# Swedish-Rock-Art-Research-Archives/rock-art-radnet

Hardware: AMD Instinct MI355X
Metric: train images/sec, ResNet50 Faster R-CNN 1000x600 (higher is better)
Workload: dtype f32; 1 GPU; full train step (RPN + RoiPoolingConv + classifier head + losses + 2x Adam), ResNet50, 1000x600, batch=1 per GPU, base frozen (train.py); identical panel and boxes on every rank and step (per-rank RNG seed); bench_workload=train, per_gpu_batch=1, global_batch=1, anchors=12, n_rois=20, mini_batch_form=image by image, parallelism=dp1, base_forward=launch list (hipGraph)

## Files before the change

### include/radnet_hip.h

```cpp
#ifndef RADNET_HIP_H
#define RADNET_HIP_H

#include <stdint.h>

#ifdef __cplusplus
extern "C" {
#endif

typedef struct radnet_ctx radnet_ctx;

#define RADNET_OK 0
#define RADNET_ERR_ARG (-1)
#define RADNET_ERR_HIP (-2)
#define RADNET_ERR_UNSUPPORTED (-3)

int radnet_create(int device, void* hip_stream, radnet_ctx** out);
void radnet_destroy(radnet_ctx* ctx);
const char* radnet_last_error(radnet_ctx* ctx);
int radnet_sync(radnet_ctx* ctx);
int radnet_set_stream(radnet_ctx* ctx, void* hip_stream);
int radnet_version(void);
int radnet_set_workspace(radnet_ctx* ctx, void* ws, uint64_t bytes);
int radnet_set_autotune(radnet_ctx* ctx, int enable);
int radnet_tuned_shapes(radnet_ctx* ctx);
int radnet_tune_save(radnet_ctx* ctx, const char* path);
int radnet_share_tuning(radnet_ctx* ctx, radnet_ctx* owner);
int radnet_tune_load(radnet_ctx* ctx, const char* path);
int radnet_force_config(radnet_ctx* ctx, int tile_a, int tile_b, int slices);
int radnet_force_waves(radnet_ctx* ctx, int waves);
int radnet_set_deterministic(radnet_ctx* ctx, int enable);
int radnet_get_deterministic(radnet_ctx* ctx);
int radnet_timing_enable(radnet_ctx* ctx, int enable);
int radnet_timing_read(radnet_ctx* ctx, int cls, double* ms, int64_t* launches, double* flops);
int radnet_timing_reset(radnet_ctx* ctx);

typedef struct radnet_conv_desc {
  const float* x;
  const float* w;
  float* y;
  const float* scale;
  const float* shift;
  const float* addend;
  int32_t nb, h, w_, c;
  int32_t oh, ow;
  int32_t kh, kw, stride, pad_t, pad_l;
  int32_t n;
  int32_t ldw, ldy, ld_add;
  int32_t act;
  int32_t act_cols;
  const float* dy;
  const float* gscale;
  float* dx;
  const float* dx_add;
  const float* dx_mask;
  float* dw;
  int32_t ld_dy, ld_dx, ld_dx_add, ld_dx_mask;
  int32_t dw_accumulate;
  float* db;
} radnet_conv_desc;

int radnet_conv_fwd(radnet_ctx* ctx, const radnet_conv_desc* d);
int radnet_gemm_batched(radnet_ctx* ctx, const float* a, const float* b, float* y, int32_t batch, int32_t m, int32_t n, int32_t k);
int radnet_winograd_filter(radnet_ctx* ctx, const float* w, int32_t c, int32_t n, int32_t ldw, float* u);
int radnet_winograd_input(radnet_ctx* ctx, const float* x, int32_t nb, int32_t h, int32_t w, int32_t c, float* v);
int radnet_winograd_output(radnet_ctx* ctx, const float* m, int32_t nb, int32_t oh, int32_t ow, int32_t n, const float* scale,
                           const float* shift, int32_t act, float* y, int32_t ldy);
int radnet_winograd_dy(radnet_ctx* ctx, const float* dy, int32_t nb, int32_t oh, int32_t ow, int32_t n, int32_t ld_dy,
                       const float* gscale, float* dz);
int radnet_wgrad_batched(radnet_ctx* ctx, const float* a, const float* dy, float* dw, int32_t batch, int32_t m, int32_t k, int32_t n,
                         int32_t accumulate);
int radnet_winograd_filter_grad(radnet_ctx* ctx, const float* du, int32_t c, int32_t n, int32_t ldw, float* dw, int32_t accumulate);
int radnet_winograd4_filter(radnet_ctx* ctx, const float* w, int32_t c, int32_t n, int32_t ldw, float* u);
int radnet_winograd4_input(radnet_ctx* ctx, const float* x, int32_t nb, int32_t h, int32_t w, int32_t c, float* v);
int radnet_winograd4_output(radnet_ctx* ctx, const float* m, int32_t nb, int32_t oh, int32_t ow, int32_t n, const float* scale,
                            const float* shift, int32_t act, float* y, int32_t ldy);
int radnet_winograd4_dy(radnet_ctx* ctx, const float* dy, int32_t nb, int32_t oh, int32_t ow, int32_t n, int32_t ld_dy,
                        const float* gscale, float* dz);
int radnet_winograd4_filter_grad(radnet_ctx* ctx, const float* du, int32_t c, int32_t n, int32_t ldw, float* dw, int32_t accumulate);
int radnet_conv_dgrad(radnet_ctx* ctx, const radnet_conv_desc* d);
int radnet_conv_wgrad(radnet_ctx* ctx, const radnet_conv_desc* d);
int radnet_conv_bwd(radnet_ctx* ctx, const radnet_conv_desc* d);
typedef struct radnet_wgrad_adam {
  float* p; float* g; float* m; float* v;
  int64_t n;
  int32_t t;
  float lr, beta1, beta2, eps, grad_scale;
} radnet_wgrad_adam;
int radnet_conv_wgrad_multi(radnet_ctx* ctx, const radnet_conv_desc* descs, int32_t n, const radnet_wgrad_adam* opt);
int radnet_conv_fwd_pair(radnet_ctx* ctx, const radnet_conv_desc* d1, const radnet_conv_desc* d2);
int radnet_conv_bottleneck(radnet_ctx* ctx, const radnet_conv_desc* db, const radnet_conv_desc* dc, const radnet_conv_desc* da);

int radnet_weights_to_bf16(radnet_ctx* ctx, const float* w, int32_t k, int32_t n, int32_t ldw, uint16_t* wt, int32_t ldk);
int radnet_conv_fwd_bf16(radnet_ctx* ctx, const radnet_conv_desc* d, const uint16_t* wt, int32_t ldk);
int radnet_conv_fwd_bf16_split(radnet_ctx* ctx, const radnet_conv_desc* d, const uint16_t* wt, int32_t ldk, int32_t ksplit);
int32_t radnet_conv_bf16_pick_split(int64_t m, int32_t n, int32_t k);
int64_t radnet_conv_bf16_tile_shape(int64_t rows, int32_t cols, int32_t* bm, int32_t* bn);

typedef struct radnet_bf16_dgrad_image {
  int64_t off;
  int32_t taps, c, n, ldw;
  uint16_t* wd;
  int32_t ldkd;
} radnet_bf16_dgrad_image;
int radnet_weights_to_bf16_dgrad(radnet_ctx* ctx, const float* w, int32_t taps, int32_t c, int32_t n, int32_t ldw, uint16_t* wd, int32_t ldkd);
int radnet_weights_to_bf16_dgrad_arena(radnet_ctx* ctx, const float* p, int64_t n_arena, const radnet_bf16_dgrad_image* layers, int32_t n_layers);
int radnet_conv_dgrad_bf16(radnet_ctx* ctx, const radnet_conv_desc* d, const uint16_t* wd, int32_t ldkd);
int radnet_conv_dgrad_bf16_split(radnet_ctx* ctx, const radnet_conv_desc* d, const uint16_t* wd, int32_t ldkd, int32_t ksplit);
int radnet_conv_wgrad_bf16(radnet_ctx* ctx, const radnet_conv_desc* d, int32_t msplit);
int32_t radnet_dgrad_bf16_pick_split(int64_t p, int32_t c, int32_t kd);
int32_t radnet_wgrad_bf16_pick_split(int64_t m, int32_t n, int32_t k);

int radnet_colsum(radnet_ctx* ctx, const float* g, int32_t m, int32_t n, int32_t ld, const float* gscale,
                  float* out, int32_t accumulate);

int radnet_maxpool_fwd(radnet_ctx* ctx, const float* x, float* y, int32_t nb, int32_t h, int32_t w, int32_t c,
                       int32_t k, int32_t s);
int radnet_roi_resize_fwd(radnet_ctx* ctx, const float* fmap, int32_t h, int32_t w, int32_t c, const float* rois,
                          int32_t r, int32_t ps, float* y);
int radnet_roi_resize_bwd(radnet_ctx* ctx, const float* dy, int32_t h, int32_t w, int32_t c, const float* rois,
                          int32_t r, int32_t ps, float* dfmap);
int radnet_avgpool_fwd(radnet_ctx* ctx, const float* x, int32_t r, int32_t hw, int32_t c, float* y);
int radnet_avgpool_bwd_relu(radnet_ctx* ctx, const float* dfeat, const float* y_act, int32_t r, int32_t hw, int32_t c,
                            float* dx);

int radnet_dense_heads_fwd(radnet_ctx* ctx, const float* feat, int32_t r, int32_t k, const float* w, int32_t ldw,
                           const float* b, int32_t nc, int32_t nreg, float* out_cls, float* out_regr);
int radnet_dense_heads_bwd(radnet_ctx* ctx, const float* feat, const float* dz, int32_t r, int32_t k, const float* w,
                           int32_t ldw, int32_t nout, float* dw, float* db, float* dfeat, int32_t accumulate);

uint64_t radnet_head_tail_scratch_bytes(int32_t r);
int radnet_head_tail_fwd(radnet_ctx* ctx, const float* y5, int32_t r, int32_t hw, int32_t c, const float* w, int32_t ldw, const float* b,
                         int32_t nc, int32_t nreg, float* feat, float* p_cls, float* p_regr, const float* y1, const float* y2,
                         float* dz, float* losses, int32_t groups, const int32_t* group_live, void* scratch);

int radnet_rpn_loss(radnet_ctx* ctx, const float* pred, int32_t ld_pred, const float* y_cls, const float* y_regr,
                    int32_t m, int32_t a, int32_t bce_mode, float* dz, int32_t ld_dz, float* losses,
                    double* scratch8);
int radnet_det_loss(radnet_ctx* ctx, const float* p_cls, const float* p_regr, const float* y1, const float* y2,
                    int32_t r, int32_t nc, int32_t nreg, float* dz, float* losses);

int radnet_adam_step(radnet_ctx* ctx, float* p, float* g, float* m, float* v, int64_t n, int32_t t, float lr,
                     float beta1, float beta2, float eps, float grad_scale, int32_t zero_grad);
int radnet_adam_step_affine(radnet_ctx* ctx, float* p, float* g, float* m, float* v, int64_t n, int32_t t, float lr, float beta1, float beta2,
                            float eps, float grad_scale, int32_t zero_grad, int64_t bias_off, int64_t bias_len, const float* scale,
                            const float* t0, float* shift);
typedef struct radnet_adam_wino {
  int64_t off;
  int32_t c, n;
  float* u;
} radnet_adam_wino;
int radnet_adam_step_fused(radnet_ctx* ctx, float* p, float* g, float* m, float* v, int64_t n, int32_t t, float lr, float beta1, float beta2,
                           float eps, float grad_scale, int32_t zero_grad, int64_t bias_off, int64_t bias_len, const float* scale,
                           const float* t0, float* shift, const radnet_adam_wino* layers, int32_t n_layers);
int radnet_adam_step_tail(radnet_ctx* ctx, float* p, float* g, float* m, float* v, int64_t n, int32_t t, float lr, float beta1, float beta2,
                          float eps, float grad_scale, int32_t zero_grad, int64_t bias_off, int64_t bias_len, const float* scale,
                          const float* t0, float* shift, const radnet_adam_wino* layers, int32_t n_layers, int64_t sweep_from);
typedef struct radnet_adam_bf16 {
  int64_t off;
  int32_t k, n, ldw;
  uint16_t* wt;
  int32_t ldk;
} radnet_adam_bf16;
int radnet_adam_step_bf16(radnet_ctx* ctx, float* p, float* g, float* m, float* v, int64_t n, int32_t t, float lr, float beta1, float beta2,
                          float eps, float grad_scale, int32_t zero_grad, int64_t bias_off, int64_t bias_len, const float* scale,
                          const float* t0, float* shift, const radnet_adam_bf16* layers, int32_t n_layers);

uint64_t radnet_proposals_ws_bytes(int64_t n_anchors_total);
int radnet_rpn_to_roi(radnet_ctx* ctx, const float* pred, int32_t ld_pred, int32_t rows, int32_t cols, int32_t a,
                      const double* anchor_wh_host, double std_scaling, int32_t use_regr, double overlap_thresh,
                      int32_t max_boxes, int64_t* out_boxes, float* out_probs, int32_t* out_count, void* ws);
int radnet_nms(radnet_ctx* ctx, const double* boxes, const float* probs, int32_t n, double overlap_thresh,
               int32_t max_boxes, int32_t* out_idx, int32_t* out_count, void* ws);

int radnet_anchor_targets(radnet_ctx* ctx, const double* gt, const int32_t* gt_is_bg, int32_t g, int32_t width,
                          int32_t height, int32_t rw, int32_t rh, int32_t fw, int32_t fh, const double* anchor_sizes_host,
                          int32_t ns, const double* anchor_ratios_host, int32_t nr, double rpn_stride,
                          double max_overlap, uint8_t* valid, uint8_t* overlap, double* regr, int32_t* best_anchor,
                          int32_t* n_for_gt, void* scratch);
int radnet_anchor_targets_pack(radnet_ctx* ctx, const uint8_t* valid, const uint8_t* overlap, const double* regr,
                               int32_t fw, int32_t fh, int32_t a, double std_scaling, float* y_cls, float* y_regr);

int radnet_roi_targets(radnet_ctx* ctx, const int64_t* rois, int32_t n, const double* gt, const int32_t* gt_cls, int32_t g,
                       int32_t width, int32_t height, int32_t rw, int32_t rh, double rpn_stride, double min_overlap,
                       double max_overlap, const double* regr_std_host4, int32_t bg_class, uint8_t* keep, int32_t* cls,
                       int32_t* box, double* t, double* iou, const int32_t* n_dev);
int radnet_roi_batch_pack(radnet_ctx* ctx, const int32_t* sel, int32_t r, const int32_t* cls, const int32_t* box,
                          const double* t, int32_t nc, int32_t bg_class, float* rois_out, float* y1, float* y2);

int64_t radnet_host_choice_round(double* live_p, int64_t* live_idx, int64_t* n_live_io, int64_t* found, int64_t n_found,
                                 const double* x, int64_t k, double* cdf, uint8_t* sel);

int radnet_preprocess_bgr(radnet_ctx* ctx, const uint8_t* img, int32_t h, int32_t w, int32_t cpad, float* out);
int radnet_copy_bytes(radnet_ctx* ctx, void* dst, const void* src, uint64_t bytes);
int radnet_resize_bicubic_u8(radnet_ctx* ctx, const uint8_t* src, int32_t sh, int32_t sw, uint8_t* dst, int32_t dh,
                             int32_t dw, int32_t channels);
int radnet_resize_bicubic_window_u8(radnet_ctx* ctx, const uint8_t* src, int32_t sh, int32_t sw, int32_t y0, int32_t x0, int32_t wh,
                                    int32_t ww, uint8_t* dst, int32_t dh, int32_t dw, int32_t channels);
int radnet_warp_affine_u8(radnet_ctx* ctx, const uint8_t* src, int32_t sh, int32_t sw, int32_t channels, uint8_t* dst, int32_t dh,
                          int32_t dw, const int32_t* col_tab, const int32_t* row_tab);
int radnet_aug_gather_u8(radnet_ctx* ctx, const uint8_t* src, int32_t sh, int32_t sw, int32_t y0, int32_t x0, int32_t wh, int32_t ww,
                         int32_t transform, uint8_t* dst);
int radnet_aug_extent_u8(radnet_ctx* ctx, const uint8_t* img, int32_t h, int32_t w, int32_t* out4);
int radnet_aug_histogram_u8(radnet_ctx* ctx, const uint8_t* img, int32_t h, int32_t w, int32_t all_channels, uint32_t* bins256);
#define RADNET_AUG_BRIGHTNESS 0
#define RADNET_AUG_CONTRAST 1
#define RADNET_AUG_SALT_PEPPER 2
#define RADNET_AUG_GAUSSIAN 3
#define RADNET_AUG_POISSON 4
int radnet_aug_pointwise_u8(radnet_ctx* ctx, const uint8_t* src, uint8_t* dst, int32_t h, int32_t w, int32_t mode, int32_t grey, double p0,
                            double p1, uint64_t noise_seed, uint32_t field_id);
#define RADNET_PNG_UNFILTER_BAND_ROWS 512
#define RADNET_PNG_UNFILTER_CHUNK_BYTES 96
int radnet_png_unfilter_u8(radnet_ctx* ctx, uint8_t* stream, int32_t rows, int32_t rowbytes, int32_t bpp);
typedef struct radnet_png_segment {
  int64_t offset;
  int32_t rows;
  int32_t rowbytes;
} radnet_png_segment;
#define RADNET_PNG_SEGMENT_TARGET_ROWS 64
int radnet_png_plan_segments(const uint8_t* stream, int64_t stream_offset, int32_t rows, int32_t rowbytes, int32_t target_rows,
                             radnet_png_segment* out, int32_t cap);
int radnet_png_unfilter_segments_u8(radnet_ctx* ctx, uint8_t* base, int64_t base_len, const radnet_png_segment* segs_host,
                                    const radnet_png_segment* segs_dev, int32_t count, int32_t bpp);
int radnet_png_expand_bgr_u8(radnet_ctx* ctx, const uint8_t* stream, int32_t pass_h, int32_t pass_w, int32_t rowbytes, int32_t color_type,
                             int32_t bit_depth, const uint8_t* palette_bgr, uint8_t* dst, int32_t dst_h, int32_t dst_w, int32_t y0,
                             int32_t x0, int32_t dy, int32_t dx);
int radnet_png_filter_rows_u8(radnet_ctx* ctx, const uint8_t* img, int32_t h, int32_t w, int32_t channels, int64_t pitch_bytes, int32_t mode,
                              uint8_t* stream);
#define RADNET_DEFLATE_CHUNK 65536
#define RADNET_DEFLATE_TILE 4096
#define RADNET_DEFLATE_SYMBOLS 286
#define RADNET_DEFLATE_HEADER_MAX_BITS 2048
typedef struct radnet_deflate_code {
  uint16_t bits, length;
} radnet_deflate_code;
int radnet_deflate_rle_scan_u8(radnet_ctx* ctx, const uint8_t* stream, int64_t n, uint32_t* hist, uint64_t* adler_parts);
int radnet_deflate_rle_emit_u8(radnet_ctx* ctx, const uint8_t* stream, int64_t n, const radnet_deflate_code* code, const uint8_t* header_bits,
                               int32_t header_nbits, int32_t dist_nbits, uint8_t* pieces, int64_t piece_cap, uint32_t* sizes);
int64_t radnet_deflate_piece_cap(const radnet_deflate_code* code, int32_t header_nbits, int32_t dist_nbits);
int radnet_deflate_pack(radnet_ctx* ctx, const uint8_t* pieces, int64_t piece_cap, const uint32_t* sizes, int32_t count, uint8_t* out,
                        int64_t out_cap, uint64_t* total);
// ... 292 lines not shown
```

### rock-art-radnet_amd/csrc/adam.hip

```cpp
#include "radnet_internal.h"
#include "adam_update.h"
#include "radnet_wino4.h"

namespace {

constexpr int kAdamWinoMax = 12;
constexpr int kAdamBf16Max = 16;
constexpr int kAdamBf16Tile = 64;
constexpr int kAdamGapMax = kAdamBf16Max + 1;

struct AdamArgs {
  float4 *p, *g, *m, *v;
  float lr_t, b1, b2, eps, gs;
  int zero_grad;
  long long aff_off4, aff_n4;
  const float4 *aff_scale, *aff_t0;
  float4* aff_shift;
  long long gap0[kAdamGapMax], pref[kAdamGapMax + 1];
  int ngap;
  unsigned sweep_blocks;
};

__device__ __forceinline__ void adam_one(float4& pp, const float4& gg, float4& mm, float4& vv, float lr_t, float b1, float b2, float eps, float gs) {
  adam_update1(pp.x, gg.x, mm.x, vv.x, lr_t, b1, b2, eps, gs);
  adam_update1(pp.y, gg.y, mm.y, vv.y, lr_t, b1, b2, eps, gs);
  adam_update1(pp.z, gg.z, mm.z, vv.z, lr_t, b1, b2, eps, gs);
  adam_update1(pp.w, gg.w, mm.w, vv.w, lr_t, b1, b2, eps, gs);
}

__device__ __forceinline__ float4 adam_at(const AdamArgs& a, long long i) {
  float4 pp = a.p[i], mm = a.m[i], vv = a.v[i];
  adam_one(pp, a.g[i], mm, vv, a.lr_t, a.b1, a.b2, a.eps, a.gs);
  a.p[i] = pp;
  a.m[i] = mm;
  a.v[i] = vv;
  if (a.zero_grad) a.g[i] = make_float4(0.f, 0.f, 0.f, 0.f);
  return pp;
}

__device__ __forceinline__ void adam_sweep(const AdamArgs& a) {
  const long long rest = a.pref[a.ngap];
  for (long long j = (long long)blockIdx.x * blockDim.x + threadIdx.x; j < rest; j += (long long)a.sweep_blocks * blockDim.x) {
    long long at = a.gap0[0];
    for (int q = 1; q < a.ngap; ++q) {
      const long long first = a.pref[q], to = a.gap0[q] - first;
      at = j >= first ? to : at;
    }
    const long long i = at + j;
    const float4 pp = adam_at(a, i);
    if (a.aff_shift != nullptr && i >= a.aff_off4 && i < a.aff_off4 + a.aff_n4) {
      const long long s = i - a.aff_off4;
      const float4 sc = a.aff_scale[s], c = a.aff_t0[s];
      a.aff_shift[s] = make_float4(sc.x * pp.x + c.x, sc.y * pp.y + c.y, sc.z * pp.z + c.z, sc.w * pp.w + c.w);
    }
  }
}

struct AdamWino {
  long long off4[kAdamWinoMax];
  int cn4[kAdamWinoMax];
  int unit0[kAdamWinoMax + 1];
  float* u[kAdamWinoMax];
  int n;
  int load_only;
};
__global__ void __launch_bounds__(256) adam_kernel(AdamArgs a, AdamWino wz) {
  if (blockIdx.x < a.sweep_blocks) {
    adam_sweep(a);
    return;
  }
  __shared__ float4 taps[9][64];
  const int unit = (int)(blockIdx.x - a.sweep_blocks);
  int layer = 0;
  for (int l = 1; l < wz.n; ++l)
    if (unit >= wz.unit0[l]) layer = l;
  const int cn4 = wz.cn4[layer];
  const long long j0 = (long long)(unit - wz.unit0[layer]) * 64;
  for (int it = threadIdx.x; it < 9 * 64; it += 256) {
    const int tap = it >> 6, jj = it & 63;
    const long long i = wz.off4[layer] + (long long)tap * cn4 + j0 + jj;
    taps[tap][jj] = wz.load_only ? a.p[i] : adam_at(a, i);
  }
  __syncthreads();
  if (threadIdx.x < 64) {
    float4 t[6][3];
#pragma unroll
    for (int bb = 0; bb < 3; ++bb) {
      float4 col[3], o[6];
#pragma unroll
      for (int aa = 0; aa < 3; ++aa) col[aa] = taps[aa * 3 + bb][threadIdx.x];
      g6(col, o);
#pragma unroll
      for (int aa = 0; aa < 6; ++aa) t[aa][bb] = o[aa];
    }
    float4* dst = reinterpret_cast<float4*>(wz.u[layer]) + j0 + threadIdx.x;
#pragma unroll
    for (int aa = 0; aa < 6; ++aa) {
      float4 o[6];
      g6(t[aa], o);
#pragma unroll
      for (int bb = 0; bb < 6; ++bb) dst[(long long)(6 * aa + bb) * cn4] = o[bb];
    }
  }
}

struct AdamBf16 {
  long long off4[kAdamBf16Max];
  int k[kAdamBf16Max], n[kAdamBf16Max], ldw4[kAdamBf16Max], ldk[kAdamBf16Max];
  int ntn[kAdamBf16Max];
  int unit0[kAdamBf16Max + 1];
  uint16_t* wt[kAdamBf16Max];
  int nl;
};
__global__ void __launch_bounds__(256) adam_bf16_kernel(AdamArgs a, AdamBf16 lz) {
  if (blockIdx.x < a.sweep_blocks) {
    adam_sweep(a);
    return;
  }
  __shared__ float tile[kAdamBf16Tile][kAdamBf16Tile + 1];
  const int unit = (int)(blockIdx.x - a.sweep_blocks);
  int layer = 0;
  for (int l = 1; l < lz.nl; ++l)
    if (unit >= lz.unit0[l]) layer = l;
  const int u = unit - lz.unit0[layer];
  const int k0 = (u / lz.ntn[layer]) * kAdamBf16Tile, n0 = (u % lz.ntn[layer]) * kAdamBf16Tile;
  const int K = lz.k[layer], ldw4 = lz.ldw4[layer];
  const int c4 = threadIdx.x & 15;
#pragma unroll
  for (int it = 0; it < 4; ++it) {
    const int r = (threadIdx.x >> 4) + 16 * it;
    const int kk = k0 + r, j4 = n0 / 4 + c4;
    float4 pp = make_float4(0.f, 0.f, 0.f, 0.f);
    if (kk < K && j4 < ldw4) pp = adam_at(a, lz.off4[layer] + (long long)kk * ldw4 + j4);
    tile[r][4 * c4] = pp.x; tile[r][4 * c4 + 1] = pp.y; tile[r][4 * c4 + 2] = pp.z; tile[r][4 * c4 + 3] = pp.w;
  }
  __syncthreads();
  const int N = lz.n[layer], ldk = lz.ldk[layer];
#pragma unroll
  for (int it = 0; it < 2; ++it) {
    const int q = threadIdx.x + 256 * it;
    const int c = q >> 3, kc = (q & 7) * 8;
    const int col = n0 + c, kk = k0 + kc;
    if (col >= N || kk >= ldk) continue;
    uint16_t h[8];
#pragma unroll
    for (int e = 0; e < 8; ++e) h[e] = kk + e < K ? __builtin_bit_cast(uint16_t, (__bf16)tile[kc + e][c]) : (uint16_t)0;
    uint4 o;
    o.x = h[0] | ((unsigned)h[1] << 16); o.y = h[2] | ((unsigned)h[3] << 16);
    o.z = h[4] | ((unsigned)h[5] << 16); o.w = h[6] | ((unsigned)h[7] << 16);
    *reinterpret_cast<uint4*>(lz.wt[layer] + (long long)col * ldk + kk) = o;
  }
}

struct AdamRange {
  int64_t off, len;
};

float adam_lr_t(float lr, float beta1, float beta2, int t) { return radnet_adam_lr_t(lr, beta1, beta2, t); }

int adam_check(radnet_ctx* ctx, const char* who, const float* p, const float* g, const float* m, const float* v, int64_t n, int32_t t,
               int64_t bias_off, int64_t bias_len, const float* scale, const float* t0, const float* shift) {
  if (!p || !g || !m || !v) RADNET_FAIL(ctx, RADNET_ERR_ARG, "%s: null arena", who);
  if (shift != nullptr && (!scale || !t0)) RADNET_FAIL(ctx, RADNET_ERR_ARG, "%s: shift without scale / t0", who);
  if ((n % 4) || (bias_off % 4) || (bias_len % 4) || n < 0 || bias_off < 0 || bias_len < 0 || bias_off + bias_len > n)
    RADNET_FAIL(ctx, RADNET_ERR_ARG, "%s: arena length %lld, bias range [%lld, +%lld) must be multiples of 4 inside the arena", who, (long long)n,
                (long long)bias_off, (long long)bias_len);
  if (((uintptr_t)p | (uintptr_t)g | (uintptr_t)m | (uintptr_t)v) & 15) RADNET_FAIL(ctx, RADNET_ERR_ARG, "%s: arenas must be 16-byte aligned", who);
  if (shift && (((uintptr_t)scale | (uintptr_t)t0 | (uintptr_t)shift) & 15)) RADNET_FAIL(ctx, RADNET_ERR_ARG, "%s: scale / t0 / shift must be 16-byte aligned", who);
  if (t < 1) RADNET_FAIL(ctx, RADNET_ERR_ARG, "%s: step counter starts at 1", who);
  return RADNET_OK;
}

int adam_gaps(radnet_ctx* ctx, const char* who, AdamRange* r, int nr, int64_t n, int64_t bias_off, int64_t bias_len, AdamArgs& a) {
  std::sort(r, r + nr, [](const AdamRange& x, const AdamRange& y) { return x.off < y.off; });
  long long at4 = 0;
  a.ngap = 0;
  a.pref[0] = 0;
  for (int q = 0; q <= nr; ++q) {
    if (q < nr) {
      if ((r[q].off & 3) || (r[q].len & 3) || r[q].off < 0 || r[q].len <= 0 || r[q].off + r[q].len > n)
        RADNET_FAIL(ctx, RADNET_ERR_ARG, "%s: layer [%lld, +%lld) must be multiples of 4 inside the arena", who, (long long)r[q].off, (long long)r[q].len);
      if (r[q].off / 4 < at4) RADNET_FAIL(ctx, RADNET_ERR_ARG, "%s: the layers at %lld and %lld overlap", who, (long long)r[q - 1].off, (long long)r[q].off);
      if (bias_len > 0 && r[q].off < bias_off + bias_len && bias_off < r[q].off + r[q].len)
        RADNET_FAIL(ctx, RADNET_ERR_ARG, "%s: layer [%lld, +%lld) overlaps the bias range", who, (long long)r[q].off, (long long)r[q].len);
    }
    const long long end4 = q < nr ? r[q].off / 4 : n / 4;
    a.gap0[a.ngap] = at4;
    a.pref[a.ngap + 1] = a.pref[a.ngap] + (end4 - at4);
    ++a.ngap;
    if (q < nr) at4 = end4 + r[q].len / 4;
  }
  a.sweep_blocks = (unsigned)grid_for(std::max<long long>(a.pref[a.ngap], 1), 256, 8192);
  return RADNET_OK;
}

int adam_prepare(radnet_ctx* ctx, const char* who, float* p, float* g, float* m, float* v, int64_t n, int32_t t, float lr, float beta1,
                 float beta2, float eps, float grad_scale, int32_t zero_grad, int64_t bias_off, int64_t bias_len, const float* scale,
                 const float* t0, float* shift, AdamRange* r, int nr, AdamArgs& a) {
  if (int rc = adam_check(ctx, who, p, g, m, v, n, t, bias_off, bias_len, scale, t0, shift)) return rc;
  a.p = reinterpret_cast<float4*>(p); a.g = reinterpret_cast<float4*>(g); a.m = reinterpret_cast<float4*>(m); a.v = reinterpret_cast<float4*>(v);
  a.lr_t = adam_lr_t(lr, beta1, beta2, t);
  a.b1 = beta1; a.b2 = beta2; a.eps = eps; a.gs = grad_scale;
  a.zero_grad = (int)zero_grad;
  a.aff_off4 = bias_off / 4;
  a.aff_n4 = shift ? bias_len / 4 : 0;
  a.aff_scale = reinterpret_cast<const float4*>(scale); a.aff_t0 = reinterpret_cast<const float4*>(t0); a.aff_shift = reinterpret_cast<float4*>(shift);
  return adam_gaps(ctx, who, r, nr, n, bias_off, shift ? bias_len : 0, a);
}

int adam_fused(radnet_ctx* ctx, const char* who, float* p, float* g, float* m, float* v, int64_t n, int32_t t, float lr, float beta1,
               float beta2, float eps, float grad_scale, int32_t zero_grad, int64_t bias_off, int64_t bias_len, const float* scale,
               const float* t0, float* shift, const radnet_adam_wino* layers, int32_t n_layers, int64_t sweep_from = 0) {
  if (!ctx) return RADNET_ERR_ARG;
  if (n_layers < 0 || n_layers > kAdamWinoMax || (n_layers > 0 && !layers)) RADNET_FAIL(ctx, RADNET_ERR_ARG, "%s: %d layers (at most %d, in a table)", who, n_layers, kAdamWinoMax);
  AdamWino wz{};
  AdamRange r[kAdamGapMax];
  wz.n = n_layers;
  wz.load_only = sweep_from > 0 ? 1 : 0;
  for (int l = 0; l < n_layers; ++l) {
    const radnet_adam_wino& d = layers[l];
    if (!d.u || d.c <= 0 || d.n <= 0 || (d.n & 3) || ((uintptr_t)d.u & 15) || (int64_t)d.c * d.n / 4 >= (1ll << 28) || ((int64_t)d.c * d.n / 4) % 64)
      RADNET_FAIL(ctx, RADNET_ERR_ARG, "%s: layer %d (offset %lld, c %d, n %d) does not describe a dense [3][3][c][n] kernel with c*n a multiple of 256 and a 16-byte aligned u",
                  who, l, (long long)d.off, d.c, d.n);
    wz.off4[l] = d.off / 4;
    wz.cn4[l] = (int)((int64_t)d.c * d.n / 4);
    wz.u[l] = d.u;
    wz.unit0[l + 1] = wz.unit0[l] + wz.cn4[l] / 64;
    r[l] = {d.off, 9ll * d.c * d.n};
  }
  int nr = n_layers;
  if (sweep_from > 0) {
    if ((sweep_from & 3) || sweep_from > n) RADNET_FAIL(ctx, RADNET_ERR_ARG, "%s: sweep_from %lld must be a multiple of 4 inside the arena", who, (long long)sweep_from);
    std::sort(r, r + n_layers, [](const AdamRange& x, const AdamRange& y) { return x.off < y.off; });
    int64_t at = 0;
    for (int l = 0; l <= n_layers; ++l) {
      const int64_t end = l < n_layers ? r[l].off : sweep_from;
      if (l < n_layers && (r[l].off < at || r[l].off + r[l].len > sweep_from))
        RADNET_FAIL(ctx, RADNET_ERR_ARG, "%s: layer [%lld, +%lld) overlaps another or reaches past sweep_from", who, (long long)r[l].off, (long long)r[l].len);
      if (end > at) {
        if (nr + 1 >= kAdamGapMax) RADNET_FAIL(ctx, RADNET_ERR_ARG, "%s: too many layers for the gap table", who);
        r[nr++] = {at, end - at};
      }
      if (l < n_layers) at = r[l].off + r[l].len;
    }
  }
  AdamArgs a{};
  if (int rc = adam_prepare(ctx, who, p, g, m, v, n, t, lr, beta1, beta2, eps, grad_scale, zero_grad, bias_off, bias_len, scale, t0, shift, r, nr, a)) return rc;
  hipLaunchKernelGGL(adam_kernel, dim3(a.sweep_blocks + (unsigned)wz.unit0[n_layers]), dim3(256), 0, ctx->stream, a, wz);
  RADNET_CHECK_LAUNCH(ctx, who);
  return RADNET_OK;
}

}

extern "C" int radnet_adam_step(radnet_ctx* ctx, float* p, float* g, float* m, float* v, int64_t n, int32_t t, float lr, float beta1,
// ... 56 lines not shown
```

### rock-art-radnet_amd/csrc/conv_args.h

```cpp
#pragma once

constexpr int BK = 32;
constexpr int NTHREADS = 256;
constexpr int kNumCU = 256;

struct GemmArgs {
  const float* x;
  const float* w;
  float* y;
  const float* scale;
  const float* shift;
  const float* addend;
  const float* mask;
  const float* in_scale;
  float* partial;
  int H, W, C;
  int OH, OW;
  int KW, npos;
  int stride, pad_t, pad_l;
  int M, N, K;
  int ldw, ldy, ld_add, ld_mask;
  int act, act_cols;
  int flip;
  int cin_fwd;
  const int* units;
  unsigned long long magic_ohow, magic_ow;
  int OHOW;
  unsigned x_bytes, w_bytes;
  unsigned y_bytes, add_bytes, mask_bytes;
  int batch;
  long long x_bstride, w_bstride, y_bstride;
  unsigned* counters;
  unsigned long long* stamps;
  int xcd_batch;
  int zper;
};

struct TailArgs {
  const float* w2; const float* sc2; const float* sh2; const float* add; float* y;
  const float* w3; const float* sc3; const float* sh3; float* t;
  int N2, ldw2, ldy2, ld_add2, ldw3, ldt;
  unsigned w2_bytes, w3_bytes, y_bytes, add_bytes, t_bytes;
};

struct WgradArgs {
  const float* x;
  const float* dy;
  const float* gscale;
  float* dw;
  float* db;
  int H, W, C, OH, OW, KW, stride, pad_t, pad_l;
  int M, N, K;
  int ld_dy, ldw;
  int mt_per_split;
  int atomic;
  const int* rowtab;
  int mpad;
  int xcd_batch;
  unsigned x_bias;
  unsigned x_bytes, dy_bytes;
  int batch, splits;
  long long x_bstride, dy_bstride, dw_bstride;
  float* slabs;
  unsigned* counters;
  int accumulate;
  int tiles_x, tiles_y;
  float* ow;
  float* om;
  float* ov;
  float lr_t, beta1, beta2, eps, grad_scale;
  int pad_opt;
};

constexpr int kWgradMultiMax = 16;
struct WgradMultiMap {
  unsigned first[kWgradMultiMax + 1];
  unsigned wx[kWgradMultiMax], wy[kWgradMultiMax];
  int n;
};
struct WgradOptScalars {
  float lr_t, beta1, beta2, eps, grad_scale;
};

struct PairMap {
  unsigned n_a, n_w;
  unsigned ax, ay;
  unsigned wx, wy;
};

struct ChainStage {
  GemmArgs g;
  const float* t_src;
  float* t_dst;
  const float* t_scale;
  const float* t_shift;
  int t_nb, t_h, t_w, t_c, t_th, t_tw, t_act, t_ldy;
  unsigned t_dst_bytes;
  int type;
};
struct ChainItem {
  int stage, bx, by, bz;
  int d0_first, d0_count, d1_first, d1_count;
  int sig0, sig1, pad0, pad1;
};
struct ChainHeader {
  unsigned next, exited, error, last_error;
  unsigned runs, host_lo, host_hi, pad;
};

constexpr int kCtrStride = 16;

static_assert(sizeof(GemmArgs) == 264 && sizeof(TailArgs) == 120 && sizeof(WgradArgs) == 248 && sizeof(PairMap) == 24, "kernel argument layout");
static_assert(sizeof(WgradMultiMap) == 200 && sizeof(WgradOptScalars) == 20, "multi-problem weight-gradient launch layout");
static_assert(sizeof(ChainStage) == 336 && sizeof(ChainItem) == 48 && sizeof(ChainHeader) == 32, "chain list layout");
```

### rock-art-radnet_amd/csrc/conv_device.h

```cpp
#pragma once
#include <hip/hip_runtime.h>
#include "conv_args.h"

typedef float f32x16 __attribute__((ext_vector_type(16)));
typedef float f32x4 __attribute__((ext_vector_type(4)));

namespace {
#ifndef RADNET_CHAINS
#define RADNET_CHAINS 2
#endif
constexpr int kChainsSmallTile = RADNET_CHAINS;

#ifdef RADNET_DIAG_STAMPS
#define RADNET_STAMP(var) const unsigned long long var = __builtin_amdgcn_s_memtime()
#else
#define RADNET_STAMP(var)
#endif

__device__ __forceinline__ int div_magic(int m, unsigned long long magic) {
  return (int)(((unsigned long long)(unsigned)m * magic) >> 40);
}

constexpr unsigned kOOB = 0x80000000u;
__device__ __forceinline__ __amdgpu_buffer_rsrc_t make_rsrc(const void* p, unsigned bytes) {
  return __builtin_amdgcn_make_buffer_rsrc(const_cast<void*>(p), 0, (int)bytes, 0x00020000);
}
__device__ __forceinline__ float4 buf_load4(__amdgpu_buffer_rsrc_t r, unsigned off) {
  f32x4 v = __builtin_bit_cast(f32x4, __builtin_amdgcn_raw_buffer_load_b128(r, (int)off, 0, 0));
  return make_float4(v.x, v.y, v.z, v.w);
}
__device__ __forceinline__ float4 buf_load4s(__amdgpu_buffer_rsrc_t r, unsigned voff, unsigned soff) {
  f32x4 v = __builtin_bit_cast(f32x4, __builtin_amdgcn_raw_buffer_load_b128(r, (int)voff, (int)__builtin_amdgcn_readfirstlane(soff), 0));
  return make_float4(v.x, v.y, v.z, v.w);
}
__device__ __forceinline__ float buf_load1s(__amdgpu_buffer_rsrc_t r, unsigned voff, unsigned soff) {
  return __builtin_bit_cast(float, __builtin_amdgcn_raw_buffer_load_b32(r, (int)voff, (int)__builtin_amdgcn_readfirstlane(soff), 0));
}
typedef unsigned u32x2 __attribute__((ext_vector_type(2)));
__device__ __forceinline__ int2 buf_load2i(__amdgpu_buffer_rsrc_t r, unsigned off) {
  const u32x2 v = __builtin_amdgcn_raw_buffer_load_b64(r, (int)off, 0, 0);
  return make_int2((int)v.x, (int)v.y);
}
__device__ __forceinline__ float buf_load1(__amdgpu_buffer_rsrc_t r, unsigned off) {
  return __builtin_bit_cast(float, __builtin_amdgcn_raw_buffer_load_b32(r, (int)off, 0, 0));
}
__device__ __forceinline__ float buf_load1_sc1(__amdgpu_buffer_rsrc_t r, unsigned off) {
  return __builtin_bit_cast(float, __builtin_amdgcn_raw_buffer_load_b32(r, (int)off, 0, 16));
}
__device__ __forceinline__ float4 buf_load4_sc1(__amdgpu_buffer_rsrc_t r, unsigned off) {
  f32x4 v = __builtin_bit_cast(f32x4, __builtin_amdgcn_raw_buffer_load_b128(r, (int)off, 0, 16));
  return make_float4(v.x, v.y, v.z, v.w);
}
__device__ __forceinline__ void buf_store4_sc1(__amdgpu_buffer_rsrc_t r, unsigned off, float4 v) {
  typedef unsigned u32x4 __attribute__((ext_vector_type(4)));
  f32x4 f = {v.x, v.y, v.z, v.w};
  __builtin_amdgcn_raw_buffer_store_b128(__builtin_bit_cast(u32x4, f), r, (int)off, 0, 16);
}
__device__ __forceinline__ void buf_store1_sc1(__amdgpu_buffer_rsrc_t r, unsigned off, float v) {
  __builtin_amdgcn_raw_buffer_store_b32(__builtin_bit_cast(unsigned, v), r, (int)off, 0, 16);
}
__device__ __forceinline__ void buf_store1(__amdgpu_buffer_rsrc_t r, unsigned off, float v) {
  __builtin_amdgcn_raw_buffer_store_b32(__builtin_bit_cast(unsigned, v), r, (int)off, 0, 0);
}
typedef float f32x2v __attribute__((ext_vector_type(2)));
__device__ __forceinline__ void buf_store2_sc1(__amdgpu_buffer_rsrc_t r, unsigned off, float2 v) {
  f32x2v f = {v.x, v.y};
  __builtin_amdgcn_raw_buffer_store_b64(__builtin_bit_cast(u32x2, f), r, (int)off, 0, 16);
}

__device__ __forceinline__ float f4_comp(const float4& v, int c) { return c == 0 ? v.x : c == 1 ? v.y : c == 2 ? v.z : v.w; }

struct NoStaging {
  __device__ __forceinline__ void operator()(int) const {}
};
template <int TM, int TN, int CH, typename Staging>
__device__ __forceinline__ void mfma_tile(const float* sA, const float* sB, int pitchA, int pitchB, int a_off, int b_off,
                                          f32x16 (&acc)[CH][TM][TN], Staging staging) {
  constexpr int kSteps = BK / 2;
  float a[3][TM], b[3][TN];
#pragma unroll
  for (int p = 0; p < 2; ++p) {
#pragma unroll
    for (int i = 0; i < TM; ++i) a[p][i] = sA[2 * p * pitchA + a_off + i * 32];
#pragma unroll
    for (int j = 0; j < TN; ++j) b[p][j] = sB[2 * p * pitchB + b_off + j * 32];
  }
#pragma unroll
  for (int s = 0; s < kSteps; ++s) {
    const int cur = s % 3, nxt = (s + 2) % 3;
    if (s + 2 < kSteps) {
#pragma unroll
      for (int i = 0; i < TM; ++i) a[nxt][i] = sA[(2 * s + 4) * pitchA + a_off + i * 32];
#pragma unroll
      for (int j = 0; j < TN; ++j) b[nxt][j] = sB[(2 * s + 4) * pitchB + b_off + j * 32];
    }
#pragma unroll
    for (int i = 0; i < TM; ++i)
#pragma unroll
      for (int j = 0; j < TN; ++j)
        acc[s % CH][i][j] = __builtin_amdgcn_mfma_f32_32x32x2f32(a[cur][i], b[cur][j], acc[s % CH][i][j], 0, 0, 0);
    staging(s);
    __builtin_amdgcn_sched_group_barrier(0x100, TM + TN, 0);
    __builtin_amdgcn_sched_group_barrier(0x008, TM * TN, 0);
    __builtin_amdgcn_sched_barrier(0);
  }
}

constexpr int kRowPitch = BK + 4;
template <int TM, int TN, int CH, bool B_ROWMAJOR, int KSTEPS, typename Staging>
__device__ __forceinline__ void mfma_tile_rows(const float* sA, const float* sB, int pitchB, int a_off, int b_off,
                                               f32x16 (&acc)[CH][TM][TN], Staging staging) {
  constexpr int kSteps = KSTEPS;
  float4 af[2][TM], bq[2][TN];
  float bf[3][TN];
#pragma unroll
  for (int i = 0; i < TM; ++i) af[0][i] = *reinterpret_cast<const float4*>(sA + a_off + i * 32 * kRowPitch);
  if (B_ROWMAJOR) {
#pragma unroll
    for (int j = 0; j < TN; ++j) bq[0][j] = *reinterpret_cast<const float4*>(sB + b_off + j * 32 * kRowPitch);
  } else {
#pragma unroll
    for (int p = 0; p < 2; ++p)
#pragma unroll
      for (int j = 0; j < TN; ++j) bf[p][j] = sB[p * pitchB + b_off + j * 32];
  }
#pragma unroll
  for (int s = 0; s < kSteps; ++s) {
    const int q = s >> 2, c = s & 3;
    const bool group_reads = c == 1 && q + 1 < kSteps / 4;
    const bool step_reads = !B_ROWMAJOR && s + 2 < kSteps;
    if (group_reads) {
#pragma unroll
      for (int i = 0; i < TM; ++i) af[(q + 1) & 1][i] = *reinterpret_cast<const float4*>(sA + a_off + i * 32 * kRowPitch + 8 * (q + 1));
      if (B_ROWMAJOR) {
#pragma unroll
        for (int j = 0; j < TN; ++j) bq[(q + 1) & 1][j] = *reinterpret_cast<const float4*>(sB + b_off + j * 32 * kRowPitch + 8 * (q + 1));
      }
    }
    if (step_reads) {
      const int s2 = s + 2;
#pragma unroll
      for (int j = 0; j < TN; ++j) bf[s2 % 3][j] = sB[(8 * (s2 >> 2) + (s2 & 3)) * pitchB + b_off + j * 32];
    }
#pragma unroll
    for (int i = 0; i < TM; ++i)
#pragma unroll
      for (int j = 0; j < TN; ++j)
        acc[s % CH][i][j] = __builtin_amdgcn_mfma_f32_32x32x2f32(f4_comp(af[q & 1][i], c), B_ROWMAJOR ? f4_comp(bq[q & 1][j], c) : bf[s % 3][j],
                                                                 acc[s % CH][i][j], 0, 0, 0);
    staging(s);
    if (group_reads && (B_ROWMAJOR || step_reads)) __builtin_amdgcn_sched_group_barrier(0x100, TM + TN, 0);
    else if (group_reads) __builtin_amdgcn_sched_group_barrier(0x100, TM, 0);
    else if (step_reads) __builtin_amdgcn_sched_group_barrier(0x100, TN, 0);
    __builtin_amdgcn_sched_group_barrier(0x008, TM * TN, 0);
    __builtin_amdgcn_sched_barrier(0);
  }
}
}
```

### rock-art-radnet_amd/csrc/conv_wgrad.hip

```cpp
#include "conv_host.h"
#include "conv_igemm_body.h"
#include "conv_wgrad_body.h"
#include "wgrad_multi_plan.h"

namespace {
template <int BMK, int BN>
__global__ void __launch_bounds__(NTHREADS) conv_wgrad_kernel(WgradArgs g) {
  __shared__ __attribute__((aligned(16))) float lds[wgrad_lds_floats<BMK, BN>()];
  if (g.batch > 1 && g.xcd_batch) {
    const unsigned gx = gridDim.x, gy = gridDim.y, total = gx * gy * gridDim.z;
    const unsigned lin = blockIdx.x + gx * (blockIdx.y + gy * blockIdx.z), per = total >> 3;
    const unsigned l2 = lin < (per << 3) ? (lin & 7u) * per + (lin >> 3) : lin;
    const unsigned z = l2 / (gx * gy), r = l2 - z * gx * gy, y = r / gx;
    conv_wgrad_body<BMK, BN>(g, lds, r - y * gx, y, z);
    return;
  }
  conv_wgrad_body<BMK, BN>(g, lds, blockIdx.x, blockIdx.y, blockIdx.z);
}


template <int ABM>
__global__ void __launch_bounds__(NTHREADS) conv_bwd_pair_kernel(GemmArgs ga, WgradArgs gw, PairMap pm) {
  constexpr int kLds = igemm_lds_floats<ABM, 64, 1>() > wgrad_lds_floats<64, 64>() ? igemm_lds_floats<ABM, 64, 1>() : wgrad_lds_floats<64, 64>();
  __shared__ __attribute__((aligned(16))) float lds[kLds];
// ... 128 lines not shown
    else if (bmk == 128 && bn == 64) RADNET_LAUNCH((conv_wgrad_kernel<128, 64>), grid, block, 0, ctx->stream, ctx->arm0, ctx->arm1, g);
    else if (bmk == 64 && bn == 128) RADNET_LAUNCH((conv_wgrad_kernel<64, 128>), grid, block, 0, ctx->stream, ctx->arm0, ctx->arm1, g);
    else RADNET_LAUNCH((conv_wgrad_kernel<64, 64>), grid, block, 0, ctx->stream, ctx->arm0, ctx->arm1, g);
    RADNET_CHECK_LAUNCH(ctx, "conv_wgrad");
    return RADNET_OK;
  };
  int bmk = (d->c % 128 == 0) ? 128 : 64, bn = g.N > 64 ? 128 : 64, splits = 1;
  const radnet_shape_key key{2 + (d->dw_accumulate == 1 ? 1 : 0) + (batch > 1 ? 16 : 0), g.M, g.N, g.K, g.C, d->kh * d->kw, batch > 1 ? batch : g.stride};
  auto it = ctx->tuned->find(key);
  if (ctx->force_a > 0) {
    bmk = ctx->force_a; bn = ctx->force_b; splits = ctx->force_splits < 1 ? 1 : ctx->force_splits;
    if (bmk < 64) bmk = 64;
    if (bn < 64) bn = 64;
    if (d->c % bmk) RADNET_FAIL(ctx, RADNET_ERR_ARG, "conv_wgrad: forced k tile %d does not divide c=%d", bmk, d->c);
  } else if (it != ctx->tuned->end()) {
    bmk = it->second.a; bn = it->second.b; splits = it->second.splits;
  } else if (const radnet_tuned* nb = (ctx->autotune == 2 && d->dw_accumulate != 1) ? radnet_tuned_neighbour(*ctx->tuned, key) : nullptr;
             nb && (nb->splits <= 1 || (nmt / nb->splits >= 2 && radnet_cdiv(nmt, radnet_cdiv(nmt, nb->splits)) == nb->splits))) {
    bmk = nb->a; bn = nb->b; splits = nb->splits;
    (*ctx->tuned)[key] = *nb;
  } else if (ctx->autotune && d->dw_accumulate != 1) {
    PairPause pause(ctx);
    struct WCand { float ms; int bmk, bn, s; };
    std::vector<WCand> seen;
    const bool for_pair = pause.saved != nullptr && batch <= 1 && d->dx != nullptr;
    for (int cb = 128; cb >= 64; cb -= 64) {
      if (d->c % cb) continue;
      if (for_pair && cb != 64) continue;
      for (int cn = 128; cn >= 64; cn -= 64) {
        if (cn > 64 && g.N <= 64) continue;
        if (for_pair && cn != 64) continue;
        for (int s0 : {1, 2, 3, 4, 6, 8, 12, 16}) {
          if (s0 > 1 && (nmt / s0 < 2 || radnet_cdiv(nmt, radnet_cdiv(nmt, s0)) != s0)) continue;
          for (int s = s0; s >= (batch > 1 ? -s0 : s0); s -= 2 * s0) {
            float ms = 0.f;
            int rc = radnet_time_launches(ctx, [&]() { return launch(cb, cn, s); }, 3, &ms);
            if (rc == RADNET_ERR_UNSUPPORTED) continue;
            if (rc != RADNET_OK) return rc;
            seen.push_back(WCand{ms, cb, cn, s});
          }
        }
      }
    }
    std::sort(seen.begin(), seen.end(), [](const WCand& a, const WCand& b) { return a.ms < b.ms; });
    float best = 1e30f;
    for (size_t i = 0; i < seen.size() && i < 4; ++i) {
      float ms = 0.f;
      const int rc = radnet_time_launches_twice(ctx, [&]() { return launch(seen[i].bmk, seen[i].bn, seen[i].s); }, 12, &ms);
      if (rc != RADNET_OK) return rc;
      if (ms < best) { best = ms; bmk = seen[i].bmk; bn = seen[i].bn; splits = seen[i].s; }
    }
    (*ctx->tuned)[key] = radnet_tuned{bmk, bn, splits, best, 4};
    if (getenv("RADNET_TUNE_LOG"))
      fprintf(stderr, "radnet tune: wgrad M=%d N=%d K=%d C=%d -> tile %dx%d slices %d : %.1f us (%.1f TFLOP/s)\n", g.M, g.N, g.K, g.C,
              bmk, bn, splits, best * 1e3, 2.0 * g.M * g.N * g.K / (best * 1e9));
    if (d->dw_accumulate == 2)
      RADNET_CHECK_HIP(ctx, hipMemset2DAsync(d->dw, (size_t)g.ldw * sizeof(float), 0, (size_t)g.N * sizeof(float), (size_t)g.K, ctx->stream));
  } else {
    const radnet_shape_key k0{2, g.M, g.N, g.K, g.C, d->kh * d->kw, g.stride};
    auto it0 = ctx->tuned->find(k0);
    if (it0 != ctx->tuned->end()) {
      bmk = it0->second.a; bn = it0->second.b; splits = it0->second.splits;
    } else {
      long long tiles = (long long)radnet_cdiv(g.K, bmk) * radnet_cdiv(g.N, bn);
      if (tiles < kNumCU && bmk == 128 && bn == 128) {
        bn = 64;
        tiles = (long long)radnet_cdiv(g.K, bmk) * radnet_cdiv(g.N, bn);
      }
      while (tiles * splits < 2 * kNumCU && nmt / (splits * 2) >= 4 && splits < 16) splits *= 2;
    }
  }
  radnet_timing_arm(ctx);
  {
    g.db = d->db;
    if (d->db && d->dw_accumulate == 0) RADNET_CHECK_HIP(ctx, hipMemsetAsync(d->db, 0, (size_t)g.N * sizeof(float), ctx->stream));
    int rc = launch(bmk, bn, splits);
    if (rc == RADNET_ERR_UNSUPPORTED && splits < 0) {
      splits = -splits;
      rc = launch(bmk, bn, splits);
    }
    if (rc == RADNET_ERR_UNSUPPORTED && splits > 1) {
      while (rc == RADNET_ERR_UNSUPPORTED && splits > 1) {
        splits = splits > 2 ? splits / 2 : 1;
        while (splits > 1 && radnet_cdiv(nmt, radnet_cdiv(nmt, splits)) != splits) --splits;
        rc = launch(bmk, bn, splits);
      }
    }
    if (rc == RADNET_ERR_UNSUPPORTED) RADNET_FAIL(ctx, rc, "conv_wgrad: no launch shape fits (tile %dx%d, workspace %llu bytes)", bmk, bn, (unsigned long long)ctx->ws_bytes);
    if (rc != RADNET_OK) return rc;
  }
  RADNET_CHECK_LAUNCH(ctx, "conv_wgrad");
  radnet_timing_end_armed(ctx, 2, 2.0 * g.M * g.N * g.K * (batch > 1 ? batch : 1));
  return RADNET_OK;
}

extern "C" int radnet_conv_wgrad(radnet_ctx* ctx, const radnet_conv_desc* d) { return run_wgrad(ctx, d, 1, 0, 0, 0); }

extern "C" int radnet_conv_bwd(radnet_ctx* ctx, const radnet_conv_desc* d) {
  if (!ctx || !d) return RADNET_ERR_ARG;
  static const bool disabled = radnet_env_flag("RADNET_NO_BWD_PAIR");
  if (disabled || ctx->pair_capture != nullptr || !d->dx) {
    int rc = radnet_conv_wgrad(ctx, d);
    return rc != RADNET_OK || !d->dx ? rc : radnet_conv_dgrad(ctx, d);
  }
  PairCapture pc;
  const int timed = ctx->timing;
  ctx->timing = 0;
  ctx->pair_capture = &pc;
  int rc = radnet_conv_wgrad(ctx, d);
  if (rc == RADNET_OK) rc = radnet_conv_dgrad(ctx, d);
  ctx->pair_capture = nullptr;
  ctx->timing = timed;
  if (rc != RADNET_OK) return rc;
  if (pc.a_slab_bytes + pc.w_slab_bytes > ctx->ws_bytes) pc.a_ok = false;
  if (!(pc.have_a && pc.have_w && pc.a_ok && pc.w_ok)) {
    rc = radnet_conv_wgrad(ctx, d);
    return rc != RADNET_OK ? rc : radnet_conv_dgrad(ctx, d);
  }
  PairMap pm{pc.ax * pc.ay, pc.wx * pc.wy * pc.wz, pc.ax, pc.ay, pc.wx, pc.wy};
  radnet_timing_arm(ctx);
  if (pc.a_bm == 32) RADNET_LAUNCH(conv_bwd_pair_kernel<32>, dim3(pm.n_a + pm.n_w), dim3(NTHREADS), 0, ctx->stream, ctx->arm0, ctx->arm1, pc.ga, pc.gw, pm);
  else RADNET_LAUNCH(conv_bwd_pair_kernel<64>, dim3(pm.n_a + pm.n_w), dim3(NTHREADS), 0, ctx->stream, ctx->arm0, ctx->arm1, pc.ga, pc.gw, pm);
  RADNET_CHECK_LAUNCH(ctx, "conv_bwd_pair");
  radnet_timing_end_armed(ctx, 4, pc.flops);
  return RADNET_OK;
}

radnet_ctx::MultiTables::~MultiTables() {
  for (auto& e : v)
    if (e.second) (void)hipFree(e.second);
}

namespace {
const WgradArgs* get_multi_table(radnet_ctx* ctx, const WgradArgs* host, int n) {
  const size_t bytes = sizeof(WgradArgs) * (size_t)n;
  auto& v = ctx->multi_tables.v;
  for (auto& e : v)
    if (e.first.size() == bytes && memcmp(e.first.data(), host, bytes) == 0) return (const WgradArgs*)e.second;
  if (v.size() >= 256) {
    (void)hipFree(v.front().second);
    v.erase(v.begin());
  }
  void* dev = nullptr;
  if (hipMalloc(&dev, bytes) != hipSuccess) return nullptr;
  if (hipMemcpy(dev, host, bytes, hipMemcpyHostToDevice) != hipSuccess) {
    (void)hipFree(dev);
    return nullptr;
  }
  v.emplace_back(std::vector<char>((const char*)host, (const char*)host + bytes), dev);
  return (const WgradArgs*)dev;
}
}

extern "C" int radnet_conv_wgrad_multi(radnet_ctx* ctx, const radnet_conv_desc* descs, int32_t n, const radnet_wgrad_adam* opt) {
  if (!ctx || n < 0 || (n > 0 && !descs)) return RADNET_ERR_ARG;
  if (n == 0) return RADNET_OK;
  if (ctx->pair_capture != nullptr) RADNET_FAIL(ctx, RADNET_ERR_ARG, "conv_wgrad_multi: called inside radnet_conv_bwd");
  const bool adam = opt != nullptr && opt->p != nullptr;
  if (adam) {
    if (!opt->g || !opt->m || !opt->v || opt->n <= 0) RADNET_FAIL(ctx, RADNET_ERR_ARG, "conv_wgrad_multi: optimizer block with a null arena");
    if (opt->t < 1) RADNET_FAIL(ctx, RADNET_ERR_ARG, "conv_wgrad_multi: step counter starts at 1");
  }
  std::vector<PairCapture> pcs((size_t)n);
  std::vector<WgradMultiItem> items((size_t)n);
  const int timed = ctx->timing;
  for (int i = 0; i < n; ++i) {
    radnet_conv_desc d = descs[i];
    d.dx = nullptr;
    if (adam) {
      if (d.dw_accumulate == 1) RADNET_FAIL(ctx, RADNET_ERR_ARG, "conv_wgrad_multi: problem %d adds to its gradient; the optimizer epilogue needs the whole gradient", i);
      const int64_t off = d.dw - opt->g, last = (int64_t)(d.kh * d.kw * d.c - 1) * d.ldw + d.n;
      if (!d.dw || d.dw < opt->g || off + last > opt->n) RADNET_FAIL(ctx, RADNET_ERR_ARG, "conv_wgrad_multi: problem %d's dw lies outside the gradient arena", i);
    }
    ctx->timing = 0;
    ctx->pair_capture = &pcs[i];
    const int rc = radnet_conv_wgrad(ctx, &d);
    ctx->pair_capture = nullptr;
    ctx->timing = timed;
    if (rc != RADNET_OK) return rc;
    PairCapture& pc = pcs[i];
    if (!pc.have_w) RADNET_FAIL(ctx, RADNET_ERR_UNSUPPORTED, "conv_wgrad_multi: problem %d produced no launch", i);
    const bool ordered = pc.gw.slabs != nullptr;
    if (adam && !ordered && pc.gw.atomic)
      RADNET_FAIL(ctx, RADNET_ERR_UNSUPPORTED, "conv_wgrad_multi: problem %d adds its slices with atomics (no final writer); the optimizer epilogue needs ordered reductions", i);
    items[i] = WgradMultiItem{pc.w_bmk, pc.w_bn, pc.wx, pc.wy, pc.wz, ordered ? pc.w_slab_need : 0, ordered ? pc.wx * pc.wy : 0u};
  }
  std::vector<WgradMultiLaunch> plan((size_t)n);
  const int nl = wgrad_multi_plan(items.data(), n, ctx->ws_bytes, (unsigned)kAuxWgradCounterCount, plan.data(), n);
  if (nl < 0) RADNET_FAIL(ctx, RADNET_ERR_UNSUPPORTED, "conv_wgrad_multi: the problems do not fit a launch plan (%d)", nl);
  WgradOptScalars os{};
  if (adam) os = WgradOptScalars{radnet_adam_lr_t(opt->lr, opt->beta1, opt->beta2, opt->t), opt->beta1, opt->beta2, opt->eps, opt->grad_scale};
  for (int l = 0; l < nl; ++l) {
    const WgradMultiLaunch& L = plan[l];
    WgradArgs host[kWgradMultiMax];
    memset(host, 0, sizeof(host));
    double flops = 0.0;
    for (int k = 0; k < L.n; ++k) {
      const PairCapture& pc = pcs[L.problem[k]];
      WgradArgs& g = host[k];
      memcpy(&g, &pc.gw, sizeof(g));
      if (g.slabs != nullptr) {
        g.slabs = reinterpret_cast<float*>(reinterpret_cast<char*>(ctx->ws) + L.slab_off[k]);
        g.counters = reinterpret_cast<unsigned*>(ctx->aux + kAuxWgradCounters) + L.counter_off[k];
      }
      g.ow = g.om = g.ov = nullptr;
      g.lr_t = g.beta1 = g.beta2 = g.eps = g.grad_scale = 0.f;
      g.pad_opt = 0;
      if (adam) {
        const int64_t off = g.dw - opt->g;
        g.ow = opt->p + off; g.om = opt->m + off; g.ov = opt->v + off;
      }
      flops += 2.0 * g.M * g.N * g.K;
    }
    const WgradArgs* tab = get_multi_table(ctx, host, L.n);
    if (!tab) RADNET_FAIL(ctx, RADNET_ERR_HIP, "conv_wgrad_multi: cannot place the problem table on the device");
    const dim3 grid(L.map.first[L.n]), block(NTHREADS);
    radnet_timing_arm(ctx);
    if (L.bmk == 128 && L.bn == 128) RADNET_LAUNCH((conv_wgrad_multi_kernel<128, 128>), grid, block, 0, ctx->stream, ctx->arm0, ctx->arm1, tab, L.map, os);
    else if (L.bmk == 128 && L.bn == 64) RADNET_LAUNCH((conv_wgrad_multi_kernel<128, 64>), grid, block, 0, ctx->stream, ctx->arm0, ctx->arm1, tab, L.map, os);
    else if (L.bmk == 64 && L.bn == 128) RADNET_LAUNCH((conv_wgrad_multi_kernel<64, 128>), grid, block, 0, ctx->stream, ctx->arm0, ctx->arm1, tab, L.map, os);
    else RADNET_LAUNCH((conv_wgrad_multi_kernel<64, 64>), grid, block, 0, ctx->stream, ctx->arm0, ctx->arm1, tab, L.map, os);
    RADNET_CHECK_LAUNCH(ctx, "conv_wgrad_multi");
    radnet_timing_end_armed(ctx, 2, flops);
  }
  return RADNET_OK;
}

extern "C" int radnet_wgrad_batched(radnet_ctx* ctx, const float* a, const float* dy, float* dw, int32_t batch, int32_t m, int32_t k, int32_t n,
                                    int32_t accumulate) {
  if (!ctx || !a || !dy || !dw) return RADNET_ERR_ARG;
  if (batch < 1 || batch > 4096) RADNET_FAIL(ctx, RADNET_ERR_ARG, "wgrad_batched: batch %d", batch);
  radnet_conv_desc d{};
  d.x = a; d.dy = dy; d.dw = dw;
  d.nb = 1; d.h = 1; d.w_ = m; d.c = k; d.oh = 1; d.ow = m;
  d.kh = 1; d.kw = 1; d.stride = 1; d.pad_t = 0; d.pad_l = 0; d.n = n;
  d.ldw = n; d.ld_dy = n;
  d.dw_accumulate = accumulate;
  return run_wgrad(ctx, &d, batch, (long long)m * k, (long long)m * n, (long long)k * n);
}
```

### rock-art-radnet_amd/csrc/conv_wgrad_body.h

```cpp
#pragma once
#include "adam_update.h"
#include "conv_device.h"

namespace {
template <int BMK, int BN>
constexpr int wgrad_lds_floats() { return 2 * BK * ((BMK + 4) + (BN + 4)); }

template <int BMK, int BN, bool OPT = false>
__device__ __forceinline__ void conv_wgrad_body(const WgradArgs& g, float* __restrict__ lds, const unsigned bid_x, const unsigned bid_y, const unsigned bid_z) {
  constexpr int TM = BMK / 64, TN = BN / 64;
  constexpr int PA = BMK + 4, PB = BN + 4;
  constexpr int A_ITERS = BMK / 32, B_ITERS = BN / 32;
  constexpr int CPRA = BMK / 4, CPRB = BN / 4;
  float* sA0 = lds;
  float* sB0 = lds + 2 * BK * PA;

  const int tid = threadIdx.x;
  const int lane = tid & 63, wave = tid >> 6;
  const int hi = lane >> 5, l31 = lane & 31;
  const int wm = wave >> 1, wn = wave & 1;
  const int k0 = bid_x * BMK, n0 = bid_y * BN;

  const int pos = k0 / g.C;
  const int cbase = k0 - pos * g.C;

  const int a_k4 = tid % CPRA, a_mr = tid / CPRA;
  const int b_n4 = tid % CPRB, b_mr = tid / CPRB;
  const bool a_kv = (k0 + a_k4 * 4) < g.K;
  const bool b_nv = (n0 + b_n4 * 4) < g.N;
  float4 gs = make_float4(1, 1, 1, 1);
  if (g.gscale != nullptr && b_nv) gs = *reinterpret_cast<const float4*>(g.gscale + n0 + b_n4 * 4);

  const int nmt = (g.M + BK - 1) / BK;
  const int zsplit = g.batch > 1 ? (int)(bid_z % (unsigned)g.splits) : (int)bid_z;
  const long long bp = g.batch > 1 ? (long long)(bid_z / (unsigned)g.splits) : 0;
  const int mt_begin = zsplit * g.mt_per_split;
  int mt_end = mt_begin + g.mt_per_split;
  if (mt_end > nmt) mt_end = nmt;

  const __amdgpu_buffer_rsrc_t rx = make_rsrc(reinterpret_cast<const char*>(g.x + bp * g.x_bstride) - g.x_bias, g.x_bytes + g.x_bias);
  const __amdgpu_buffer_rsrc_t rdy = make_rsrc(g.dy + bp * g.dy_bstride, g.dy_bytes);
  float4 ra[A_ITERS], rb[B_ITERS];
  const bool do_bias = g.db != nullptr && bid_x == 0;
  float4 csum = make_float4(0.f, 0.f, 0.f, 0.f);

  const __amdgpu_buffer_rsrc_t rtab = make_rsrc(g.rowtab + (size_t)pos * g.mpad, (unsigned)g.mpad * 4u);
  const unsigned s_tap = (unsigned)(cbase * 4);
  unsigned b_voff[B_ITERS], e_voff[A_ITERS];
#pragma unroll
  for (int i = 0; i < B_ITERS; ++i) b_voff[i] = b_nv ? (unsigned)(((b_mr + (NTHREADS / CPRB) * i) * g.ld_dy + n0 + b_n4 * 4) * 4) : kOOB;
#pragma unroll
  for (int i = 0; i < A_ITERS; ++i) e_voff[i] = (unsigned)((a_mr + (NTHREADS / CPRA) * i) * 4);
  const unsigned a_lane = a_kv ? (unsigned)a_k4 * 16u : kOOB;
  const unsigned dy_tile_bytes = (unsigned)(BK * g.ld_dy * 4);
  struct Entries {
    unsigned e[A_ITERS];
  };
  Entries ent0, ent1;

  constexpr int kLoadOps = A_ITERS + B_ITERS, kStoreOps = A_ITERS + B_ITERS;
  auto entry_op = [&](int i, int mt, Entries& en) {
    en.e[i] = __builtin_amdgcn_raw_buffer_load_b32(rtab, (int)e_voff[i], (int)__builtin_amdgcn_readfirstlane(mt < mt_end ? (unsigned)mt * (BK * 4u) : kOOB), 0);
  };
  auto load_op = [&](int idx, int mt, const Entries& en) {
    const bool live = mt < mt_end;
    if (idx < A_ITERS) {
      ra[idx] = buf_load4s(rx, en.e[idx] + a_lane, live ? s_tap : kOOB);
    } else {
      rb[idx - A_ITERS] = buf_load4s(rdy, b_voff[idx - A_ITERS], live ? (unsigned)mt * dy_tile_bytes : kOOB);
    }
  };
  auto store_op = [&](int idx, int buf) {
    float* sA = sA0 + buf * BK * PA;
    float* sB = sB0 + buf * BK * PB;
    if (idx < A_ITERS) {
      const int i = idx;
      *reinterpret_cast<float4*>(sA + (a_mr + (NTHREADS / CPRA) * i) * PA + a_k4 * 4) = ra[i];
    } else {
      const int i = idx - A_ITERS;
      float4 v = rb[i];
      v.x *= gs.x; v.y *= gs.y; v.z *= gs.z; v.w *= gs.w;
      *reinterpret_cast<float4*>(sB + (b_mr + (NTHREADS / CPRB) * i) * PB + b_n4 * 4) = v;
      csum.x += do_bias ? v.x : 0.f; csum.y += do_bias ? v.y : 0.f; csum.z += do_bias ? v.z : 0.f; csum.w += do_bias ? v.w : 0.f;
    }
  };

  constexpr int CH = (TM * TN >= 4) ? 1 : kChainsSmallTile;
  f32x16 accs[CH][TM][TN];
#pragma unroll
  for (int c = 0; c < CH; ++c)
#pragma unroll
    for (int i = 0; i < TM; ++i)
#pragma unroll
      for (int j = 0; j < TN; ++j)
#pragma unroll
        for (int r = 0; r < 16; ++r) accs[c][i][j][r] = 0.f;

  if (mt_begin < mt_end) {
#pragma unroll
    for (int i = 0; i < A_ITERS; ++i) entry_op(i, mt_begin, ent0);
#pragma unroll
    for (int op = 0; op < kLoadOps; ++op) load_op(op, mt_begin, ent0);
#pragma unroll
    for (int i = 0; i < A_ITERS; ++i) entry_op(i, mt_begin + 1, ent1);
#pragma unroll
    for (int op = 0; op < kStoreOps; ++op) store_op(op, 0);
    __syncthreads();
    const int a_off = hi * PA + wm * (BMK / 2) + l31;
    const int b_off = hi * PB + wn * (BN / 2) + l31;
    constexpr int kSteps = BK / 2;
    constexpr int kStoreSteps = (kStoreOps < kSteps - 1 - kLoadOps) ? kStoreOps : kSteps - 1 - kLoadOps;
    constexpr int kStoresPerStep = (kStoreOps + kStoreSteps - 1) / kStoreSteps;
    constexpr int kFirstStoreStep = kSteps - 1 - kStoreSteps;
    static_assert(kStoreSteps >= 1, "tile too large for the 16-step staging schedule");
    auto step = [&](int mt, int buf, Entries& cur, Entries& nxt) {
      mfma_tile<TM, TN, CH>(sA0 + buf * BK * PA, sB0 + buf * BK * PB, PA, PB, a_off, b_off, accs, [&](int s) {
        if (s < kLoadOps) {
          load_op(s, mt + 1, cur);
          if (s < A_ITERS) entry_op(s, mt + 2, nxt);
        } else if (s >= kFirstStoreStep && s < kSteps - 1) {
#pragma unroll
          for (int q = 0; q < kStoresPerStep; ++q) {
            const int op = (s - kFirstStoreStep) * kStoresPerStep + q;
            if (op < kStoreOps) store_op(op, buf ^ 1);
          }
        }
      });
      __syncthreads();
    };
    for (int mt = mt_begin; mt < mt_end; mt += 2) {
      step(mt, 0, ent1, ent0);
      if (mt + 1 < mt_end) step(mt + 1, 1, ent0, ent1);
    }
  }
  f32x16(&acc)[TM][TN] = accs[0];
#pragma unroll
  for (int c = 1; c < CH; ++c)
#pragma unroll
    for (int i = 0; i < TM; ++i)
#pragma unroll
      for (int j = 0; j < TN; ++j) acc[i][j] += accs[c][i][j];

  const bool ordered = g.slabs != nullptr;
  float4 bias_t = make_float4(0.f, 0.f, 0.f, 0.f);
  if (do_bias) {
    float4* red = reinterpret_cast<float4*>(lds);
    red[tid] = csum;
    __syncthreads();
    if (tid < CPRB) {
      float4 t = red[tid];
      for (int q = 1; q < NTHREADS / CPRB; ++q) {
        const float4 u = red[tid + q * CPRB];
        t.x += u.x; t.y += u.y; t.z += u.z; t.w += u.w;
      }
      bias_t = t;
      const int n = n0 + tid * 4;
      if (!ordered && n < g.N) {
        atomicAdd(g.db + n, t.x);
        atomicAdd(g.db + n + 1, t.y);
        atomicAdd(g.db + n + 2, t.z);
        atomicAdd(g.db + n + 3, t.w);
      }
    }
    __syncthreads();
  }

  if (ordered) {
    const unsigned tile = ((unsigned)bp * (unsigned)g.tiles_y + bid_y) * (unsigned)g.tiles_x + bid_x;
    const unsigned lane_off = (unsigned)((wave * TM * TN * 64 + lane) * 16) * 4u;
    const size_t total_tiles = (size_t)(g.batch > 1 ? g.batch : 1) * g.tiles_y * g.tiles_x;
    const __amdgpu_buffer_rsrc_t rslab = make_rsrc(g.slabs + ((size_t)tile * g.splits + zsplit) * (BMK * BN), BMK * BN * 4u);
#pragma unroll
    for (int i = 0; i < TM; ++i)
#pragma unroll
      for (int j = 0; j < TN; ++j)
#pragma unroll
        for (int q = 0; q < 4; ++q)
          buf_store4_sc1(rslab, lane_off + (unsigned)(((i * TN + j) * 64 * 16 + q * 4) * 4),
                         make_float4(acc[i][j][4 * q], acc[i][j][4 * q + 1], acc[i][j][4 * q + 2], acc[i][j][4 * q + 3]));
    float* bias_slabs = g.slabs + total_tiles * g.splits * (size_t)(BMK * BN) + ((size_t)((unsigned)bp * g.tiles_y + bid_y) * g.splits) * BN;
    if (do_bias && tid < CPRB) {
      const __amdgpu_buffer_rsrc_t rb = make_rsrc(bias_slabs + (size_t)zsplit * BN, BN * 4u);
      buf_store4_sc1(rb, (unsigned)tid * 16u, bias_t);
    }
    asm volatile("s_waitcnt vmcnt(0)" ::: "memory");
    __syncthreads();
    volatile int* flag = reinterpret_cast<volatile int*>(lds);
    if (tid == 0) {
      const unsigned ticket = __hip_atomic_fetch_add(g.counters + tile, 1u, __ATOMIC_RELAXED, __HIP_MEMORY_SCOPE_AGENT);
      const int last = ticket == (unsigned)(g.splits - 1);
      if (last) __hip_atomic_store(g.counters + tile, 0u, __ATOMIC_RELAXED, __HIP_MEMORY_SCOPE_AGENT);
      flag[0] = last;
    }
    __syncthreads();
    if (flag[0] == 0) return;
    __builtin_amdgcn_fence(__ATOMIC_ACQUIRE, "wavefront");
#pragma unroll
    for (int i = 0; i < TM; ++i)
#pragma unroll
      for (int j = 0; j < TN; ++j)
#pragma unroll
        for (int r = 0; r < 16; ++r) acc[i][j][r] = 0.f;
    constexpr int kGroup = (TM * TN == 1) ? 4 : 1;
    for (int s0 = 0; s0 < g.splits; s0 += kGroup) {
      float4 v[kGroup][TM * TN * 4];
#pragma unroll
      for (int u = 0; u < kGroup; ++u) {
        const __amdgpu_buffer_rsrc_t rsrc = make_rsrc(g.slabs + ((size_t)tile * g.splits + (s0 + u < g.splits ? s0 + u : 0)) * (BMK * BN), BMK * BN * 4u);
        const unsigned off = (s0 + u < g.splits) ? lane_off : kOOB;
#pragma unroll
        for (int t = 0; t < TM * TN * 4; ++t) v[u][t] = buf_load4_sc1(rsrc, off + (unsigned)(((t >> 2) * 64 * 16 + (t & 3) * 4) * 4));
      }
#pragma unroll
      for (int u = 0; u < kGroup; ++u)
#pragma unroll
        for (int i = 0; i < TM; ++i)
#pragma unroll
          for (int j = 0; j < TN; ++j)
#pragma unroll
            for (int q = 0; q < 4; ++q) {
              const float4 w = v[u][(i * TN + j) * 4 + q];
              acc[i][j][4 * q] += w.x; acc[i][j][4 * q + 1] += w.y; acc[i][j][4 * q + 2] += w.z; acc[i][j][4 * q + 3] += w.w;
            }
    }
    if (do_bias && tid < CPRB) {
      float4 t = make_float4(0.f, 0.f, 0.f, 0.f);
      for (int z = 0; z < g.splits; ++z) {
        const __amdgpu_buffer_rsrc_t rb = make_rsrc(bias_slabs + (size_t)z * BN, BN * 4u);
        const float4 u = buf_load4_sc1(rb, (unsigned)tid * 16u);
        t.x += u.x; t.y += u.y; t.z += u.z; t.w += u.w;
      }
      const int n = n0 + tid * 4;
      if (n < g.N) {
        g.db[n] += t.x; g.db[n + 1] += t.y; g.db[n + 2] += t.z; g.db[n + 3] += t.w;
      }
    }
  }

  if (!ordered && g.atomic) {
#pragma unroll
    for (int j = 0; j < TN; ++j) {
      const int n = n0 + wn * (BN / 2) + j * 32 + l31;
#pragma unroll
      for (int i = 0; i < TM; ++i) {
#pragma unroll
        for (int r = 0; r < 16; ++r) {
          const int k = k0 + wm * (BMK / 2) + i * 32 + (r & 3) + 8 * (r >> 2) + 4 * hi;
          if (n < g.N && k < g.K) atomicAdd(g.dw + bp * g.dw_bstride + (size_t)k * g.ldw + n, acc[i][j][r]);
        }
      }
    }
    return;
  }
  if constexpr (OPT) {
    if (g.ow != nullptr) {
      const unsigned bytes = (unsigned)((size_t)g.K * (size_t)g.ldw * 4u);
      const __amdgpu_buffer_rsrc_t rw = make_rsrc(g.ow + bp * g.dw_bstride, bytes), rm = make_rsrc(g.om + bp * g.dw_bstride, bytes),
                                   rv = make_rsrc(g.ov + bp * g.dw_bstride, bytes);
      const unsigned ldw4 = (unsigned)g.ldw * 4u;
#pragma unroll
      for (int j = 0; j < TN; ++j) {
        const int n = n0 + wn * (BN / 2) + j * 32 + l31;
#pragma unroll
        for (int i = 0; i < TM; ++i) {
          const int kb = k0 + wm * (BMK / 2) + i * 32 + 4 * hi;
          const unsigned voff = (n < g.N && kb < g.K) ? ((unsigned)kb * (unsigned)g.ldw + (unsigned)n) * 4u : kOOB;
          float pw[16], pm[16], pv[16];
#pragma unroll
          for (int r = 0; r < 16; ++r) {
            const unsigned off = voff + (unsigned)((r & 3) + 8 * (r >> 2)) * ldw4;
            pw[r] = buf_load1(rw, off);
            pm[r] = buf_load1(rm, off);
            pv[r] = buf_load1(rv, off);
          }
#pragma unroll
          for (int r = 0; r < 16; ++r) {
            const unsigned off = voff + (unsigned)((r & 3) + 8 * (r >> 2)) * ldw4;
            adam_update1(pw[r], acc[i][j][r], pm[r], pv[r], g.lr_t, g.beta1, g.beta2, g.eps, g.grad_scale);
            buf_store1(rw, off, pw[r]);
            buf_store1(rm, off, pm[r]);
            buf_store1(rv, off, pv[r]);
          }
        }
      }
      return;
    }
  }
  const __amdgpu_buffer_rsrc_t rdw = make_rsrc(g.dw + bp * g.dw_bstride, (unsigned)((size_t)g.K * (size_t)g.ldw * 4u));
  const bool rmw = ordered && g.accumulate;
  const unsigned ldw4 = (unsigned)g.ldw * 4u;
#pragma unroll
  for (int j = 0; j < TN; ++j) {
    const int n = n0 + wn * (BN / 2) + j * 32 + l31;
#pragma unroll
    for (int i = 0; i < TM; ++i) {
      const int kb = k0 + wm * (BMK / 2) + i * 32 + 4 * hi;
      const unsigned voff = (n < g.N && kb < g.K) ? ((unsigned)kb * (unsigned)g.ldw + (unsigned)n) * 4u : kOOB;
      float old[16];
      if (rmw) {
#pragma unroll
        for (int r = 0; r < 16; ++r) old[r] = buf_load1(rdw, voff + (unsigned)((r & 3) + 8 * (r >> 2)) * ldw4);
      } else {
#pragma unroll
        for (int r = 0; r < 16; ++r) old[r] = 0.f;
      }
#pragma unroll
      for (int r = 0; r < 16; ++r) buf_store1(rdw, voff + (unsigned)((r & 3) + 8 * (r >> 2)) * ldw4, rmw ? old[r] + acc[i][j][r] : acc[i][j][r]);
    }
  }
}
}
```

### rock-art-radnet_amd/csrc/radnet_wino4.h

```cpp
#pragma once
#include <hip/hip_runtime.h>

namespace {

template <typename VT> __device__ __forceinline__ VT vzero();
template <> __device__ __forceinline__ float vzero<float>() { return 0.f; }
template <> __device__ __forceinline__ float2 vzero<float2>() { return make_float2(0.f, 0.f); }
template <> __device__ __forceinline__ float4 vzero<float4>() { return make_float4(0.f, 0.f, 0.f, 0.f); }
__device__ __forceinline__ float vmax0(float a) { return fmaxf(a, 0.f); }
__device__ __forceinline__ float2 vmax0(float2 a) { return make_float2(fmaxf(a.x, 0.f), fmaxf(a.y, 0.f)); }
__device__ __forceinline__ float4 vmax0(float4 a) { return make_float4(fmaxf(a.x, 0.f), fmaxf(a.y, 0.f), fmaxf(a.z, 0.f), fmaxf(a.w, 0.f)); }

template <typename VT> __device__ __forceinline__ void bt6(const VT (&d)[6], VT (&o)[6]) {
  o[0] = d[0] * 4.f + (d[4] - d[2] * 5.f);
  const VT p = d[4] - d[2] * 4.f, q = d[3] - d[1] * 4.f;
  o[1] = p + q;
  o[2] = p - q;
  const VT r = d[4] - d[2], t = (d[3] - d[1]) * 2.f;
  o[3] = r + t;
  o[4] = r - t;
  o[5] = d[1] * 4.f + (d[5] - d[3] * 5.f);
}
template <typename VT> __device__ __forceinline__ void at6(const VT (&m)[6], VT (&o)[4]) {
  const VT s12 = m[1] + m[2], d12 = m[1] - m[2], s34 = m[3] + m[4], d34 = m[3] - m[4];
  o[0] = (m[0] + s12) + s34;
  o[1] = d34 * 2.f + d12;
  o[2] = s34 * 4.f + s12;
  o[3] = (d34 * 8.f + d12) + m[5];
}
template <typename VT> __device__ __forceinline__ void a6(const VT (&y)[4], VT (&z)[6]) {
  const VT e = y[0] + y[2], o = y[1] + y[3];
  const VT e4 = y[2] * 4.f + y[0], o2 = y[3] * 8.f + y[1] * 2.f;
  z[0] = y[0];
  z[1] = e + o;
  z[2] = e - o;
  z[3] = e4 + o2;
  z[4] = e4 - o2;
  z[5] = y[3];
}
template <typename VT> __device__ __forceinline__ void g6(const VT (&g)[3], VT (&u)[6]) {
  const VT s = g[0] + g[2];
  u[0] = g[0] * 0.25f;
  u[1] = (s + g[1]) * (-1.f / 6.f);
  u[2] = (s - g[1]) * (-1.f / 6.f);
  const VT a = g[0] * (1.f / 24.f) + g[2] * (1.f / 6.f), b = g[1] * (1.f / 12.f);
  u[3] = a + b;
  u[4] = a - b;
  u[5] = g[2];
}
template <typename VT> __device__ __forceinline__ void gt6(const VT (&u)[6], VT (&w)[3]) {
  const VT s12 = u[1] + u[2], s34 = u[3] + u[4];
  w[0] = u[0] * 0.25f + (s12 * (-1.f / 6.f) + s34 * (1.f / 24.f));
  w[1] = (u[2] - u[1]) * (1.f / 6.f) + (u[3] - u[4]) * (1.f / 12.f);
  w[2] = (s12 * (-1.f / 6.f) + s34 * (1.f / 6.f)) + u[5];
}


}
```

### rock-art-radnet_amd/csrc/wgrad_multi_plan.cpp

```cpp
#include "wgrad_multi_plan.h"

#include <string.h>

int wgrad_multi_plan(const WgradMultiItem* items, int n, uint64_t ws_bytes, unsigned counter_cap, WgradMultiLaunch* out, int cap) {
  if (n < 0 || cap < 0 || (n > 0 && !items) || (cap > 0 && !out)) return kWgradMultiErrArg;
  const uint64_t kMaxGrid = 0x7fffffffull;
  for (int i = 0; i < n; ++i) {
    const WgradMultiItem& it = items[i];
    if ((it.bmk != 64 && it.bmk != 128) || (it.bn != 64 && it.bn != 128) || it.wx == 0 || it.wy == 0 || it.wz == 0) return kWgradMultiErrArg;
    if ((uint64_t)it.wx * it.wy * it.wz > kMaxGrid) return kWgradMultiErrFit;
    if (it.slab_bytes > ws_bytes || it.counters > counter_cap) return kWgradMultiErrFit;
  }
  int n_out = 0;
  for (int first = 0; first < n; ++first) {
    const int bmk = items[first].bmk, bn = items[first].bn;
    bool seen = false;
    for (int j = 0; j < first && !seen; ++j) seen = items[j].bmk == bmk && items[j].bn == bn;
    if (seen) continue;
    WgradMultiLaunch* cur = nullptr;
    uint64_t slab_at = 0, grid = 0;
    unsigned ctr_at = 0;
    for (int i = first; i < n; ++i) {
      const WgradMultiItem& it = items[i];
      if (it.bmk != bmk || it.bn != bn) continue;
      const uint64_t wgs = (uint64_t)it.wx * it.wy * it.wz;
      if (cur != nullptr && (cur->n == kWgradMultiMax || slab_at + it.slab_bytes > ws_bytes || (uint64_t)ctr_at + it.counters > counter_cap ||
                             grid + wgs > kMaxGrid))
        cur = nullptr;
      if (cur == nullptr) {
        if (n_out == cap) return kWgradMultiErrCap;
        cur = &out[n_out++];
        memset(cur, 0, sizeof(*cur));
        cur->bmk = bmk;
        cur->bn = bn;
        slab_at = 0;
        grid = 0;
        ctr_at = 0;
      }
      const int k = cur->n++;
      cur->problem[k] = i;
      cur->slab_off[k] = slab_at;
      cur->counter_off[k] = ctr_at;
      cur->map.first[k] = (unsigned)grid;
      cur->map.wx[k] = it.wx;
      cur->map.wy[k] = it.wy;
      grid += wgs;
      for (int q = k + 1; q <= kWgradMultiMax; ++q) cur->map.first[q] = (unsigned)grid;
      cur->map.n = cur->n;
      slab_at = (slab_at + it.slab_bytes + 255) & ~(uint64_t)255;
      ctr_at += it.counters;
    }
  }
  return n_out;
}
```

### rock-art-radnet_amd/csrc/wgrad_multi_plan.h

```cpp
#pragma once
#include <stdint.h>

#include "conv_args.h"

struct WgradMultiItem {
  int bmk, bn;
  unsigned wx, wy, wz;
  uint64_t slab_bytes;
  unsigned counters;
};

struct WgradMultiLaunch {
  int bmk, bn, n;
  int problem[kWgradMultiMax];
  uint64_t slab_off[kWgradMultiMax];
  unsigned counter_off[kWgradMultiMax];
  WgradMultiMap map;
};

constexpr int kWgradMultiErrArg = -1, kWgradMultiErrFit = -2, kWgradMultiErrCap = -3;

int wgrad_multi_plan(const WgradMultiItem* items, int n, uint64_t ws_bytes, unsigned counter_cap, WgradMultiLaunch* out, int cap);
```

### rock-art-radnet_amd/csrc/winograd.hip

```cpp
#include "radnet_internal.h"
#include "radnet_wino4.h"

namespace {

__device__ __forceinline__ float4 f4add(float4 a, float4 b) { return make_float4(a.x + b.x, a.y + b.y, a.z + b.z, a.w + b.w); }
__device__ __forceinline__ float4 f4sub(float4 a, float4 b) { return make_float4(a.x - b.x, a.y - b.y, a.z - b.z, a.w - b.w); }
__device__ __forceinline__ float4 f4half(float4 a) { return make_float4(0.5f * a.x, 0.5f * a.y, 0.5f * a.z, 0.5f * a.w); }

__global__ void __launch_bounds__(256) wino_filter_kernel(const float* __restrict__ g, int C, int N, int ldw, float* __restrict__ U) {
  const int n4 = N >> 2;
  const long long total = (long long)C * n4;
  for (unsigned i = blockIdx.x * blockDim.x + threadIdx.x; i < (unsigned)total; i += gridDim.x * blockDim.x) {
    const int c = (int)(i / (unsigned)n4), nq = (int)(i - (unsigned)c * (unsigned)n4);
    float4 w[3][3];
#pragma unroll
    for (int a = 0; a < 3; ++a)
#pragma unroll
      for (int b = 0; b < 3; ++b) w[a][b] = *reinterpret_cast<const float4*>(g + ((long long)(a * 3 + b) * C + c) * ldw + nq * 4);
    float4 t[4][3];
#pragma unroll
    for (int b = 0; b < 3; ++b) {
      t[0][b] = w[0][b];
      t[1][b] = f4half(f4add(f4add(w[0][b], w[1][b]), w[2][b]));
      t[2][b] = f4half(f4add(f4sub(w[0][b], w[1][b]), w[2][b]));
// ... 28 lines not shown
      for (int b = 0; b < 4; ++b) {
        const int iw = 2 * tj - 1 + b;
        d[a][b] = ((unsigned)ih < (unsigned)H && (unsigned)iw < (unsigned)W)
                      ? *reinterpret_cast<const float4*>(x + (((long long)img * H + ih) * W + iw) * C + cq * 4)
                      : make_float4(0.f, 0.f, 0.f, 0.f);
      }
    }
    float4 t[4][4];
#pragma unroll
    for (int b = 0; b < 4; ++b) {
      t[0][b] = f4sub(d[0][b], d[2][b]);
      t[1][b] = f4add(d[1][b], d[2][b]);
      t[2][b] = f4sub(d[2][b], d[1][b]);
      t[3][b] = f4sub(d[1][b], d[3][b]);
    }
    const long long ps = T * c4;
    float4* dst = reinterpret_cast<float4*>(V) + tile * c4 + cq;
#pragma unroll
    for (int a = 0; a < 4; ++a) {
      dst[(4 * a + 0) * ps] = f4sub(t[a][0], t[a][2]);
      dst[(4 * a + 1) * ps] = f4add(t[a][1], t[a][2]);
      dst[(4 * a + 2) * ps] = f4sub(t[a][2], t[a][1]);
      dst[(4 * a + 3) * ps] = f4sub(t[a][1], t[a][3]);
    }
  }
}

__global__ void __launch_bounds__(256) wino_output_kernel(const float* __restrict__ Mm, int nb, int OH, int OW, int N, int TH, int TW,
                                                          const float* __restrict__ scale, const float* __restrict__ shift, int act,
                                                          float* __restrict__ y, int ldy) {
  const int n4 = N >> 2;
  const long long T = (long long)nb * TH * TW, total = T * n4;
  for (unsigned i = blockIdx.x * blockDim.x + threadIdx.x; i < (unsigned)total; i += gridDim.x * blockDim.x) {
    const unsigned tile = i / (unsigned)n4;
    const int nq = (int)(i - tile * (unsigned)n4);
    const unsigned trow = tile / (unsigned)TW;
    const int tj = (int)(tile - trow * (unsigned)TW);
    const int img = (int)(trow / (unsigned)TH);
    const int ti = (int)(trow - (unsigned)img * (unsigned)TH);
    const long long ps = T * n4;
    const float4* src = reinterpret_cast<const float4*>(Mm) + tile * n4 + nq;
    float4 m[4][4];
#pragma unroll
    for (int a = 0; a < 4; ++a)
#pragma unroll
      for (int b = 0; b < 4; ++b) m[a][b] = src[(4 * a + b) * ps];
    float4 t[2][4];
#pragma unroll
    for (int b = 0; b < 4; ++b) {
      t[0][b] = f4add(f4add(m[0][b], m[1][b]), m[2][b]);
      t[1][b] = f4sub(f4sub(m[1][b], m[2][b]), m[3][b]);
    }
    const float4 sc = scale ? *reinterpret_cast<const float4*>(scale + nq * 4) : make_float4(1.f, 1.f, 1.f, 1.f);
    const float4 sh = shift ? *reinterpret_cast<const float4*>(shift + nq * 4) : make_float4(0.f, 0.f, 0.f, 0.f);
#pragma unroll
    for (int a = 0; a < 2; ++a) {
      const int oh = 2 * ti + a;
      if (oh >= OH) continue;
      const float4 o[2] = {f4add(f4add(t[a][0], t[a][1]), t[a][2]), f4sub(f4sub(t[a][1], t[a][2]), t[a][3])};
#pragma unroll
      for (int b = 0; b < 2; ++b) {
        const int ow = 2 * tj + b;
        if (ow >= OW) continue;
        float4 v = make_float4(o[b].x * sc.x + sh.x, o[b].y * sc.y + sh.y, o[b].z * sc.z + sh.z, o[b].w * sc.w + sh.w);
        if (act == 1) v = make_float4(fmaxf(v.x, 0.f), fmaxf(v.y, 0.f), fmaxf(v.z, 0.f), fmaxf(v.w, 0.f));
        *reinterpret_cast<float4*>(y + (((long long)img * OH + oh) * OW + ow) * ldy + nq * 4) = v;
      }
    }
  }
}

__global__ void __launch_bounds__(256) wino_dy_kernel(const float* __restrict__ dy, int nb, int OH, int OW, int N, int ld_dy, int TH, int TW,
                                                      const float* __restrict__ gscale, float* __restrict__ dZ) {
  const int n4 = N >> 2;
  const long long T = (long long)nb * TH * TW, total = T * n4;
  for (unsigned i = blockIdx.x * blockDim.x + threadIdx.x; i < (unsigned)total; i += gridDim.x * blockDim.x) {
    const unsigned tile = i / (unsigned)n4;
    const int nq = (int)(i - tile * (unsigned)n4);
    const unsigned trow = tile / (unsigned)TW;
    const int tj = (int)(tile - trow * (unsigned)TW);
    const int img = (int)(trow / (unsigned)TH);
    const int ti = (int)(trow - (unsigned)img * (unsigned)TH);
    const float4 gs = gscale ? *reinterpret_cast<const float4*>(gscale + nq * 4) : make_float4(1.f, 1.f, 1.f, 1.f);
    float4 d[2][2];
#pragma unroll
    for (int a = 0; a < 2; ++a)
#pragma unroll
      for (int b = 0; b < 2; ++b) {
        const int oh = 2 * ti + a, ow = 2 * tj + b;
        float4 v = make_float4(0.f, 0.f, 0.f, 0.f);
        if (oh < OH && ow < OW) v = *reinterpret_cast<const float4*>(dy + (((long long)img * OH + oh) * OW + ow) * ld_dy + nq * 4);
        d[a][b] = make_float4(v.x * gs.x, v.y * gs.y, v.z * gs.z, v.w * gs.w);
      }
    float4 r[4][2];
#pragma unroll
    for (int b = 0; b < 2; ++b) {
      r[0][b] = d[0][b];
      r[1][b] = f4add(d[0][b], d[1][b]);
      r[2][b] = f4sub(d[0][b], d[1][b]);
      r[3][b] = f4sub(make_float4(0.f, 0.f, 0.f, 0.f), d[1][b]);
    }
    const long long ps = T * n4;
    float4* dst = reinterpret_cast<float4*>(dZ) + tile * n4 + nq;
#pragma unroll
    for (int a = 0; a < 4; ++a) {
      dst[(4 * a + 0) * ps] = r[a][0];
      dst[(4 * a + 1) * ps] = f4add(r[a][0], r[a][1]);
      dst[(4 * a + 2) * ps] = f4sub(r[a][0], r[a][1]);
      dst[(4 * a + 3) * ps] = f4sub(make_float4(0.f, 0.f, 0.f, 0.f), r[a][1]);
    }
  }
}

__global__ void __launch_bounds__(256) wino_filter_grad_kernel(const float* __restrict__ dU, int C, int N, int ldw, float* __restrict__ dw, int accumulate) {
  const int n4 = N >> 2;
  const long long total = (long long)C * n4;
  for (unsigned i = blockIdx.x * blockDim.x + threadIdx.x; i < (unsigned)total; i += gridDim.x * blockDim.x) {
    const int c = (int)(i / (unsigned)n4), nq = (int)(i - (unsigned)c * (unsigned)n4);
    const long long ps = (long long)C * n4;
    const float4* src = reinterpret_cast<const float4*>(dU) + (long long)c * n4 + nq;
    float4 u[4][4];
#pragma unroll
    for (int a = 0; a < 4; ++a)
#pragma unroll
      for (int b = 0; b < 4; ++b) u[a][b] = src[(4 * a + b) * ps];
    float4 t[3][4];
#pragma unroll
    for (int b = 0; b < 4; ++b) {
      const float4 hs = f4half(f4add(u[1][b], u[2][b])), hd = f4half(f4sub(u[1][b], u[2][b]));
      t[0][b] = f4add(u[0][b], hs);
      t[1][b] = hd;
      t[2][b] = f4add(hs, u[3][b]);
    }
#pragma unroll
    for (int a = 0; a < 3; ++a) {
      const float4 hs = f4half(f4add(t[a][1], t[a][2])), hd = f4half(f4sub(t[a][1], t[a][2]));
      const float4 g3[3] = {f4add(t[a][0], hs), hd, f4add(hs, t[a][3])};
#pragma unroll
      for (int b = 0; b < 3; ++b) {
        float4* p = reinterpret_cast<float4*>(dw + ((long long)(a * 3 + b) * C + c) * ldw + nq * 4);
        *p = accumulate ? f4add(*p, g3[b]) : g3[b];
      }
    }
  }
}

template <typename VT>
__global__ void __launch_bounds__(256) wino4_filter_kernel(const float* __restrict__ g, int C, int N, int ldw, float* __restrict__ U) {
  constexpr int W = sizeof(VT) / 4;
  const int nv = N / W;
  const long long total = (long long)C * nv, ps = total;
  for (unsigned i = blockIdx.x * blockDim.x + threadIdx.x; i < (unsigned)total; i += gridDim.x * blockDim.x) {
    const int c = (int)(i / (unsigned)nv), nq = (int)(i - (unsigned)c * (unsigned)nv);
    VT t[6][3];
#pragma unroll
    for (int b = 0; b < 3; ++b) {
      VT col[3], o[6];
#pragma unroll
      for (int a = 0; a < 3; ++a) col[a] = *reinterpret_cast<const VT*>(g + ((long long)(a * 3 + b) * C + c) * ldw + nq * W);
      g6(col, o);
#pragma unroll
      for (int a = 0; a < 6; ++a) t[a][b] = o[a];
    }
    VT* dst = reinterpret_cast<VT*>(U) + (long long)c * nv + nq;
#pragma unroll
    for (int a = 0; a < 6; ++a) {
      VT o[6];
      g6(t[a], o);
#pragma unroll
      for (int b = 0; b < 6; ++b) dst[(6 * a + b) * ps] = o[b];
    }
  }
}

template <typename VT>
__global__ void __launch_bounds__(256) wino4_input_kernel(const float* __restrict__ x, int nb, int H, int W_, int C, int TH, int TW,
                                                          float* __restrict__ V) {
  constexpr int W = sizeof(VT) / 4;
  const int cv = C / W;
  const long long T = (long long)nb * TH * TW, total = T * cv, ps = total;
  for (unsigned i = blockIdx.x * blockDim.x + threadIdx.x; i < (unsigned)total; i += gridDim.x * blockDim.x) {
    const unsigned tile = i / (unsigned)cv;
    const int cq = (int)(i - tile * (unsigned)cv);
    const unsigned trow = tile / (unsigned)TW;
    const int tj = (int)(tile - trow * (unsigned)TW);
    const int img = (int)(trow / (unsigned)TH);
    const int ti = (int)(trow - (unsigned)img * (unsigned)TH);
    VT t[6][6];
#pragma unroll
    for (int b = 0; b < 6; ++b) {
      const int iw = 4 * tj - 1 + b;
      VT col[6], o[6];
#pragma unroll
      for (int a = 0; a < 6; ++a) {
        const int ih = 4 * ti - 1 + a;
        col[a] = ((unsigned)ih < (unsigned)H && (unsigned)iw < (unsigned)W_)
                     ? *reinterpret_cast<const VT*>(x + (((long long)img * H + ih) * W_ + iw) * C + cq * W)
                     : vzero<VT>();
      }
      bt6(col, o);
#pragma unroll
      for (int a = 0; a < 6; ++a) t[a][b] = o[a];
    }
    VT* dst = reinterpret_cast<VT*>(V) + tile * cv + cq;
#pragma unroll
    for (int a = 0; a < 6; ++a) {
      VT o[6];
      bt6(t[a], o);
#pragma unroll
      for (int b = 0; b < 6; ++b) dst[(6 * a + b) * ps] = o[b];
    }
  }
}

template <typename VT>
__global__ void __launch_bounds__(256) wino4_output_kernel(const float* __restrict__ Mm, int nb, int OH, int OW, int N, int TH, int TW,
                                                           const float* __restrict__ scale, const float* __restrict__ shift, int act,
                                                           float* __restrict__ y, int ldy) {
  constexpr int W = sizeof(VT) / 4;
  const int nv = N / W;
  const long long T = (long long)nb * TH * TW, total = T * nv, ps = total;
  for (unsigned i = blockIdx.x * blockDim.x + threadIdx.x; i < (unsigned)total; i += gridDim.x * blockDim.x) {
    const unsigned tile = i / (unsigned)nv;
    const int nq = (int)(i - tile * (unsigned)nv);
    const unsigned trow = tile / (unsigned)TW;
    const int tj = (int)(tile - trow * (unsigned)TW);
    const int img = (int)(trow / (unsigned)TH);
    const int ti = (int)(trow - (unsigned)img * (unsigned)TH);
    const VT* src = reinterpret_cast<const VT*>(Mm) + tile * nv + nq;
    VT t[4][6];
#pragma unroll
    for (int b = 0; b < 6; ++b) {
      VT col[6], o[4];
#pragma unroll
      for (int a = 0; a < 6; ++a) col[a] = src[(6 * a + b) * ps];
      at6(col, o);
#pragma unroll
      for (int a = 0; a < 4; ++a) t[a][b] = o[a];
    }
    VT sc, sh = vzero<VT>();
    if (scale) sc = *reinterpret_cast<const VT*>(scale + nq * W);
    if (shift) sh = *reinterpret_cast<const VT*>(shift + nq * W);
#pragma unroll
    for (int a = 0; a < 4; ++a) {
      const int oh = 4 * ti + a;
      VT o[4];
      at6(t[a], o);
      if (oh >= OH) continue;
#pragma unroll
      for (int b = 0; b < 4; ++b) {
        const int ow = 4 * tj + b;
        if (ow >= OW) continue;
        VT v = scale ? o[b] * sc + sh : o[b] + sh;
        if (act == 1) v = vmax0(v);
        *reinterpret_cast<VT*>(y + (((long long)img * OH + oh) * OW + ow) * ldy + nq * W) = v;
      }
    }
  }
}

template <typename VT>
__global__ void __launch_bounds__(256) wino4_dy_kernel(const float* __restrict__ dy, int nb, int OH, int OW, int N, int ld_dy, int TH, int TW,
                                                       const float* __restrict__ gscale, float* __restrict__ dZ) {
  constexpr int W = sizeof(VT) / 4;
  const int nv = N / W;
  const long long T = (long long)nb * TH * TW, total = T * nv, ps = total;
  for (unsigned i = blockIdx.x * blockDim.x + threadIdx.x; i < (unsigned)total; i += gridDim.x * blockDim.x) {
    const unsigned tile = i / (unsigned)nv;
    const int nq = (int)(i - tile * (unsigned)nv);
    const unsigned trow = tile / (unsigned)TW;
    const int tj = (int)(tile - trow * (unsigned)TW);
    const int img = (int)(trow / (unsigned)TH);
    const int ti = (int)(trow - (unsigned)img * (unsigned)TH);
    VT gs;
    if (gscale) gs = *reinterpret_cast<const VT*>(gscale + nq * W);
    VT r[6][4];
#pragma unroll
    for (int b = 0; b < 4; ++b) {
      const int ow = 4 * tj + b;
      VT col[4], o[6];
#pragma unroll
      for (int a = 0; a < 4; ++a) {
        const int oh = 4 * ti + a;
        VT v = vzero<VT>();
        if (oh < OH && ow < OW) v = *reinterpret_cast<const VT*>(dy + (((long long)img * OH + oh) * OW + ow) * ld_dy + nq * W);
        col[a] = gscale ? v * gs : v;
      }
      a6(col, o);
#pragma unroll
      for (int a = 0; a < 6; ++a) r[a][b] = o[a];
    }
    VT* dst = reinterpret_cast<VT*>(dZ) + tile * nv + nq;
#pragma unroll
    for (int a = 0; a < 6; ++a) {
      VT o[6];
      a6(r[a], o);
#pragma unroll
      for (int b = 0; b < 6; ++b) dst[(6 * a + b) * ps] = o[b];
    }
  }
}

template <typename VT>
__global__ void __launch_bounds__(256) wino4_filter_grad_kernel(const float* __restrict__ dU, int C, int N, int ldw, float* __restrict__ dw, int accumulate) {
  constexpr int W = sizeof(VT) / 4;
  const int nv = N / W;
  const long long total = (long long)C * nv, ps = total;
  for (unsigned i = blockIdx.x * blockDim.x + threadIdx.x; i < (unsigned)total; i += gridDim.x * blockDim.x) {
    const int c = (int)(i / (unsigned)nv), nq = (int)(i - (unsigned)c * (unsigned)nv);
    const VT* src = reinterpret_cast<const VT*>(dU) + (long long)c * nv + nq;
    VT t[3][6];
#pragma unroll
    for (int b = 0; b < 6; ++b) {
      VT col[6], o[3];
#pragma unroll
      for (int a = 0; a < 6; ++a) col[a] = src[(6 * a + b) * ps];
      gt6(col, o);
#pragma unroll
      for (int a = 0; a < 3; ++a) t[a][b] = o[a];
    }
#pragma unroll
    for (int a = 0; a < 3; ++a) {
      VT o[3];
      gt6(t[a], o);
// ... 221 lines not shown
```

### rock-art-radnet_amd/radnet_hip/engine.py

```python
import collections
import ctypes as C
import contextlib
import os
import math

import numpy as np
import torch

from . import lib as L
from . import program as prog
from .bf16_images import Bf16Images
from .program import MIXED_PRECISIONS, PRECISIONS

BN_EPS = 1e-3
ADAM_BETA1, ADAM_BETA2, ADAM_EPS = 0.9, 0.999, 1e-7
RES_STAGES = ((2, "abc", (64, 64, 256), 1), (3, "abcd", (128, 128, 512), 2), (4, "abcdef", (256, 256, 1024), 2))
HEAD_STAGE = (5, "abc", (512, 512, 2048), 2)
RPN_LD = 64


def feat_len(n):
    n += 6
    for k in (7, 3, 1, 1):
        n = (n - k + 2) // 2
# ... 51 lines not shown
    d.out_boxes, d.out_probs, d.out_count, d.out_status, d.ws = ob.data_ptr(), op.data_ptr(), oc.data_ptr(), os_.data_ptr(), ws.data_ptr()
    ctx.check(ctx.lib.radnet_final_nms(ctx.h, C.byref(d)), "radnet_final_nms")
    ob, op, oc, os_ = ob.cpu().numpy(), op.cpu().numpy(), oc.cpu().numpy(), os_.cpu().numpy()
    out = []
    for g in range(ng):
        lo, k, st = int(offsets[g]), int(oc[g]), int(os_[g])
        out.append((st, None, None) if st < 0 else (0, ob[lo:lo + k].copy(), op[lo:lo + k].copy()))
    return out


def read_scan_records(words):
    words = words.numpy() if hasattr(words, "numpy") else np.asarray(words)
    m, status = int(words[0]), int(words[1])
    rec = words[L.DETECT_HEADER:L.DETECT_HEADER + L.DETECT_RECORD * m].reshape(m, L.DETECT_RECORD).copy()
    return status, rec[:, 0], rec[:, 1:5], rec[:, 5].view(np.float32)


class Arena:

    def __init__(self, device):
        self.device = device
        self.spec = []
        self.views = {}
        self.offsets = {}
        self.n = 0

    def add(self, name, shape):
        size = int(np.prod(shape))
        self.spec.append((name, tuple(shape)))
        self.offsets[name] = (self.n, size)
        self.n += _pad4(size)

    def finalize(self):
        self.n = (self.n + 255) // 256 * 256
        self.p = torch.zeros(self.n, dtype=torch.float32, device=self.device)
        self.g = torch.zeros_like(self.p)
        self.m = torch.zeros_like(self.p)
        self.v = torch.zeros_like(self.p)
        self.t = 0
        for name, shape in self.spec:
            o, s = self.offsets[name]
            self.views[name] = self.p[o:o + s].view(shape)
            self.views["d:" + name] = self.g[o:o + s].view(shape)

    def param(self, name):
        return self.views[name]

    def grad(self, name):
        return self.views["d:" + name]


class PlanCache(collections.OrderedDict):

    def __init__(self, limit, on_evict):
        super().__init__()
        self.limit, self.on_evict = limit, on_evict

    def __getitem__(self, key):
        v = super().__getitem__(key)
        self.move_to_end(key)
        return v

    def __setitem__(self, key, value):
        super().__setitem__(key, value)
        self.move_to_end(key)
        same = [k for k in self if k[0] == key[0]]
        while len(same) > self.limit:
            old = same.pop(0)
            value = collections.OrderedDict.__getitem__(self, old)
            collections.OrderedDict.__delitem__(self, old)
            self.on_evict(old, value)


class ConvLayer:

    def __init__(self, name, kh, cin, cout, stride=1, pad=0, ldw=None):
        self.name, self.kh, self.cin, self.cout, self.stride, self.pad = name, kh, cin, cout, stride, pad
        self.ldw = ldw or cout
        self.weight = None
        self.bias = None
        self.scale = None
        self.shift = None
        self.t0 = None
        self.dweight = None
        self.dbias = None
        self.wino_u = None
        self.wino_m = 2


class FasterRCNNEngine:

    NETWORK = "resnet50"
    N_FEATURES = 1024
    WORKLOAD = "train"
    supports_batched = True
    feat_len = staticmethod(feat_len)

    def __init__(self, C_cfg, device_index=0, n_classes=None, bce_mode=0, lr=5e-5, autotune=True, workload=None, precision="fp32"):
        if precision not in PRECISIONS:
            raise ValueError("precision must be 'fp32', 'bf16', 'bf16-mixed' or 'bf16-train', not %r" % (precision,))
        if precision != "fp32" and (self.NETWORK != "resnet50" or C_cfg.network != "resnet50"):
            raise NotImplementedError("precision=%r is implemented for the ResNet50 network only (not %r)" % (precision, C_cfg.network))
        if precision in MIXED_PRECISIONS and (workload or self.WORKLOAD) == "cont":
            raise NotImplementedError("precision='bf16-mixed' / 'bf16-train' is not implemented for the cont_train.py mode (its gradients flow through stages 3/4)")
        self.precision = precision
        self.bf16 = Bf16Images(self)
        self._inference_filters_stale = False
        self._head_shift_fresh = False
        self._chain_clamped = self._chain_warned = False
        self._head_slices = False
        self._count_pins = {}
        self.workload = workload or self.WORKLOAD
        self.TUNED_PREFIX = "%s_%s_" % (self.workload, self.NETWORK)
        if C_cfg.network != self.NETWORK:
            raise L.RadnetError("engine: %s asked to run network %r (use radnet_hip.make_engine)" % (type(self).__name__, C_cfg.network))
        self.C = C_cfg
        self.dev = torch.device("cuda", device_index)
        torch.cuda.set_device(self.dev)
        self.main_stream = torch.cuda.current_stream(self.dev)
        self.ctx = L.Context(device_index)
        self.lib = self.ctx.lib
        self.A = len(C_cfg.anchor_box_scales) * len(C_cfg.anchor_box_ratios)
        self.nc = n_classes or len(C_cfg.class_mapping)
        self.nreg = 4 * (self.nc - 1)
        self.bg = C_cfg.class_mapping.get("bg", self.nc - 1)
        self.bce_mode = bce_mode
        self.lr = lr
        if 5 * self.A > RPN_LD:
            raise L.RadnetError("engine: %d anchors exceed the fused RPN head width" % self.A)
        if self.nc + self.nreg > 64:
            raise L.RadnetError("engine: %d classes need %d dense-head columns, the fused dense-head kernel holds 64 (at most 13 classes)"
                                % (self.nc, self.nc + self.nreg))
        self.dense_ld = 32 if self.nc + self.nreg <= 32 else 64
        self._build_layers()
        self._plans = PlanCache(int(os.environ.get("RADNET_PLAN_CACHE", "32")), self._evict_plan)
        self._graphs = {}
        self._compiled = {}
        self.use_graphs = os.environ.get("RADNET_NO_GRAPHS", "0") != "1"
        self.fuse_tail = os.environ.get("RADNET_NO_TAIL_FUSION", "0") != "1"
        self.use_winograd = os.environ.get("RADNET_NO_WINOGRAD", "0") != "1"
        self.use_chain = os.environ.get("RADNET_CHAIN", "0") == "1"
        self.fwd_pair = os.environ.get("RADNET_NO_FWD_PAIR", "0") != "1"
        self.bneck_fuse = os.environ.get("RADNET_NO_BNECK_FUSE", "0") != "1"
        self.head_train_wino = (self.HEAD_TRAIN_WINOGRAD and self.use_winograd and os.environ.get("RADNET_NO_HEAD_TRAIN_WINOGRAD", "0") != "1"
                                and os.environ.get("RADNET_NO_INFERENCE_WINOGRAD", "0") != "1")
        self._adam_wino = None
        self.chain_wgs = int(os.environ.get("RADNET_CHAIN_WGS", "256"))
        if precision != "fp32":
            self.use_chain = self.fwd_pair = self.bneck_fuse = self.head_train_wino = False
        self._chain_plans = []
        self.wino_wgrad = os.environ.get("RADNET_NO_WINOGRAD_WGRAD", "0") != "1"
        self.head_wino_wgrad = self.head_train_wino and self.wino_wgrad and os.environ.get("RADNET_NO_HEAD_WINO_WGRAD", "0") != "1"
        self.head_deferred_wgrad = (self.HEAD_DEFERRED_WGRAD and precision == "fp32" and os.environ.get("RADNET_HEAD_DEFERRED_WGRAD", "1") != "0")
        self.ws = torch.empty(256 << 20, dtype=torch.uint8, device=self.dev)
        self.ctx.check(self.lib.radnet_set_workspace(self.ctx.h, self.ws.data_ptr(), self.ws.numel()), "set_workspace")
        self.autotune_mode = int(os.environ.get("RADNET_AUTOTUNE", int(autotune))) if autotune else 0
        self.ctx.check(self.lib.radnet_set_autotune(self.ctx.h, self.autotune_mode), "set_autotune")
        self.use_copy_stream = os.environ.get("RADNET_COPY_STREAM", "0") == "1"
        self.copy_stream = torch.cuda.Stream(device=self.dev) if self.use_copy_stream else None
        self.side_stream = torch.cuda.Stream(device=self.dev)
        self.ctx2 = L.Context(device_index, stream_handle=self.side_stream.cuda_stream)
        self.ctx2.check(self.lib.radnet_set_autotune(self.ctx2.h, self.autotune_mode), "set_autotune")
        self.ws2 = torch.empty(256 << 20, dtype=torch.uint8, device=self.dev)
        self.ctx2.check(self.lib.radnet_set_workspace(self.ctx2.h, self.ws2.data_ptr(), self.ws2.numel()), "set_workspace")
        self.head_stream = torch.cuda.Stream(device=self.dev)
        self.ctx3 = L.Context(device_index, stream_handle=self.head_stream.cuda_stream)
        self.ctx3.check(self.lib.radnet_set_autotune(self.ctx3.h, self.autotune_mode), "set_autotune")
        self.ws3 = torch.empty(256 << 20, dtype=torch.uint8, device=self.dev)
        self.ctx3.check(self.lib.radnet_set_workspace(self.ctx3.h, self.ws3.data_ptr(), self.ws3.numel()), "set_workspace")
        self._lanes = {"side": (self.ctx2, self.side_stream), "head": (self.ctx3, self.head_stream)}
        self.n_side_lanes = max(1, int(os.environ.get("RADNET_SIDE_LANES", "2")))
        self._extra_lanes = []
        for k in range(1, self.n_side_lanes):
            st = torch.cuda.Stream(device=self.dev)
            cx = L.Context(device_index, stream_handle=st.cuda_stream)
            cx.check(self.lib.radnet_set_autotune(cx.h, self.autotune_mode), "set_autotune")
            ws = torch.empty(256 << 20, dtype=torch.uint8, device=self.dev)
            cx.check(self.lib.radnet_set_workspace(cx.h, ws.data_ptr(), ws.numel()), "set_workspace")
            self._extra_lanes.append((st, cx, ws))
            self._lanes["side%d" % k] = (cx, st)
        if os.environ.get("RADNET_FORCE_CONFIG"):
            fa, fb, fs = (int(v) for v in os.environ["RADNET_FORCE_CONFIG"].split(","))
            for c in [self.ctx, self.ctx2, self.ctx3] + [e[1] for e in self._extra_lanes]:
                c.check(self.lib.radnet_force_config(c.h, fa, fb, fs), "force_config")
        for c in [self.ctx2, self.ctx3] + [e[1] for e in self._extra_lanes]:
            self.ctx.check(self.lib.radnet_share_tuning(c.h, self.ctx.h), "share_tuning")
        self.shipped_tuning = []
        tuned_dir = os.path.join(os.path.dirname(os.path.abspath(__file__)), "tuned")
        if self.autotune_mode and os.environ.get("RADNET_SHIPPED_TUNING", "1") != "0" and os.path.isdir(tuned_dir):
            for name in sorted(os.listdir(tuned_dir)):
                if name.endswith(".txt") and name.startswith(self.TUNED_PREFIX):
                    self.load_tuning(os.path.join(tuned_dir, name))
                    self.shipped_tuning.append(name)
        self.anchor_wh = np.array([[(s * r[0]) / C_cfg.rpn_stride, (s * r[1]) / C_cfg.rpn_stride]
                                   for s in C_cfg.anchor_box_scales for r in C_cfg.anchor_box_ratios], dtype=np.float64)
        self.anchor_sizes = np.array(C_cfg.anchor_box_scales, dtype=np.float64)
        self.anchor_ratios = np.array(C_cfg.anchor_box_ratios, dtype=np.float64).reshape(-1, 2)
        self.regr_std = np.array(C_cfg.classifier_regr_std, dtype=np.float64)
        self.loss_scratch = torch.zeros(8, dtype=torch.float64, device=self.dev)
        self.rpn_losses = torch.zeros(2, dtype=torch.float32, device=self.dev)
        self.det_losses = torch.zeros(3, dtype=torch.float32, device=self.dev)

    def _build_layers(self):
        dev = self.dev
        self.base_layers = []
        self.convs = {}
        frozen_elems = 0

        def conv(name, kh, cin, cout, stride=1, pad=0, ldw=None):
            c = ConvLayer(name, kh, cin, cout, stride, pad, ldw)
            self.convs[name] = c
            return c

        conv("conv1", 7, 4, 64, 2, 3)
        cin = 64
        for st, blocks, (f1, f2, f3), stride in RES_STAGES + (HEAD_STAGE,):
            if st == 5:
                cin = 1024
            for bl in blocks:
                b = "res%d%s_branch" % (st, bl)
                first = bl == "a"
                conv(b + "2a", 1, cin, f1, stride if first else 1)
                conv(b + "2b", 3, f1, f2, 1, 1)
                conv(b + "2c", 1, f2, f3)
                if first:
                    conv(b + "1", 1, cin, f3, stride)
                cin = f3
        conv("rpn_conv1", 3, 1024, 512, 1, 1)
        conv("rpn_heads", 1, 512, 5 * self.A, 1, 0, ldw=RPN_LD)

        for name, c in self.convs.items():
            if name.startswith(("res5", "rpn")):
                continue
            c.weight = torch.zeros(c.kh * c.kh * c.cin, c.ldw, dtype=torch.float32, device=dev)
            c.scale = torch.ones(c.cout, dtype=torch.float32, device=dev)
            c.shift = torch.zeros(c.cout, dtype=torch.float32, device=dev)

        self.rpn_arena = Arena(dev)
        for name in ("rpn_conv1", "rpn_heads"):
            c = self.convs[name]
            self.rpn_arena.add(name + "/kernel", (c.kh * c.kh * c.cin, c.ldw))
            self.rpn_arena.add(name + "/bias", (c.ldw,))
        self.rpn_arena.finalize()
        for name in ("rpn_conv1", "rpn_heads"):
            c = self.convs[name]
            c.weight, c.bias = self.rpn_arena.param(name + "/kernel"), self.rpn_arena.param(name + "/bias")
            c.dweight, c.dbias = self.rpn_arena.grad(name + "/kernel"), self.rpn_arena.grad(name + "/bias")
            c.shift = c.bias

        self.head_arena = Arena(dev)
        head_names = [n for n in self.convs if n.startswith("res5")]
        self.head_conv_names = head_names
        for name in head_names:
            c = self.convs[name]
            self.head_arena.add(name + "/kernel", (c.kh * c.kh * c.cin, c.cout))
        self.head_bias_off = self.head_arena.n
        for name in head_names:
            self.head_arena.add(name + "/bias", (self.convs[name].cout,))
        self.head_bias_len = self.head_arena.n - self.head_bias_off
        self.head_arena.add("dense/kernel", (2048, self.dense_ld))
        self.head_arena.add("dense/bias", (self.dense_ld,))
        self.head_arena.finalize()
        self.head_scale = torch.ones(self.head_bias_len, dtype=torch.float32, device=dev)
        self.head_t0 = torch.zeros(self.head_bias_len, dtype=torch.float32, device=dev)
        self.head_shift = torch.zeros(self.head_bias_len, dtype=torch.float32, device=dev)
        for name in head_names:
            c = self.convs[name]
            c.weight, c.bias = self.head_arena.param(name + "/kernel"), self.head_arena.param(name + "/bias")
            c.dweight, c.dbias = self.head_arena.grad(name + "/kernel"), self.head_arena.grad(name + "/bias")
            o = self.head_arena.offsets[name + "/bias"][0] - self.head_bias_off
            c.scale = self.head_scale[o:o + c.cout]
            c.t0 = self.head_t0[o:o + c.cout]
            c.shift = self.head_shift[o:o + c.cout]
        self.dense_w, self.dense_b = self.head_arena.param("dense/kernel"), self.head_arena.param("dense/bias")
        self.dense_dw, self.dense_db = self.head_arena.grad("dense/kernel"), self.head_arena.grad("dense/bias")

    def sync_inference_filters(self):
        if self._inference_filters_stale:
            self._inference_filters_stale = False
            self.bf16.refresh()
            self._refresh_winograd([n for n in self.INFERENCE_WINOGRAD_LAYERS if getattr(self.convs.get(n), "wino_u", None) is not None])

    def refresh_head_shift(self, force=False):
        fresh, self._head_shift_fresh = self._head_shift_fresh, False
        if fresh and not force:
            return
        bias = self.head_arena.p[self.head_bias_off:self.head_bias_off + self.head_bias_len]
        self.ctx.call("radnet_affine_vec", self.head_shift, self.head_scale, bias, self.head_t0, C.c_int64(self.head_bias_len))

    def set_weights(self, W):
        dev = self.dev

        def t(a):
            return torch.from_numpy(np.ascontiguousarray(a, dtype=np.float32)).to(dev)

        def bn_name(conv_name):
            if conv_name == "conv1":
                return "bn_conv1"
            return conv_name.replace("res", "bn", 1)

        for name, c in self.convs.items():
            if name == "rpn_heads":
                kc, kr = W["rpn_out_class"], W["rpn_out_regress"]
                k = np.zeros((512, RPN_LD), np.float32)
                k[:, :self.A] = kc["kernel"].reshape(512, self.A)
                k[:, self.A:5 * self.A] = kr["kernel"].reshape(512, 4 * self.A)
# ... 687 lines not shown
                sc = cur
            if first and self.fwd_pair:
                fwd += [("conv_pair_first", da), ("conv_pair_second", ds)]
            else:
                fwd.append(("conv", da))
            bb = buf(R, oh, ow, f2)
            n_keep = len(keep)
            op_b, db = self._fwd_op(cb, a, R, oh, ow, bb, keep, relu=True, inference=not training)
            fwd.append(op_b)
            wino_v = keep[n_keep] if (training and op_b[0] == "wino" and self.head_wino_wgrad and R >= self.HEAD_WINO_WGRAD_MIN_ROIS) else None
            if first and not self.fwd_pair:
                fwd.append(("conv", ds))
            out = buf(R, oh, ow, f3); dc, _, _ = self._desc(cc, bb, R, oh, ow, out, relu=True, addend=sc); fwd.append(("conv", dc))
            blocks.append(dict(first=first, x=cur, a=a, b=bb, out=out, da=da, db=db, dc=dc, ds=ds, names=(b + "2a", b + "2b", b + "2c", b + "1"), wino_v=wino_v))
            cur, h, w = out, oh, ow
        M = R * h * w
        feat = buf(R, 2048)
        pcls, pregr = buf(R, self.nc), buf(R, self.nreg)
        y1, y2 = buf(R, self.nc), buf(R, 2 * self.nreg)
        tail_scratch = torch.zeros(int(self.lib.radnet_head_tail_scratch_bytes(R)), dtype=torch.uint8, device=dev)
        keep.append(tail_scratch)
        fwd = self._forward_program(fwd)
        if not training:
            plan = dict(R=R, rois=rois, pooled=pooled, fwd=fwd, blocks=blocks, y5=cur, hw=h * w, M=M, feat=feat, pcls=pcls, pregr=pregr,
                        F=F, fh=fh, fw=fw, keep=keep, groups=groups, tail_scratch=tail_scratch)
            self._plans[key] = plan
            return plan
        dz = buf(R, self.nc + self.nreg)
        dfeat = buf(R, 2048)
        bwd = []
        shared_wg = {}
        bwd_parts = []
        g_out = buf(M, f3)
        g_first = g_out
        for bi in range(len(blocks) - 1, -1, -1):
            B = blocks[bi]
            part_from = len(bwd)
            ca, cb, cc = (self.convs[n] for n in B["names"][:3])
            g_b, g_a = buf(M, f2), buf(M, f1)

            def bias_grad(g, n, conv):
                return prog.colsum(g=g.data_ptr(), m=M, n=n, ld=n, gscale=conv.scale.data_ptr(), out=conv.dbias.data_ptr(), accumulate=1)

            def bdesc(fdesc, conv, dy, ld_dy, dx=None, ld_dx=0, dx_add=None, dx_mask=None):
                d = L.ConvDesc.from_buffer_copy(fdesc)
                d.dy, d.ld_dy, d.gscale = dy.data_ptr(), ld_dy, conv.scale.data_ptr()
                d.dw, d.dw_accumulate = conv.dweight.data_ptr(), 1
                if dx is not None:
                    d.dx, d.ld_dx = dx.data_ptr(), ld_dx
                    d.dx_add = dx_add.data_ptr() if dx_add is not None else None
                    d.ld_dx_add = ld_dx
                    d.dx_mask = dx_mask.data_ptr() if dx_mask is not None else None
                    d.ld_dx_mask = ld_dx
                return d

            B["g_out"], B["g_a"], B["g_b"] = g_out, g_a, g_b
            dC = bdesc(B["dc"], cc, g_out, f3, g_b, f2, None, B["b"])
            bwd += [("wgrad", dC), bias_grad(g_out, f3, cc), ("dgrad", dC)]
            dB = bdesc(B["db"], cb, g_b, f2, g_a, f1, None, B["a"])
            wg_b = self._wino_wgrad_op(cb, B.get("wino_v"), g_b, f2, R, B["db"].oh, B["db"].ow, shared_wg) if B.get("wino_v") is not None else None
            bwd += [wg_b or ("wgrad", dB), bias_grad(g_b, f2, cb), ("dgrad", dB)]
            if B["first"]:
                dA = bdesc(B["da"], ca, g_a, f1)
                bwd += [("wgrad", dA), bias_grad(g_a, f1, ca)]
                cs = self.convs[B["names"][3]]
                dS = bdesc(B["ds"], cs, g_out, f3)
                bwd += [("wgrad", dS), bias_grad(g_out, f3, cs)]
            else:
                g_prev = buf(M, f3)
                dA = bdesc(B["da"], ca, g_a, f1, g_prev, f3, g_out, B["x"])
                bwd += [("wgrad", dA), bias_grad(g_a, f1, ca), ("dgrad", dA)]
                g_out = g_prev
            k0 = self.head_arena.offsets[B["names"][0] + "/kernel"][0]
            kl, sl = self.head_arena.offsets[B["names"][3 if B["first"] else 2] + "/kernel"]
            bwd_parts.append((self._backward_program(bwd[part_from:]), (k0, kl + _pad4(sl))))
        bwd = [op for part, _ in bwd_parts for op in part]
        cover = sorted(sl for _, sl in bwd_parts)
        if cover[0][0] != 0 or cover[-1][1] != self.head_bias_off or any(a[1] != b[0] for a, b in zip(cover, cover[1:])):
            raise RuntimeError("head gradient buckets do not tile the kernel part of the arena: %r" % (cover,))
        if [sl for _, sl in bwd_parts] != self.head_exchange_slices():
            raise RuntimeError("head backward parts and head_exchange_slices() disagree")
        live = torch.ones(groups, dtype=torch.int32, device=dev)
        keep.append(live)
        plan = dict(R=R, rois=rois, pooled=pooled, fwd=fwd, bwd=bwd, bwd_parts=bwd_parts, blocks=blocks, y5=cur, hw=h * w, M=M, feat=feat, pcls=pcls,
                    tail_scratch=tail_scratch, live=live, live_host=[1] * groups, wg_scratch=shared_wg,
                    pregr=pregr, y1=y1, y2=y2, dz=dz, dfeat=dfeat, g_last=g_first, F=F, fh=fh, fw=fw, keep=keep, groups=groups)
        form = prog.deferred_wgrad_form(bwd) if self.head_deferred_wgrad else None
        if form is not None and len(form[1]) == len(self.head_conv_names):
            plan["bwd_dgrad"], plan["bwd_wgrad"] = form
        self._plans[key] = plan
        return plan

    def head_exchange_slices(self):
        if self._head_slices is False:
            self._head_slices = None
            names = self.head_conv_names
            blocks = []
            for n in names:
                b = n.split("_")[0]
                if not blocks or blocks[-1][0] != b:
                    blocks.append([b, n, n])
                blocks[-1][2] = n
            if blocks and all(n.startswith("res5") for n in names):
                sl = []
                for _, first, last in blocks:
                    o0 = self.head_arena.offsets[first + "/kernel"][0]
                    ol, szl = self.head_arena.offsets[last + "/kernel"]
                    sl.append((o0, ol + _pad4(szl)))
                self._head_slices = sl[::-1]
        return self._head_slices

    def head_crop(self, hp):
        G = hp.get("groups", 1)
        if G == 1:
            self.ctx.call("radnet_roi_resize_fwd", hp["F"], hp["fh"], hp["fw"], 1024, hp["rois"], hp["R"], 14, hp["pooled"])
        else:
            rg = hp["R"] // G
            for g in range(G):
                self.ctx.call("radnet_roi_resize_fwd", hp["F"][g], hp["fh"], hp["fw"], 1024, hp["rois"][g * rg:], rg, 14, hp["pooled"][g * rg:])

    def head_forward(self, hp, training=False, loss_out=None, group_live=None, cropped=False):
        G = hp.get("groups", 1)
        if "live" not in hp:
            self.sync_inference_filters()
        if not cropped:
            self.head_crop(hp)
        self._run(hp["fwd"])
        hp["_tail_fused"] = False
        if self.fuse_tail:
            fused_loss = training and loss_out is not None and "live" in hp
            if fused_loss:
                flags = [1] * G if group_live is None else [1 if f else 0 for f in group_live]
                if flags != hp["live_host"]:
                    hp["live"].copy_(torch.tensor(flags, dtype=torch.int32), non_blocking=False)
                    hp["live_host"] = flags
            self.ctx.call("radnet_head_tail_fwd", hp["y5"], hp["R"], hp["hw"], 2048, self.dense_w, self.dense_ld, self.dense_b, self.nc, self.nreg,
                          hp["feat"], hp["pcls"], hp["pregr"], hp["y1"] if fused_loss else None, hp["y2"] if fused_loss else None,
                          hp["dz"] if fused_loss else None, loss_out if fused_loss else None, G, hp["live"] if fused_loss else None,
                          hp["tail_scratch"])
            hp["_tail_fused"] = fused_loss
            return
        self.ctx.call("radnet_avgpool_fwd", hp["y5"], hp["R"], hp["hw"], 2048, hp["feat"])
        self.ctx.call("radnet_dense_heads_fwd", hp["feat"], hp["R"], 2048, self.dense_w, self.dense_ld, self.dense_b, self.nc, self.nreg,
                      hp["pcls"], hp["pregr"])

    def head_deferred_ok(self, hp):
        return (self.head_deferred_wgrad and "bwd_wgrad" in hp and self.head_bias_len > 0 and self.head_bias_off % 4 == 0 and self.head_bias_len % 4 == 0
                and int(self.lib.radnet_get_deterministic(self.ctx.h)) == 1 and all(d.dw_accumulate != 1 for d in hp["bwd_wgrad"]))

    def head_update_deferred(self, hp, grad_scale=1.0):
        arena = self.head_arena
        arena.t += 1
        modes = tuple(d.dw_accumulate for d in hp["bwd_wgrad"])
        ent = hp.get("_wgrad_arr")
        if ent is None or ent[0] != modes:
            ent = hp["_wgrad_arr"] = (modes, prog.desc_array(hp["bwd_wgrad"]))
        opt = L.WgradAdam()
        opt.p, opt.g, opt.m, opt.v, opt.n, opt.t = arena.p.data_ptr(), arena.g.data_ptr(), arena.m.data_ptr(), arena.v.data_ptr(), arena.n, arena.t
        opt.lr, opt.beta1, opt.beta2, opt.eps, opt.grad_scale = self.lr, ADAM_BETA1, ADAM_BETA2, ADAM_EPS, grad_scale
        self.ctx.check(self.lib.radnet_conv_wgrad_multi(self.ctx.h, ent[1], len(modes), C.byref(opt)), "radnet_conv_wgrad_multi")
        off = self.head_bias_off
        wino = self._head_adam_wino() if self.head_train_wino else None
        if wino is not None:
            self.ctx.call("radnet_adam_step_tail", arena.p, arena.g, arena.m, arena.v, C.c_int64(arena.n), arena.t, C.c_float(self.lr),
                          C.c_float(ADAM_BETA1), C.c_float(ADAM_BETA2), C.c_float(ADAM_EPS), C.c_float(grad_scale), 1, C.c_int64(off),
                          C.c_int64(self.head_bias_len), self.head_scale, self.head_t0, self.head_shift, wino[0], wino[1], C.c_int64(off))
            return
        self.ctx.call("radnet_adam_step_affine", arena.p[off:], arena.g[off:], arena.m[off:], arena.v[off:], C.c_int64(arena.n - off), arena.t,
                      C.c_float(self.lr), C.c_float(ADAM_BETA1), C.c_float(ADAM_BETA2), C.c_float(ADAM_EPS), C.c_float(grad_scale), 1,
                      C.c_int64(0), C.c_int64(self.head_bias_len), self.head_scale, self.head_t0, self.head_shift)
        if self.head_train_wino:
            self._refresh_winograd(list(self.INFERENCE_WINOGRAD_LAYERS))
        else:
            self._inference_filters_stale = True

    def head_backward(self, hp, accumulate=False, loss_out=None, on_part=None, defer_wgrad=False):
        G = hp.get("groups", 1)
        if hp.get("_tail_fused"):
            pass
        elif G == 1:
            self.ctx.call("radnet_det_loss", hp["pcls"], hp["pregr"], hp["y1"], hp["y2"], hp["R"], self.nc, self.nreg, hp["dz"],
                          self.det_losses if loss_out is None else loss_out)
        else:
            rg = hp["R"] // G
            for g in range(G):
                lo = loss_out[g] if loss_out is not None else self.det_losses
                if lo is None:
                    self.ctx.call("radnet_fill_zero", hp["dz"][g * rg:], C.c_uint64(rg * (self.nc + self.nreg) * 4))
                    continue
                self.ctx.call("radnet_det_loss", hp["pcls"][g * rg:], hp["pregr"][g * rg:], hp["y1"][g * rg:], hp["y2"][g * rg:], rg, self.nc,
                              self.nreg, hp["dz"][g * rg:], lo)
        self.ctx.call("radnet_dense_heads_bwd", hp["feat"], hp["dz"], hp["R"], 2048, self.dense_w, self.dense_ld, self.nc + self.nreg,
                      self.dense_dw, self.dense_db, hp["dfeat"], 1 if accumulate else 0)
        self.ctx.call("radnet_avgpool_bwd_relu", hp["dfeat"], hp["y5"], hp["R"], hp["hw"], 2048, hp["g_last"])
        if defer_wgrad:
            self._run(hp["bwd_dgrad"])
            return
        if on_part is None or "bwd_parts" not in hp:
            self._run(hp["bwd"])
            return
        for part, (lo, hi) in hp["bwd_parts"]:
            self._run(part)
            on_part(lo, hi)

    def upload_gt(self, gt_boxes, gt_is_bg, gt_cls):
        g = len(gt_boxes)
        dev = self.dev
        return dict(g=g,
                    boxes=torch.from_numpy(np.ascontiguousarray(gt_boxes, dtype=np.float64).reshape(-1, 4)).to(dev) if g else None,
                    isbg=torch.from_numpy(np.ascontiguousarray(gt_is_bg, dtype=np.int32)).to(dev) if g else None,
                    cls=torch.from_numpy(np.ascontiguousarray(gt_cls, dtype=np.int32)).to(dev) if g else None)

    def anchor_targets_launch(self, gt, width, height, rw, rh, slot=0):
        fw, fh = self.feat_len(rw), self.feat_len(rh)
        A = self.A
        key = ("atgt", fh, fw, slot)
        if key not in self._plans:
            dev = self.dev
            self._plans[key] = dict(valid=torch.zeros(A, fh, fw, dtype=torch.uint8, device=dev), overlap=torch.zeros(A, fh, fw, dtype=torch.uint8, device=dev),
                                    regr=torch.zeros(fh, fw, 4 * A, dtype=torch.float64, device=dev),
                                    ycls=torch.zeros(fh, fw, 2 * A, dtype=torch.float32, device=dev),
                                    yregr=torch.zeros(fh, fw, 8 * A, dtype=torch.float32, device=dev),
                                    h_valid=torch.zeros(A, fh, fw, dtype=torch.uint8).pin_memory(), h_overlap=torch.zeros(A, fh, fw, dtype=torch.uint8).pin_memory(),
                                    best=torch.zeros(1024, 4, dtype=torch.int32, device=dev), nfor=torch.zeros(1024, dtype=torch.int32, device=dev),
                                    scratch=torch.zeros(1024, dtype=torch.int64, device=dev), event=torch.cuda.Event(), fw=fw, fh=fh)
        P = self._plans[key]
        g = gt["g"]
        rc = self.lib.radnet_anchor_targets(self.ctx.h, gt["boxes"].data_ptr() if g else None, gt["isbg"].data_ptr() if g else None, g, int(width), int(height),
                                            int(rw), int(rh), fw, fh, self.anchor_sizes.ctypes.data_as(C.POINTER(C.c_double)), len(self.anchor_sizes),
                                            self.anchor_ratios.ctypes.data_as(C.POINTER(C.c_double)), len(self.anchor_ratios), float(self.C.rpn_stride),
                                            float(self.C.rpn_max_overlap), P["valid"].data_ptr(), P["overlap"].data_ptr(), P["regr"].data_ptr(),
                                            P["best"].data_ptr(), P["nfor"].data_ptr(), P["scratch"].data_ptr())
        self.ctx.check(rc, "radnet_anchor_targets")
        self._copy(P["h_valid"], P["valid"])
        self._copy(P["h_overlap"], P["overlap"])
        P["event"].record()
        P["g"] = g
        return P

    def anchor_targets_finish(self, P):
        P["event"].synchronize()
        valid = P["h_valid"].numpy()
        n_pos = subsample_valid(valid, P["h_overlap"].numpy())
        self._copy(P["valid"], P["h_valid"])
        self.ctx.call("radnet_anchor_targets_pack", P["valid"], P["overlap"], P["regr"], P["fw"], P["fh"], self.A, C.c_double(float(self.C.std_scaling)),
                      P["ycls"], P["yregr"])
        return P["ycls"], P["yregr"], n_pos

    def anchor_targets(self, gt_boxes, gt_is_bg, width, height, rw, rh, slot=0):
        gt = self.upload_gt(gt_boxes, gt_is_bg, np.zeros(len(gt_boxes), np.int32))
        P = self.anchor_targets_launch(gt, width, height, rw, rh, slot)
        ycls, yregr, n_pos = self.anchor_targets_finish(P)
        g = gt["g"]
        best_h = P["best"][:g].cpu().numpy().astype(np.int64) if g else np.zeros((0, 4), np.int64)
        return ycls, yregr, best_h, n_pos

    def roi_targets(self, R_dev, n_dev, gt, width, height, rw, rh, n_max=300):
        return self.roi_targets_finish(self.roi_targets_launch(R_dev, n_dev, gt, width, height, rw, rh, n_max))

    def roi_targets_launch(self, R_dev, n_dev, gt, width, height, rw, rh, n_max=300, slot=0):
        dev = self.dev
        key = ("rtgt", slot)
        if key not in self._plans:
            self._plans[key] = dict(keep=torch.zeros(1024, dtype=torch.uint8, device=dev), cls=torch.zeros(1024, dtype=torch.int32, device=dev),
                                    box=torch.zeros(1024, 4, dtype=torch.int32, device=dev), t=torch.zeros(1024, 4, dtype=torch.float64, device=dev),
                                    iou=torch.zeros(1024, dtype=torch.float64, device=dev), h_cls=torch.zeros(1024, dtype=torch.int32).pin_memory(),
                                    h_n=torch.zeros(1, dtype=torch.int32).pin_memory(), sel=torch.zeros(1024, dtype=torch.int32, device=dev),
                                    h_sel=torch.zeros(1024, dtype=torch.int32).pin_memory())
        P = self._plans[key]
        rc = self.lib.radnet_roi_targets(self.ctx.h, R_dev.data_ptr(), int(n_max), gt["boxes"].data_ptr() if gt["g"] else None,
                                         gt["cls"].data_ptr() if gt["g"] else None, gt["g"], int(width), int(height), int(rw), int(rh),
                                         float(self.C.rpn_stride), float(self.C.classifier_min_overlap), float(self.C.classifier_max_overlap),
                                         self.regr_std.ctypes.data_as(C.POINTER(C.c_double)), int(self.bg), P["keep"].data_ptr(), P["cls"].data_ptr(),
                                         P["box"].data_ptr(), P["t"].data_ptr(), P["iou"].data_ptr(), n_dev.data_ptr())
        self.ctx.check(rc, "radnet_roi_targets")
        self._copy(P["h_cls"][:n_max], P["cls"][:n_max])
        self._copy(P["h_n"], n_dev)
        if "event" not in P:
            P["event"] = torch.cuda.Event()
        P["event"].record()
        return P

    def roi_targets_finish(self, P):
        P["event"].synchronize()
        if self._chain_plans:
            self.check_chains()
        n = int(P["h_n"][0])
        return P, P["h_cls"].numpy()[:max(n, 0)], n

    def pack_roi_batch(self, P, sel, hp, group=0):
        k = len(sel)
        o = group * (hp["R"] // hp.get("groups", 1))
        P["h_sel"][:k] = torch.from_numpy(np.ascontiguousarray(sel, dtype=np.int32))
        if self.KERNEL_COPIES and os.environ.get("RADNET_NO_PINNED_SEL", "0") != "1":
            self.ctx.call("radnet_roi_batch_pack", P["h_sel"], k, P["cls"], P["box"], P["t"], self.nc, int(self.bg), hp["rois"][o:], hp["y1"][o:], hp["y2"][o:])
            return
        self._copy(P["sel"][:k], P["h_sel"][:k])
        self.ctx.call("radnet_roi_batch_pack", P["sel"], k, P["cls"], P["box"], P["t"], self.nc, int(self.bg), hp["rois"][o:], hp["y1"][o:], hp["y2"][o:])

    def idle_roi_group(self, hp, group):
        rg = hp["R"] // hp["groups"]
        hp["rois"][group * rg:(group + 1) * rg].copy_(torch.tensor([0.0, 0.0, 1.0, 1.0], device=self.dev).expand(rg, 4))


def _uniform_table_probs(chan_of_item, neg_chans, n_total):
    counts = np.bincount(neg_chans, minlength=int(chan_of_item.max()) + 1 if len(chan_of_item) else 1)
    if (counts == 0).any():
        bad = counts[chan_of_item] == 0
        if bad.any():
            raise KeyError(int(chan_of_item[np.argmax(bad)]))
    per_chan = np.zeros(counts.shape[0], dtype=np.float64)
    nz = counts > 0
    per_chan[nz] = (counts[nz] / n_total) / counts[nz]
    return per_chan[chan_of_item]


def choice_without_replacement(n, size, p):
    lib = L.load_library()
    p = np.array(p, dtype=np.float64, copy=True)
    if p.ndim != 1 or p.shape[0] != n:
        raise ValueError("'a' and 'p' must have same size")
    if size > n:
        raise ValueError("Cannot take a larger sample than population when 'replace=False'")
    if np.count_nonzero(p > 0) < size:
        raise ValueError("Fewer non-zero entries in p than size")
    found = np.zeros(size + 1, dtype=np.int64)
    live_idx = np.flatnonzero(p > 0).astype(np.int64)
# ... 55 lines not shown
```

### rock-art-radnet_amd/radnet_hip/lib.py

```python
import ctypes as C
import os
import re

_HERE = os.path.dirname(os.path.abspath(__file__))
LIB_PATH = os.environ.get("RADNET_HIP_LIBRARY", os.path.join(_HERE, "libradnet_hip.so"))
HEADER_PATH = os.path.abspath(os.path.join(_HERE, "..", "..", "include", "radnet_hip.h"))

c_float_p = C.c_void_p
_lib = None


class RadnetError(RuntimeError):
    pass


class ConvDesc(C.Structure):
    _fields_ = [
        ("x", C.c_void_p), ("w", C.c_void_p), ("y", C.c_void_p),
        ("scale", C.c_void_p), ("shift", C.c_void_p), ("addend", C.c_void_p),
        ("nb", C.c_int32), ("h", C.c_int32), ("w_", C.c_int32), ("c", C.c_int32),
        ("oh", C.c_int32), ("ow", C.c_int32),
        ("kh", C.c_int32), ("kw", C.c_int32), ("stride", C.c_int32), ("pad_t", C.c_int32), ("pad_l", C.c_int32),
        ("n", C.c_int32),
        ("ldw", C.c_int32), ("ldy", C.c_int32), ("ld_add", C.c_int32),
# ... 57 lines not shown


class ScanMergeDesc(C.Structure):
    _fields_ = [("pool", C.c_void_p), ("pool_words", C.c_int64), ("slot_rows", C.c_int32),
                ("tiles_host", C.c_void_p), ("tiles_dev", C.c_void_p),
                ("n_tiles", C.c_int32), ("nc", C.c_int32),
                ("obj_avg_threshold", C.c_double), ("obj_confidence_threshold", C.c_float), ("n_obj_avg", C.c_int32),
                ("nms_thresh", C.c_double), ("max_boxes", C.c_int32),
                ("out", C.c_void_p), ("ws", C.c_void_p)]


AUG_BRIGHTNESS, AUG_CONTRAST, AUG_SALT_PEPPER, AUG_GAUSSIAN, AUG_POISSON = range(5)


class AdamDesc(C.Structure):
    _fields_ = [("p", C.c_void_p), ("g", C.c_void_p), ("m", C.c_void_p), ("v", C.c_void_p), ("n", C.c_int64), ("t", C.c_int32), ("lr", C.c_float)]


SUBSAMPLE_FN = C.CFUNCTYPE(C.c_int32, C.c_void_p, C.POINTER(C.c_uint8), C.POINTER(C.c_uint8), C.c_int32, C.c_int32, C.c_int32)
SELECT_FN = C.CFUNCTYPE(C.c_int32, C.c_void_p, C.POINTER(C.c_int32), C.c_int32, C.POINTER(C.c_int32), C.c_int32)


class HostHooks(C.Structure):
    _fields_ = [("user", C.c_void_p), ("subsample_anchors", SUBSAMPLE_FN), ("select_rois", SELECT_FN)]


class AdamWino(C.Structure):
    _fields_ = [("off", C.c_int64), ("c", C.c_int32), ("n", C.c_int32), ("u", C.c_void_p)]


class WgradAdam(C.Structure):
    _fields_ = [("p", C.c_void_p), ("g", C.c_void_p), ("m", C.c_void_p), ("v", C.c_void_p), ("n", C.c_int64), ("t", C.c_int32),
                ("lr", C.c_float), ("beta1", C.c_float), ("beta2", C.c_float), ("eps", C.c_float), ("grad_scale", C.c_float)]


class AdamBf16(C.Structure):
    _fields_ = [("off", C.c_int64), ("k", C.c_int32), ("n", C.c_int32), ("ldw", C.c_int32), ("wt", C.c_void_p), ("ldk", C.c_int32)]


class Bf16DgradImage(C.Structure):
    _fields_ = [("off", C.c_int64), ("taps", C.c_int32), ("c", C.c_int32), ("n", C.c_int32), ("ldw", C.c_int32), ("wd", C.c_void_p), ("ldkd", C.c_int32)]


class TrainDesc(C.Structure):
    _d, _i, _vp = C.c_double, C.c_int32, C.c_void_p
    _fields_ = [("img_u8", _vp), ("h", _i), ("w", _i), ("x", _vp),
                ("gt", _vp), ("gt_is_bg", _vp), ("gt_cls", _vp), ("g", _i), ("width", _i), ("height", _i),
                ("anchor_sizes_host", C.POINTER(_d)), ("ns", _i), ("anchor_ratios_host", C.POINTER(_d)), ("nr", _i),
                ("rpn_stride", _d), ("rpn_max_overlap", _d), ("std_scaling", _d),
                ("valid", _vp), ("overlap", _vp), ("regr", _vp), ("best_anchor", _vp), ("n_for_gt", _vp), ("at_scratch", _vp),
                ("h_valid", _vp), ("h_overlap", _vp), ("y_cls", _vp), ("y_regr", _vp),
                ("base_ops", C.POINTER(Op)), ("n_base", _i),
                ("rpn_fwd_ops", C.POINTER(Op)), ("n_rpn_fwd", _i),
                ("rpn_bwd_ops", C.POINTER(Op)), ("n_rpn_bwd", _i),
                ("rpn_refwd_ops", C.POINTER(Op)), ("n_rpn_refwd", _i),
                ("pred", _vp), ("dz", _vp), ("ld_pred", _i), ("fh", _i), ("fw", _i), ("a", _i), ("bce_mode", _i), ("loss_scratch8", _vp), ("rpn_losses", _vp),
                ("rpn_opt", AdamDesc), ("head_opt", AdamDesc), ("world", _i),
                ("wino_w", _vp), ("wino_c", _i), ("wino_n", _i), ("wino_ldw", _i), ("wino_form", _i), ("wino_u", _vp),
                ("anchor_wh_host", C.POINTER(_d)), ("overlap_thresh", _d), ("max_boxes", _i),
                ("R", _vp), ("Rp", _vp), ("Rn", _vp), ("prop_ws", _vp),
                ("rw", _i), ("rh", _i), ("min_overlap", _d), ("max_overlap", _d), ("regr_std_host4", C.POINTER(_d)), ("bg_class", _i),
                ("keep", _vp), ("roi_cls", _vp), ("roi_box", _vp), ("roi_t", _vp), ("roi_iou", _vp),
                ("h_roi_cls", _vp), ("h_n", _vp), ("sel", _vp), ("h_sel", _vp),
                ("head", C.POINTER(HeadDesc)), ("y1", _vp), ("y2", _vp),
                ("head_dz", _vp), ("det_losses", _vp), ("dense_dw", _vp), ("dense_db", _vp), ("dfeat", _vp), ("g_last", _vp),
                ("head_bwd_ops", C.POINTER(Op)), ("n_head_bwd", _i),
                ("head_shift", _vp), ("head_scale", _vp), ("head_bias", _vp), ("head_t0", _vp), ("head_bias_len", C.c_int64),
                ("tail_scratch", _vp), ("head_wino", _vp), ("n_head_wino", C.c_int32)]


def declared_symbols():
    with open(HEADER_PATH) as f:
        text = f.read()
    text = re.sub(r"/\*.*?\*/", "", text, flags=re.S)
    return sorted(set(re.findall(r"\b(radnet_[a-z0-9_]+)\s*\(", text)))


def header_constant(name):
    with open(HEADER_PATH) as f:
        m = re.search(r"^#define\s+%s\s+(-?\d+)\s*$" % re.escape(name), f.read(), flags=re.M)
    if m is None:
        raise RadnetError("include/radnet_hip.h does not define %s" % name)
    return int(m.group(1))


DETECT_HEADER, DETECT_RECORD = header_constant("RADNET_DETECT_HEADER_WORDS"), header_constant("RADNET_DETECT_RECORD_WORDS")


def load_library():
    global _lib
    if _lib is not None:
        return _lib
    import torch
    if not os.path.exists(LIB_PATH):
        raise RadnetError("libradnet_hip.so not built: run `python -c 'import __graft_entry__ as g; g.build()'` "
                          "(or `make -C rock-art-radnet_amd/csrc`). There is no CPU fallback.")
    lib = C.CDLL(LIB_PATH)
    i32, i64, u64, f32, f64, vp = C.c_int32, C.c_int64, C.c_uint64, C.c_float, C.c_double, C.c_void_p
    sig = {
        "radnet_create": (C.c_int, [C.c_int, vp, C.POINTER(vp)]),
        "radnet_destroy": (None, [vp]),
        "radnet_last_error": (C.c_char_p, [vp]),
        "radnet_sync": (C.c_int, [vp]),
        "radnet_set_stream": (C.c_int, [vp, vp]),
        "radnet_version": (C.c_int, []),
        "radnet_set_workspace": (C.c_int, [vp, vp, u64]),
        "radnet_set_autotune": (C.c_int, [vp, C.c_int]),
        "radnet_tuned_shapes": (C.c_int, [vp]),
        "radnet_tune_save": (C.c_int, [vp, C.c_char_p]),
        "radnet_share_tuning": (C.c_int, [vp, vp]),
        "radnet_tune_load": (C.c_int, [vp, C.c_char_p]),
        "radnet_force_config": (C.c_int, [vp, C.c_int, C.c_int, C.c_int]),
        "radnet_force_waves": (C.c_int, [vp, C.c_int]),
        "radnet_set_deterministic": (C.c_int, [vp, C.c_int]),
        "radnet_get_deterministic": (C.c_int, [vp]),
        "radnet_timing_enable": (C.c_int, [vp, C.c_int]),
        "radnet_timing_read": (C.c_int, [vp, C.c_int, C.POINTER(f64), C.POINTER(i64), C.POINTER(f64)]),
        "radnet_timing_reset": (C.c_int, [vp]),
        "radnet_conv_fwd": (C.c_int, [vp, C.POINTER(ConvDesc)]),
        "radnet_conv_fwd_bf16": (C.c_int, [vp, C.POINTER(ConvDesc), vp, i32]),
        "radnet_conv_fwd_bf16_split": (C.c_int, [vp, C.POINTER(ConvDesc), vp, i32, i32]),
        "radnet_conv_bf16_pick_split": (i32, [C.c_int64, i32, i32]),
        "radnet_conv_bf16_tile_shape": (i64, [i64, i32, C.POINTER(i32), C.POINTER(i32)]),
        "radnet_weights_to_bf16": (C.c_int, [vp, vp, i32, i32, i32, vp, i32]),
        "radnet_weights_to_bf16_dgrad": (C.c_int, [vp, vp, i32, i32, i32, i32, vp, i32]),
        "radnet_weights_to_bf16_dgrad_arena": (C.c_int, [vp, vp, i64, C.POINTER(Bf16DgradImage), i32]),
        "radnet_conv_dgrad_bf16": (C.c_int, [vp, C.POINTER(ConvDesc), vp, i32]),
        "radnet_conv_dgrad_bf16_split": (C.c_int, [vp, C.POINTER(ConvDesc), vp, i32, i32]),
        "radnet_conv_wgrad_bf16": (C.c_int, [vp, C.POINTER(ConvDesc), i32]),
        "radnet_dgrad_bf16_pick_split": (i32, [C.c_int64, i32, i32]),
        "radnet_wgrad_bf16_pick_split": (i32, [C.c_int64, i32, i32]),
        "radnet_conv_dgrad": (C.c_int, [vp, C.POINTER(ConvDesc)]),
        "radnet_gemm_batched": (C.c_int, [vp, vp, vp, vp, i32, i32, i32, i32]),
        "radnet_winograd_filter": (C.c_int, [vp, vp, i32, i32, i32, vp]),
        "radnet_winograd_input": (C.c_int, [vp, vp, i32, i32, i32, i32, vp]),
        "radnet_winograd_output": (C.c_int, [vp, vp, i32, i32, i32, i32, vp, vp, i32, vp, i32]),
        "radnet_winograd_dy": (C.c_int, [vp, vp, i32, i32, i32, i32, i32, vp, vp]),
        "radnet_wgrad_batched": (C.c_int, [vp, vp, vp, vp, i32, i32, i32, i32, i32]),
        "radnet_winograd_filter_grad": (C.c_int, [vp, vp, i32, i32, i32, vp, i32]),
        "radnet_winograd4_filter": (C.c_int, [vp, vp, i32, i32, i32, vp]),
        "radnet_winograd4_input": (C.c_int, [vp, vp, i32, i32, i32, i32, vp]),
        "radnet_winograd4_output": (C.c_int, [vp, vp, i32, i32, i32, i32, vp, vp, i32, vp, i32]),
        "radnet_winograd4_dy": (C.c_int, [vp, vp, i32, i32, i32, i32, i32, vp, vp]),
        "radnet_winograd4_filter_grad": (C.c_int, [vp, vp, i32, i32, i32, vp, i32]),
        "radnet_adam_step_fused": (C.c_int, [vp, vp, vp, vp, vp, C.c_int64, i32, C.c_float, C.c_float, C.c_float, C.c_float, C.c_float, i32,
                                            C.c_int64, C.c_int64, vp, vp, vp, C.POINTER(AdamWino), i32]),
        "radnet_adam_step_tail": (C.c_int, [vp, vp, vp, vp, vp, C.c_int64, i32, C.c_float, C.c_float, C.c_float, C.c_float, C.c_float, i32,
                                           C.c_int64, C.c_int64, vp, vp, vp, C.POINTER(AdamWino), i32, C.c_int64]),
        "radnet_adam_step_bf16": (C.c_int, [vp, vp, vp, vp, vp, C.c_int64, i32, C.c_float, C.c_float, C.c_float, C.c_float, C.c_float, i32,
                                           C.c_int64, C.c_int64, vp, vp, vp, C.POINTER(AdamBf16), i32]),
        "radnet_conv_wgrad": (C.c_int, [vp, C.POINTER(ConvDesc)]),
        "radnet_conv_bwd": (C.c_int, [vp, C.POINTER(ConvDesc)]),
        "radnet_conv_wgrad_multi": (C.c_int, [vp, C.POINTER(ConvDesc), i32, C.POINTER(WgradAdam)]),
        "radnet_conv_fwd_pair": (C.c_int, [vp, C.POINTER(ConvDesc), C.POINTER(ConvDesc)]),
        "radnet_conv_bottleneck": (C.c_int, [vp, C.POINTER(ConvDesc), C.POINTER(ConvDesc), C.POINTER(ConvDesc)]),
        "radnet_colsum": (C.c_int, [vp, vp, i32, i32, i32, vp, vp, i32]),
        "radnet_maxpool_fwd": (C.c_int, [vp, vp, vp, i32, i32, i32, i32, i32, i32]),
        "radnet_roi_resize_fwd": (C.c_int, [vp, vp, i32, i32, i32, vp, i32, i32, vp]),
        "radnet_roi_resize_bwd": (C.c_int, [vp, vp, i32, i32, i32, vp, i32, i32, vp]),
        "radnet_avgpool_fwd": (C.c_int, [vp, vp, i32, i32, i32, vp]),
        "radnet_avgpool_bwd_relu": (C.c_int, [vp, vp, vp, i32, i32, i32, vp]),
        "radnet_dense_heads_fwd": (C.c_int, [vp, vp, i32, i32, vp, i32, vp, i32, i32, vp, vp]),
        "radnet_dense_heads_bwd": (C.c_int, [vp, vp, vp, i32, i32, vp, i32, i32, vp, vp, vp, i32]),
        "radnet_head_tail_scratch_bytes": (u64, [i32]),
        "radnet_head_tail_fwd": (C.c_int, [vp, vp, i32, i32, i32, vp, i32, vp, i32, i32, vp, vp, vp, vp, vp, vp, vp, i32, vp, vp]),
        "radnet_rpn_loss": (C.c_int, [vp, vp, i32, vp, vp, i32, i32, i32, vp, i32, vp, vp]),
        "radnet_det_loss": (C.c_int, [vp, vp, vp, vp, vp, i32, i32, i32, vp, vp]),
        "radnet_adam_step": (C.c_int, [vp, vp, vp, vp, vp, i64, i32, f32, f32, f32, f32, f32, i32]),
        "radnet_adam_step_affine": (C.c_int, [vp, vp, vp, vp, vp, i64, i32, f32, f32, f32, f32, f32, i32, i64, i64, vp, vp, vp]),
        "radnet_affine_vec": (C.c_int, [vp, vp, vp, vp, vp, i64]),
        "radnet_relu_mask": (C.c_int, [vp, vp, vp, i64]),
        "radnet_scatter_strided": (C.c_int, [vp, vp, i32, i32, i32, i32, i32, i32, i32, vp, vp]),
        "radnet_proposals_ws_bytes": (u64, [i64]),
        "radnet_rpn_to_roi": (C.c_int, [vp, vp, i32, i32, i32, i32, C.POINTER(f64), f64, i32, f64, i32, vp, vp, vp, vp]),
        "radnet_nms": (C.c_int, [vp, vp, vp, i32, f64, i32, vp, vp, vp]),
        "radnet_anchor_targets": (C.c_int, [vp, vp, vp, i32, i32, i32, i32, i32, i32, i32, C.POINTER(f64), i32, C.POINTER(f64), i32,
                                            f64, f64, vp, vp, vp, vp, vp, vp]),
        "radnet_anchor_targets_pack": (C.c_int, [vp, vp, vp, vp, i32, i32, i32, f64, vp, vp]),
        "radnet_roi_targets": (C.c_int, [vp, vp, i32, vp, vp, i32, i32, i32, i32, i32, f64, f64, f64, C.POINTER(f64), i32,
                                         vp, vp, vp, vp, vp, vp]),
        "radnet_roi_batch_pack": (C.c_int, [vp, vp, i32, vp, vp, vp, i32, i32, vp, vp, vp]),
        "radnet_host_choice_round": (i64, [vp, vp, vp, vp, i64, vp, i64, vp, vp]),
        "radnet_preprocess_bgr": (C.c_int, [vp, vp, i32, i32, i32, vp]),
        "radnet_resize_bicubic_u8": (C.c_int, [vp, vp, i32, i32, vp, i32, i32, i32]),
        "radnet_resize_bicubic_window_u8": (C.c_int, [vp, vp, i32, i32, i32, i32, i32, i32, vp, i32, i32, i32]),
        "radnet_warp_affine_u8": (C.c_int, [vp, vp, i32, i32, i32, vp, i32, i32, vp, vp]),
        "radnet_aug_gather_u8": (C.c_int, [vp, vp, i32, i32, i32, i32, i32, i32, i32, vp]),
        "radnet_aug_extent_u8": (C.c_int, [vp, vp, i32, i32, vp]),
        "radnet_aug_histogram_u8": (C.c_int, [vp, vp, i32, i32, i32, vp]),
        "radnet_aug_pointwise_u8": (C.c_int, [vp, vp, vp, i32, i32, i32, i32, f64, f64, u64, C.c_uint32]),
        "radnet_png_unfilter_u8": (C.c_int, [vp, vp, i32, i32, i32]),
        "radnet_png_plan_segments": (C.c_int, [vp, i64, i32, i32, i32, vp, i32]),
        "radnet_png_unfilter_segments_u8": (C.c_int, [vp, vp, i64, vp, vp, i32, i32]),
        "radnet_png_expand_bgr_u8": (C.c_int, [vp, vp, i32, i32, i32, i32, i32, vp, vp, i32, i32, i32, i32, i32, i32]),
        "radnet_png_filter_rows_u8": (C.c_int, [vp, vp, i32, i32, i32, i64, i32, vp]),
        "radnet_deflate_rle_scan_u8": (C.c_int, [vp, vp, i64, vp, vp]),
        "radnet_deflate_rle_emit_u8": (C.c_int, [vp, vp, i64, vp, vp, i32, i32, vp, i64, vp]),
        "radnet_deflate_piece_cap": (i64, [vp, i32, i32]),
        "radnet_deflate_pack": (C.c_int, [vp, vp, i64, vp, i32, vp, i64, vp]),
        "radnet_deflate_build_code": (C.c_int, [vp, vp, vp, i32, C.POINTER(i32)]),
        "radnet_png_check_crcs": (C.c_int, [vp, i64, vp, vp, i32, i32]),
        "radnet_inflate_find_blocks": (C.c_int, [vp, vp, i64, i64, vp, i32, vp]),
        "radnet_inflate_rle_measure": (C.c_int, [vp, vp, i64, vp, i32]),
        "radnet_inflate_chain": (C.c_int, [vp, i32, i64, i64, i64, vp, i32, C.POINTER(i32), C.POINTER(i32), C.POINTER(i32)]),
        "radnet_inflate_rle_emit": (C.c_int, [vp, vp, i64, vp, i32, vp, i64]),
        "radnet_inflate_lz_measure": (C.c_int, [vp, vp, i64, vp, i32]),
        "radnet_inflate_lz_chain": (C.c_int, [vp, i32, i64, i64, i64, vp, i32, C.POINTER(i32), C.POINTER(i32), C.POINTER(i32)]),
        "radnet_inflate_lz_emit": (C.c_int, [vp, vp, i64, vp, i32, vp, vp, i64]),
        "radnet_inflate_lz_resolve": (C.c_int, [vp, vp, i64, i32, vp]),
        "radnet_inflate_lz_gather": (C.c_int, [vp, vp, vp, i64]),
        "radnet_png_gather_column_u8": (C.c_int, [vp, vp, i64, vp, vp, vp, i32, vp]),
        "radnet_png_plan_segments_column": (C.c_int, [vp, i64, i32, i32, i32, vp, i32]),
        "radnet_png_plan_tiles": (C.c_int, [i32, i32, i32, vp]),
        "radnet_png_tiles_on_sweep": (C.c_int, [i32, i32, i32, i32, vp, i32]),
        "radnet_png_unfilter_tiles_u8": (C.c_int, [vp, vp, i64, vp, vp, i32, i32]),
        "radnet_png_unfilter_tiles_width_u8": (C.c_int, [vp, vp, i64, vp, vp, i32, i32, i32]),
        "radnet_draw_rects_u8": (C.c_int, [vp, vp, i32, i32, i64, vp, vp, i32]),
        "radnet_draw_list_u8": (C.c_int, [vp, vp, i32, i32, i64, vp, vp, i32, vp, vp, i32]),
        "radnet_draw_glyph_rows": (C.c_int, [i32, vp]),
        "radnet_draw_scene_u8": (C.c_int, [vp, vp, i32, i32, i64, vp, vp, i32, vp, vp, i32]),
        "radnet_draw_scene_check": (C.c_int, [vp, i32, vp, i32, C.POINTER(i32), C.c_char_p, i32]),
        "radnet_grey3_u8": (C.c_int, [vp, vp, vp, i32, i32, i64, i64]),
        "radnet_score_levels_u8": (C.c_int, [vp, vp, i32, i32, i32, i32, vp]),
        "radnet_heat_paint_u8": (C.c_int, [vp, vp, i32, i32, i64, vp, i64, vp, vp, i32, vp, i32, i32]),
        "radnet_heat_check": (C.c_int, [vp, i32, i64, i32, i32, C.POINTER(i32), C.c_char_p, i32]),
        "radnet_fill_zero": (C.c_int, [vp, vp, u64]),
        "radnet_copy_bytes": (C.c_int, [vp, vp, vp, C.c_uint64]),
        "radnet_program_run": (C.c_int, [vp, C.POINTER(Op), i32]),
        "radnet_rpn_forward": (C.c_int, [vp, C.POINTER(Op), i32, C.POINTER(Op), i32]),
        "radnet_predict_tile": (C.c_int, [vp, C.POINTER(TileDesc)]),
        "radnet_detect_tail_out_bytes": (u64, [i32]),
        "radnet_detect_tail": (C.c_int, [vp, C.POINTER(DetectTailDesc)]),
        "radnet_rois_from_proposals": (C.c_int, [vp, vp, vp, i32, i32, i32, vp]),
        "radnet_predict_tile_detect": (C.c_int, [vp, C.POINTER(TileDesc), C.POINTER(DetectTailDesc)]),
        "radnet_final_nms_ws_bytes": (u64, [i32, i32]),
        "radnet_final_nms": (C.c_int, [vp, C.POINTER(FinalNmsDesc)]),
        "radnet_scan_merge_out_bytes": (u64, [i32, i32]),
        "radnet_scan_merge_ws_bytes": (u64, [i32, i32, i32, i32, i32]),
        "radnet_scan_merge": (C.c_int, [vp, C.POINTER(ScanMergeDesc)]),
        "radnet_scan_merge_check": (C.c_int, [vp, i32, i64, i32, C.POINTER(i32), C.POINTER(i32), C.c_char_p, i32]),
        "radnet_train_step": (C.c_int, [vp, C.POINTER(TrainDesc), C.POINTER(HostHooks), C.POINTER(C.c_float), C.POINTER(i32)]),
        "radnet_comm_unique_id": (C.c_int, [C.c_char_p]),
        "radnet_comm_init": (C.c_int, [vp, i32, i32, C.c_char_p]),
        "radnet_comm_destroy": (C.c_int, [vp]),
        "radnet_allreduce_grads": (C.c_int, [vp, vp, i64]),
        "radnet_comm_stats": (C.c_int, [vp, C.POINTER(C.c_int64), C.POINTER(C.c_int64)]),
        "radnet_chain_build": (C.c_int, [vp, vp, i32, i32, C.POINTER(vp)]),
        "radnet_chain_run": (C.c_int, [vp, vp]),
        "radnet_chain_error": (C.c_uint32, [vp]),
        "radnet_chain_status": (C.c_int, [vp, vp, C.POINTER(i32), C.POINTER(i32), C.POINTER(i32), C.POINTER(i32), C.POINTER(f64), C.POINTER(f64)]),
        "radnet_chain_destroy": (None, [vp]),
        "radnet_chain_peek": (C.c_int, [vp, i32, C.POINTER(C.c_uint32), i32]),
        "radnet_chain_check": (C.c_int, [vp, i32, C.POINTER(i32), C.POINTER(i32), C.POINTER(i32), C.POINTER(i32), C.POINTER(i32), C.c_char_p, i32]),
        "radnet_scale": (C.c_int, [vp, vp, i64, f32]),
    }
    for name, (res, args) in sig.items():
        fn = getattr(lib, name)
        fn.restype = res
        fn.argtypes = args
    _lib = lib
    return lib


def glyph_rows(code):
    rows = (C.c_uint8 * 8)()
    rc = load_library().radnet_draw_glyph_rows(int(code), rows)
    if rc != 0:
        raise RadnetError("radnet_draw_glyph_rows: no glyph for the code 0x%02X (the font has 0x20..0x7E)" % int(code))
    return bytes(rows)


def draw_scene_check(table, chars=b"", count=None, n_chars=None):
    import numpy as np
    rows = np.zeros((0, 8), np.int32) if table is None else np.ascontiguousarray(table).view(np.int32).reshape(-1, 8)
    pool = np.frombuffer(bytes(chars or b""), np.uint8)
    bad, msg = C.c_int32(-2), C.create_string_buffer(256)
    rc = load_library().radnet_draw_scene_check(rows.ctypes.data if len(rows) else None, len(rows) if count is None else int(count),
                                                pool.ctypes.data if len(pool) else None, len(pool) if n_chars is None else int(n_chars),
                                                C.byref(bad), msg, len(msg))
    return rc, bad.value, msg.value.decode()


def heat_check(table, pool_len, h, w, count=None):
    import numpy as np
    rows = np.zeros((0, 32), np.uint8) if table is None else np.ascontiguousarray(table).view(np.uint8).reshape(-1, 32)
    bad, msg = C.c_int32(-2), C.create_string_buffer(256)
    rc = load_library().radnet_heat_check(rows.ctypes.data if len(rows) else None, len(rows) if count is None else int(count), int(pool_len), int(h),
                                          int(w), C.byref(bad), msg, len(msg))
    return rc, bad.value, msg.value.decode()


def scan_merge_check(table, pool_words, slot_rows, count=None):
    import numpy as np
    rows = np.zeros((0, 16), np.uint8) if table is None else np.ascontiguousarray(table).view(np.uint8).reshape(-1, 16)
    n_images, bad, msg = C.c_int32(-2), C.c_int32(-2), C.create_string_buffer(256)
    rc = load_library().radnet_scan_merge_check(rows.ctypes.data if len(rows) else None, len(rows) if count is None else int(count), int(pool_words),
                                                int(slot_rows), C.byref(n_images), C.byref(bad), msg, len(msg))
    return rc, n_images.value, bad.value, msg.value.decode()


def _ptr(t):
    if t is None:
        return None
    if isinstance(t, int):
        return t
    return t.data_ptr()
# ... 60 lines not shown
```

Baseline: 604.2 images/sec.

## Fuse Winograd filter transform into head weight-gradient Adam epilogue

```diff
diff --git a/include/radnet_hip.h b/include/radnet_hip.h
--- a/include/radnet_hip.h
+++ b/include/radnet_hip.h
@@ -87,6 +87,9 @@
   float lr, beta1, beta2, eps, grad_scale;
 } radnet_wgrad_adam;
 int radnet_conv_wgrad_multi(radnet_ctx* ctx, const radnet_conv_desc* descs, int32_t n, const radnet_wgrad_adam* opt);
+struct radnet_adam_wino;
+int radnet_conv_wgrad_multi_filters(radnet_ctx* ctx, const radnet_conv_desc* descs, int32_t n, const radnet_wgrad_adam* opt,
+                                    const struct radnet_adam_wino* layers, int32_t n_layers);
 int radnet_conv_fwd_pair(radnet_ctx* ctx, const radnet_conv_desc* d1, const radnet_conv_desc* d2);
 int radnet_conv_bottleneck(radnet_ctx* ctx, const radnet_conv_desc* db, const radnet_conv_desc* dc, const radnet_conv_desc* da);
 
diff --git a/rock-art-radnet_amd/csrc/adam.hip b/rock-art-radnet_amd/csrc/adam.hip
--- a/rock-art-radnet_amd/csrc/adam.hip
+++ b/rock-art-radnet_amd/csrc/adam.hip
@@ -83,24 +83,8 @@
   }
   __syncthreads();
   if (threadIdx.x < 64) {
-    float4 t[6][3];
-#pragma unroll
-    for (int bb = 0; bb < 3; ++bb) {
-      float4 col[3], o[6];
-#pragma unroll
-      for (int aa = 0; aa < 3; ++aa) col[aa] = taps[aa * 3 + bb][threadIdx.x];
-      g6(col, o);
-#pragma unroll
-      for (int aa = 0; aa < 6; ++aa) t[aa][bb] = o[aa];
-    }
     float4* dst = reinterpret_cast<float4*>(wz.u[layer]) + j0 + threadIdx.x;
-#pragma unroll
-    for (int aa = 0; aa < 6; ++aa) {
-      float4 o[6];
-      g6(t[aa], o);
-#pragma unroll
-      for (int bb = 0; bb < 6; ++bb) dst[(long long)(6 * aa + bb) * cn4] = o[bb];
-    }
+    wino4_filter_chunk([&](int tap) { return taps[tap][threadIdx.x]; }, [&](int p, const float4& o) { dst[(long long)p * cn4] = o; });
   }
 }
 
diff --git a/rock-art-radnet_amd/csrc/conv_args.h b/rock-art-radnet_amd/csrc/conv_args.h
--- a/rock-art-radnet_amd/csrc/conv_args.h
+++ b/rock-art-radnet_amd/csrc/conv_args.h
@@ -70,6 +70,8 @@
   float* ov;
   float lr_t, beta1, beta2, eps, grad_scale;
   int pad_opt;
+  float* ou;
+  unsigned* tap_counters;
 };
 
 constexpr int kWgradMultiMax = 16;
@@ -110,6 +112,6 @@
 
 constexpr int kCtrStride = 16;
 
-static_assert(sizeof(GemmArgs) == 264 && sizeof(TailArgs) == 120 && sizeof(WgradArgs) == 248 && sizeof(PairMap) == 24, "kernel argument layout");
+static_assert(sizeof(GemmArgs) == 264 && sizeof(TailArgs) == 120 && sizeof(WgradArgs) == 264 && sizeof(PairMap) == 24, "kernel argument layout");
 static_assert(sizeof(WgradMultiMap) == 200 && sizeof(WgradOptScalars) == 20, "multi-problem weight-gradient launch layout");
 static_assert(sizeof(ChainStage) == 336 && sizeof(ChainItem) == 48 && sizeof(ChainHeader) == 32, "chain list layout");
diff --git a/rock-art-radnet_amd/csrc/conv_device.h b/rock-art-radnet_amd/csrc/conv_device.h
--- a/rock-art-radnet_amd/csrc/conv_device.h
+++ b/rock-art-radnet_amd/csrc/conv_device.h
@@ -55,6 +55,11 @@
   typedef unsigned u32x4 __attribute__((ext_vector_type(4)));
   f32x4 f = {v.x, v.y, v.z, v.w};
   __builtin_amdgcn_raw_buffer_store_b128(__builtin_bit_cast(u32x4, f), r, (int)off, 0, 16);
+}
+__device__ __forceinline__ void buf_store4(__amdgpu_buffer_rsrc_t r, unsigned off, float4 v) {
+  typedef unsigned u32x4 __attribute__((ext_vector_type(4)));
+  f32x4 f = {v.x, v.y, v.z, v.w};
+  __builtin_amdgcn_raw_buffer_store_b128(__builtin_bit_cast(u32x4, f), r, (int)off, 0, 0);
 }
 __device__ __forceinline__ void buf_store1_sc1(__amdgpu_buffer_rsrc_t r, unsigned off, float v) {
   __builtin_amdgcn_raw_buffer_store_b32(__builtin_bit_cast(unsigned, v), r, (int)off, 0, 16);
diff --git a/rock-art-radnet_amd/csrc/conv_wgrad.hip b/rock-art-radnet_amd/csrc/conv_wgrad.hip
--- a/rock-art-radnet_amd/csrc/conv_wgrad.hip
+++ b/rock-art-radnet_amd/csrc/conv_wgrad.hip
@@ -304,14 +304,49 @@
 }
 }
 
-extern "C" int radnet_conv_wgrad_multi(radnet_ctx* ctx, const radnet_conv_desc* descs, int32_t n, const radnet_wgrad_adam* opt) {
+static int wgrad_multi_impl(radnet_ctx* ctx, const radnet_conv_desc* descs, int32_t n, const radnet_wgrad_adam* opt, const radnet_adam_wino* layers,
+                            int32_t n_layers) {
   if (!ctx || n < 0 || (n > 0 && !descs)) return RADNET_ERR_ARG;
-  if (n == 0) return RADNET_OK;
+  if (n_layers < 0 || (n_layers > 0 && !layers)) RADNET_FAIL(ctx, RADNET_ERR_ARG, "conv_wgrad_multi_filters: %d layers without a table", n_layers);
+  if (n == 0 && n_layers == 0) return RADNET_OK;
   if (ctx->pair_capture != nullptr) RADNET_FAIL(ctx, RADNET_ERR_ARG, "conv_wgrad_multi: called inside radnet_conv_bwd");
   const bool adam = opt != nullptr && opt->p != nullptr;
   if (adam) {
     if (!opt->g || !opt->m || !opt->v || opt->n <= 0) RADNET_FAIL(ctx, RADNET_ERR_ARG, "conv_wgrad_multi: optimizer block with a null arena");
     if (opt->t < 1) RADNET_FAIL(ctx, RADNET_ERR_ARG, "conv_wgrad_multi: step counter starts at 1");
+  }
+  std::vector<int> layer_of((size_t)n, -1);
+  auto filter_problem = [&](int i, int bmk, int bn, unsigned slices, bool ordered) {
+    const radnet_conv_desc& d = descs[i];
+    return WgradFilterProblem{d.kh, d.kw, d.c, d.n, d.ldw, bmk, bn, slices, ordered ? 1 : 0, adam ? 1 : 0,
+                              adam ? (uint64_t)(uintptr_t)(opt->p + (d.dw - opt->g)) : 0, (uint64_t)(uintptr_t)layers[layer_of[(size_t)i]].u};
+  };
+  auto filter_refused = [&](int i, int code) {
+    const char* why = code == kWgradFilterErrTaps ? "the layer is not 3x3"
+                    : code == kWgradFilterErrChannels ? "its channels are no multiple of the k tile"
+                    : code == kWgradFilterErrPitch ? "its kernel is not dense (ldw == n, n a multiple of 4)"
+                    : code == kWgradFilterErrAlign ? "u must be 16-byte aligned and the kernel must own its 128-byte lines"
+                    : code == kWgradFilterErrOptimizer ? "the call has no optimizer block"
+                    : code == kWgradFilterErrOrder ? "a split problem needs ordered reductions"
+                    : code == kWgradFilterErrSize ? "u is 2 GiB or larger" : "malformed";
+    RADNET_FAIL(ctx, RADNET_ERR_UNSUPPORTED, "conv_wgrad_multi_filters: problem %d (c %d, n %d, ldw %d, %dx%d): %s", i, descs[i].c, descs[i].n, descs[i].ldw,
+                descs[i].kh, descs[i].kw, why);
+  };
+  if (n_layers > 0) {
+    if (!adam) RADNET_FAIL(ctx, RADNET_ERR_UNSUPPORTED, "conv_wgrad_multi_filters: the call has no optimizer block");
+    std::vector<int64_t> poff((size_t)n), loff((size_t)n_layers);
+    for (int i = 0; i < n; ++i) poff[(size_t)i] = descs[i].dw ? (int64_t)(descs[i].dw - opt->g) : -1;
+    for (int l = 0; l < n_layers; ++l) loff[(size_t)l] = layers[l].off;
+    if (wgrad_filter_match(poff.data(), n, loff.data(), n_layers, layer_of.data()) != 0)
+      RADNET_FAIL(ctx, RADNET_ERR_ARG, "conv_wgrad_multi_filters: every listed layer must be the dw of exactly one problem (by arena offset)");
+    for (int i = 0; i < n; ++i) {
+      if (layer_of[(size_t)i] < 0) continue;
+      const radnet_adam_wino& lw = layers[layer_of[(size_t)i]];
+      if (lw.c != descs[i].c || lw.n != descs[i].n)
+        RADNET_FAIL(ctx, RADNET_ERR_ARG, "conv_wgrad_multi_filters: layer %d is [3][3][%d][%d], its problem has c %d, n %d", layer_of[(size_t)i], lw.c, lw.n, descs[i].c, descs[i].n);
+      const int fp = wgrad_filter_footprints(filter_problem(i, 64, 64, 1u, true));
+      if (fp < 0) return filter_refused(i, fp);
+    }
   }
   std::vector<PairCapture> pcs((size_t)n);
   std::vector<WgradMultiItem> items((size_t)n);
@@ -336,6 +371,11 @@
     if (adam && !ordered && pc.gw.atomic)
       RADNET_FAIL(ctx, RADNET_ERR_UNSUPPORTED, "conv_wgrad_multi: problem %d adds its slices with atomics (no final writer); the optimizer epilogue needs ordered reductions", i);
     items[i] = WgradMultiItem{pc.w_bmk, pc.w_bn, pc.wx, pc.wy, pc.wz, ordered ? pc.w_slab_need : 0, ordered ? pc.wx * pc.wy : 0u};
+    if (layer_of[(size_t)i] >= 0) {
+      const int fp = wgrad_filter_footprints(filter_problem(i, pc.w_bmk, pc.w_bn, pc.wz, ordered));
+      if (fp < 0) return filter_refused(i, fp);
+      items[i].counters += (unsigned)fp;
+    }
   }
   std::vector<WgradMultiLaunch> plan((size_t)n);
   const int nl = wgrad_multi_plan(items.data(), n, ctx->ws_bytes, (unsigned)kAuxWgradCounterCount, plan.data(), n);
@@ -362,6 +402,12 @@
         const int64_t off = g.dw - opt->g;
         g.ow = opt->p + off; g.om = opt->m + off; g.ov = opt->v + off;
       }
+      g.ou = nullptr;
+      g.tap_counters = nullptr;
+      if (layer_of[(size_t)L.problem[k]] >= 0) {
+        g.ou = layers[layer_of[(size_t)L.problem[k]]].u;
+        g.tap_counters = reinterpret_cast<unsigned*>(ctx->aux + kAuxWgradCounters) + L.counter_off[k] + (g.slabs != nullptr ? pc.wx * pc.wy : 0u);
+      }
       flops += 2.0 * g.M * g.N * g.K;
     }
     const WgradArgs* tab = get_multi_table(ctx, host, L.n);
@@ -376,6 +422,15 @@
     radnet_timing_end_armed(ctx, 2, flops);
   }
   return RADNET_OK;
+}
+
+extern "C" int radnet_conv_wgrad_multi(radnet_ctx* ctx, const radnet_conv_desc* descs, int32_t n, const radnet_wgrad_adam* opt) {
+  return wgrad_multi_impl(ctx, descs, n, opt, nullptr, 0);
+}
+
+extern "C" int radnet_conv_wgrad_multi_filters(radnet_ctx* ctx, const radnet_conv_desc* descs, int32_t n, const radnet_wgrad_adam* opt,
+                                               const radnet_adam_wino* layers, int32_t n_layers) {
+  return wgrad_multi_impl(ctx, descs, n, opt, layers, n_layers);
 }
 
 extern "C" int radnet_wgrad_batched(radnet_ctx* ctx, const float* a, const float* dy, float* dw, int32_t batch, int32_t m, int32_t k, int32_t n,
diff --git a/rock-art-radnet_amd/csrc/conv_wgrad_body.h b/rock-art-radnet_amd/csrc/conv_wgrad_body.h
--- a/rock-art-radnet_amd/csrc/conv_wgrad_body.h
+++ b/rock-art-radnet_amd/csrc/conv_wgrad_body.h
@@ -1,6 +1,9 @@
 #pragma once
 #include "adam_update.h"
 #include "conv_device.h"
+#include "radnet_wino4.h"
+
+#include <type_traits>
 
 namespace {
 template <int BMK, int BN>
@@ -258,30 +261,62 @@
       const __amdgpu_buffer_rsrc_t rw = make_rsrc(g.ow + bp * g.dw_bstride, bytes), rm = make_rsrc(g.om + bp * g.dw_bstride, bytes),
                                    rv = make_rsrc(g.ov + bp * g.dw_bstride, bytes);
       const unsigned ldw4 = (unsigned)g.ldw * 4u;
-#pragma unroll
-      for (int j = 0; j < TN; ++j) {
-        const int n = n0 + wn * (BN / 2) + j * 32 + l31;
-#pragma unroll
-        for (int i = 0; i < TM; ++i) {
-          const int kb = k0 + wm * (BMK / 2) + i * 32 + 4 * hi;
-          const unsigned voff = (n < g.N && kb < g.K) ? ((unsigned)kb * (unsigned)g.ldw + (unsigned)n) * 4u : kOOB;
-          float pw[16], pm[16], pv[16];
-#pragma unroll
-          for (int r = 0; r < 16; ++r) {
-            const unsigned off = voff + (unsigned)((r & 3) + 8 * (r >> 2)) * ldw4;
-            pw[r] = buf_load1(rw, off);
-            pm[r] = buf_load1(rm, off);
-            pv[r] = buf_load1(rv, off);
-          }
-#pragma unroll
-          for (int r = 0; r < 16; ++r) {
-            const unsigned off = voff + (unsigned)((r & 3) + 8 * (r >> 2)) * ldw4;
-            adam_update1(pw[r], acc[i][j][r], pm[r], pv[r], g.lr_t, g.beta1, g.beta2, g.eps, g.grad_scale);
-            buf_store1(rw, off, pw[r]);
-            buf_store1(rm, off, pm[r]);
-            buf_store1(rv, off, pv[r]);
+      auto adam_tile = [&](auto filt) {
+#pragma unroll
+        for (int j = 0; j < TN; ++j) {
+          const int n = n0 + wn * (BN / 2) + j * 32 + l31;
+#pragma unroll
+          for (int i = 0; i < TM; ++i) {
+            const int kb = k0 + wm * (BMK / 2) + i * 32 + 4 * hi;
+            const unsigned voff = (n < g.N && kb < g.K) ? ((unsigned)kb * (unsigned)g.ldw + (unsigned)n) * 4u : kOOB;
+            float pw[16], pm[16], pv[16];
+#pragma unroll
+            for (int r = 0; r < 16; ++r) {
+              const unsigned off = voff + (unsigned)((r & 3) + 8 * (r >> 2)) * ldw4;
+              pw[r] = decltype(filt)::value ? buf_load1_sc1(rw, off) : buf_load1(rw, off);
+              pm[r] = buf_load1(rm, off);
+              pv[r] = buf_load1(rv, off);
+            }
+#pragma unroll
+            for (int r = 0; r < 16; ++r) {
+              const unsigned off = voff + (unsigned)((r & 3) + 8 * (r >> 2)) * ldw4;
+              adam_update1(pw[r], acc[i][j][r], pm[r], pv[r], g.lr_t, g.beta1, g.beta2, g.eps, g.grad_scale);
+              if constexpr (decltype(filt)::value) buf_store1_sc1(rw, off, pw[r]);
+              else buf_store1(rw, off, pw[r]);
+              buf_store1(rm, off, pm[r]);
+              buf_store1(rv, off, pv[r]);
+            }
           }
         }
+      };
+      if (g.ou == nullptr) {
+        adam_tile(std::false_type{});
+        return;
+      }
+      adam_tile(std::true_type{});
+      asm volatile("s_waitcnt vmcnt(0)" ::: "memory");
+      __syncthreads();
+      volatile int* last9 = reinterpret_cast<volatile int*>(lds);
+      if (tid == 0) {
+        unsigned* ctr = g.tap_counters + bid_y * (unsigned)(g.C / BMK) + (unsigned)(cbase / BMK);
+        const unsigned ticket = __hip_atomic_fetch_add(ctr, 1u, __ATOMIC_RELAXED, __HIP_MEMORY_SCOPE_AGENT);
+        const int last = ticket == 8u;
+        if (last) __hip_atomic_store(ctr, 0u, __ATOMIC_RELAXED, __HIP_MEMORY_SCOPE_AGENT);
+        last9[0] = last;
+      }
+      __syncthreads();
+      if (last9[0] == 0) return;
+      __builtin_amdgcn_fence(__ATOMIC_ACQUIRE, "wavefront");
+      const __amdgpu_buffer_rsrc_t ru = make_rsrc(g.ou, (unsigned)(36ull * (unsigned)g.C * (unsigned)g.N * 4ull));
+      const unsigned tap_bytes = (unsigned)g.C * ldw4, pos_bytes = (unsigned)g.C * (unsigned)g.N * 4u;
+#pragma unroll 1
+      for (int ch = tid; ch < BMK * CPRB; ch += NTHREADS) {
+        const int c = cbase + ch / CPRB, n = n0 + (ch % CPRB) * 4;
+        const bool live = c < g.C && n < g.N;
+        const unsigned woff = live ? ((unsigned)c * (unsigned)g.ldw + (unsigned)n) * 4u : kOOB;
+        const unsigned uoff = live ? ((unsigned)c * (unsigned)g.N + (unsigned)n) * 4u : kOOB;
+        wino4_filter_chunk([&](int tap) { return buf_load4_sc1(rw, woff + (unsigned)tap * tap_bytes); },
+                           [&](int p, const float4& o) { buf_store4(ru, uoff + (unsigned)p * pos_bytes, o); });
       }
       return;
     }
diff --git a/rock-art-radnet_amd/csrc/radnet_wino4.h b/rock-art-radnet_amd/csrc/radnet_wino4.h
--- a/rock-art-radnet_amd/csrc/radnet_wino4.h
+++ b/rock-art-radnet_amd/csrc/radnet_wino4.h
@@ -55,5 +55,24 @@
   w[2] = (s12 * (-1.f / 6.f) + s34 * (1.f / 6.f)) + u[5];
 }
 
+template <typename Tap, typename Emit> __device__ __forceinline__ void wino4_filter_chunk(Tap&& tap, Emit&& emit) {
+  float4 t[6][3];
+#pragma unroll
+  for (int b = 0; b < 3; ++b) {
+    float4 col[3], o[6];
+#pragma unroll
+    for (int a = 0; a < 3; ++a) col[a] = tap(a * 3 + b);
+    g6(col, o);
+#pragma unroll
+    for (int a = 0; a < 6; ++a) t[a][b] = o[a];
+  }
+#pragma unroll
+  for (int a = 0; a < 6; ++a) {
+    float4 o[6];
+    g6(t[a], o);
+#pragma unroll
+    for (int b = 0; b < 6; ++b) emit(6 * a + b, o[b]);
+  }
+}
 
 }
diff --git a/rock-art-radnet_amd/csrc/wgrad_multi_plan.cpp b/rock-art-radnet_amd/csrc/wgrad_multi_plan.cpp
--- a/rock-art-radnet_amd/csrc/wgrad_multi_plan.cpp
+++ b/rock-art-radnet_amd/csrc/wgrad_multi_plan.cpp
@@ -1,6 +1,35 @@
 #include "wgrad_multi_plan.h"
 
 #include <string.h>
+
+int wgrad_filter_footprints(const WgradFilterProblem& p) {
+  if (p.taps_h != 3 || p.taps_w != 3) return kWgradFilterErrTaps;
+  if ((p.bmk != 64 && p.bmk != 128) || (p.bn != 64 && p.bn != 128) || p.c <= 0 || p.c % p.bmk) return kWgradFilterErrChannels;
+  if (p.n <= 0 || p.ldw != p.n || (p.n & 3)) return kWgradFilterErrPitch;
+  const uint64_t w_bytes = (uint64_t)kWgradFilterTaps * (uint64_t)p.c * (uint64_t)p.n * 4u;
+  if (!p.u_addr || (p.u_addr & 15) || !p.w_addr || p.w_addr % kWgradFilterLine || w_bytes % kWgradFilterLine) return kWgradFilterErrAlign;
+  if (!p.optimizer) return kWgradFilterErrOptimizer;
+  if (p.slices == 0 || (p.slices > 1 && !p.ordered)) return kWgradFilterErrOrder;
+  if (4u * w_bytes >= (1ull << 31)) return kWgradFilterErrSize;
+  const uint64_t fp = (uint64_t)(p.c / p.bmk) * (uint64_t)((p.n + p.bn - 1) / p.bn);
+  return (int)fp;
+}
+
+int wgrad_filter_match(const int64_t* problem_off, int n, const int64_t* layer_off, int n_layers, int* layer_of) {
+  if (n < 0 || n_layers < 0 || (n > 0 && (!problem_off || !layer_of)) || (n_layers > 0 && !layer_off)) return kWgradMultiErrArg;
+  for (int i = 0; i < n; ++i) layer_of[i] = -1;
+  for (int l = 0; l < n_layers; ++l) {
+    int hit = -1;
+    for (int i = 0; i < n; ++i)
+      if (problem_off[i] == layer_off[l]) {
+        if (hit >= 0 || layer_of[i] >= 0) return kWgradFilterErrMatch;
+        hit = i;
+      }
+    if (hit < 0) return kWgradFilterErrMatch;
+    layer_of[hit] = l;
+  }
+  return 0;
+}
 
 int wgrad_multi_plan(const WgradMultiItem* items, int n, uint64_t ws_bytes, unsigned counter_cap, WgradMultiLaunch* out, int cap) {
   if (n < 0 || cap < 0 || (n > 0 && !items) || (cap > 0 && !out)) return kWgradMultiErrArg;
diff --git a/rock-art-radnet_amd/csrc/wgrad_multi_plan.h b/rock-art-radnet_amd/csrc/wgrad_multi_plan.h
--- a/rock-art-radnet_amd/csrc/wgrad_multi_plan.h
+++ b/rock-art-radnet_amd/csrc/wgrad_multi_plan.h
@@ -21,3 +21,21 @@
 constexpr int kWgradMultiErrArg = -1, kWgradMultiErrFit = -2, kWgradMultiErrCap = -3;
 
 int wgrad_multi_plan(const WgradMultiItem* items, int n, uint64_t ws_bytes, unsigned counter_cap, WgradMultiLaunch* out, int cap);
+
+struct WgradFilterProblem {
+  int taps_h, taps_w;
+  int c, n, ldw;
+  int bmk, bn;
+  unsigned slices;
+  int ordered;
+  int optimizer;
+  uint64_t w_addr, u_addr;
+};
+constexpr int kWgradFilterErrTaps = -11, kWgradFilterErrChannels = -12, kWgradFilterErrPitch = -13, kWgradFilterErrAlign = -14,
+              kWgradFilterErrOptimizer = -15, kWgradFilterErrOrder = -16, kWgradFilterErrMatch = -17, kWgradFilterErrSize = -18;
+constexpr int kWgradFilterTaps = 9;
+constexpr unsigned kWgradFilterLine = 128;
+
+int wgrad_filter_footprints(const WgradFilterProblem& p);
+inline unsigned wgrad_filter_counter(const WgradFilterProblem& p, unsigned kc, unsigned ntile) { return ntile * (unsigned)(p.c / p.bmk) + kc; }
+int wgrad_filter_match(const int64_t* problem_off, int n, const int64_t* layer_off, int n_layers, int* layer_of);
diff --git a/rock-art-radnet_amd/csrc/winograd.hip b/rock-art-radnet_amd/csrc/winograd.hip
--- a/rock-art-radnet_amd/csrc/winograd.hip
+++ b/rock-art-radnet_amd/csrc/winograd.hip
@@ -204,24 +204,10 @@
   const long long total = (long long)C * nv, ps = total;
   for (unsigned i = blockIdx.x * blockDim.x + threadIdx.x; i < (unsigned)total; i += gridDim.x * blockDim.x) {
     const int c = (int)(i / (unsigned)nv), nq = (int)(i - (unsigned)c * (unsigned)nv);
-    VT t[6][3];
-#pragma unroll
-    for (int b = 0; b < 3; ++b) {
-      VT col[3], o[6];
-#pragma unroll
-      for (int a = 0; a < 3; ++a) col[a] = *reinterpret_cast<const VT*>(g + ((long long)(a * 3 + b) * C + c) * ldw + nq * W);
-      g6(col, o);
-#pragma unroll
-      for (int a = 0; a < 6; ++a) t[a][b] = o[a];
-    }
+    static_assert(W == 4, "the shared chunk transform (radnet_wino4.h) works on float4");
     VT* dst = reinterpret_cast<VT*>(U) + (long long)c * nv + nq;
-#pragma unroll
-    for (int a = 0; a < 6; ++a) {
-      VT o[6];
-      g6(t[a], o);
-#pragma unroll
-      for (int b = 0; b < 6; ++b) dst[(6 * a + b) * ps] = o[b];
-    }
+    wino4_filter_chunk([&](int tap) { return *reinterpret_cast<const VT*>(g + ((long long)tap * C + c) * ldw + nq * W); },
+                       [&](int p, const VT& o) { dst[p * ps] = o; });
   }
 }
 
diff --git a/rock-art-radnet_amd/radnet_hip/engine.py b/rock-art-radnet_amd/radnet_hip/engine.py
--- a/rock-art-radnet_amd/radnet_hip/engine.py
+++ b/rock-art-radnet_amd/radnet_hip/engine.py
@@ -227,6 +227,7 @@
         self.wino_wgrad = os.environ.get("RADNET_NO_WINOGRAD_WGRAD", "0") != "1"
         self.head_wino_wgrad = self.head_train_wino and self.wino_wgrad and os.environ.get("RADNET_NO_HEAD_WINO_WGRAD", "0") != "1"
         self.head_deferred_wgrad = (self.HEAD_DEFERRED_WGRAD and precision == "fp32" and os.environ.get("RADNET_HEAD_DEFERRED_WGRAD", "1") != "0")
+        self.head_filters_in_wgrad = os.environ.get("RADNET_HEAD_FILTERS_IN_WGRAD", "1") != "0"
         self.ws = torch.empty(256 << 20, dtype=torch.uint8, device=self.dev)
         self.ctx.check(self.lib.radnet_set_workspace(self.ctx.h, self.ws.data_ptr(), self.ws.numel()), "set_workspace")
         self.autotune_mode = int(os.environ.get("RADNET_AUTOTUNE", int(autotune))) if autotune else 0
@@ -1220,15 +1221,28 @@
         arena = self.head_arena
         arena.t += 1
         modes = tuple(d.dw_accumulate for d in hp["bwd_wgrad"])
+        wino = self._head_adam_wino() if self.head_train_wino else None
+        in_wgrad = wino is not None and self.head_filters_in_wgrad
+        if in_wgrad:
+            if "_filters_fit" not in hp:
+                hp["_filters_fit"] = self._head_filters_fit(hp, wino)
+            in_wgrad = hp["_filters_fit"]
         ent = hp.get("_wgrad_arr")
-        if ent is None or ent[0] != modes:
-            ent = hp["_wgrad_arr"] = (modes, prog.desc_array(hp["bwd_wgrad"]))
+        if ent is None or ent[0] != (modes, in_wgrad):
+            descs = list(hp["bwd_wgrad"])
+            if in_wgrad:
+                descs.sort(key=lambda d: d.kh != 3)
+            ent = hp["_wgrad_arr"] = ((modes, in_wgrad), prog.desc_array(descs))
         opt = L.WgradAdam()
         opt.p, opt.g, opt.m, opt.v, opt.n, opt.t = arena.p.data_ptr(), arena.g.data_ptr(), arena.m.data_ptr(), arena.v.data_ptr(), arena.n, arena.t
         opt.lr, opt.beta1, opt.beta2, opt.eps, opt.grad_scale = self.lr, ADAM_BETA1, ADAM_BETA2, ADAM_EPS, grad_scale
-        self.ctx.check(self.lib.radnet_conv_wgrad_multi(self.ctx.h, ent[1], len(modes), C.byref(opt)), "radnet_conv_wgrad_multi")
         off = self.head_bias_off
-        wino = self._head_adam_wino() if self.head_train_wino else None
+        if in_wgrad:
+            self.ctx.check(self.lib.radnet_conv_wgrad_multi_filters(self.ctx.h, ent[1], len(modes), C.byref(opt), wino[0], wino[1]),
+                           "radnet_conv_wgrad_multi_filters")
+            wino = None
+        else:
+            self.ctx.check(self.lib.radnet_conv_wgrad_multi(self.ctx.h, ent[1], len(modes), C.byref(opt)), "radnet_conv_wgrad_multi")
         if wino is not None:
             self.ctx.call("radnet_adam_step_tail", arena.p, arena.g, arena.m, arena.v, C.c_int64(arena.n), arena.t, C.c_float(self.lr),
                           C.c_float(ADAM_BETA1), C.c_float(ADAM_BETA2), C.c_float(ADAM_EPS), C.c_float(grad_scale), 1, C.c_int64(off),
@@ -1237,10 +1251,18 @@
         self.ctx.call("radnet_adam_step_affine", arena.p[off:], arena.g[off:], arena.m[off:], arena.v[off:], C.c_int64(arena.n - off), arena.t,
                       C.c_float(self.lr), C.c_float(ADAM_BETA1), C.c_float(ADAM_BETA2), C.c_float(ADAM_EPS), C.c_float(grad_scale), 1,
                       C.c_int64(0), C.c_int64(self.head_bias_len), self.head_scale, self.head_t0, self.head_shift)
+        if in_wgrad:
+            return
         if self.head_train_wino:
             self._refresh_winograd(list(self.INFERENCE_WINOGRAD_LAYERS))
         else:
             self._inference_filters_stale = True
+
+    def _head_filters_fit(self, hp, wino):
+        arena = self.head_arena
+        offs = [(d.dw - arena.g.data_ptr()) // 4 for d in hp["bwd_wgrad"] if d.kh == 3 and d.kw == 3]
+        return all(wino[0][k].off in offs and (arena.p.data_ptr() + 4 * wino[0][k].off) % 128 == 0 and (36 * wino[0][k].c * wino[0][k].n) % 128 == 0
+                   for k in range(wino[1]))
 
     def head_backward(self, hp, accumulate=False, loss_out=None, on_part=None, defer_wgrad=False):
         G = hp.get("groups", 1)
diff --git a/rock-art-radnet_amd/radnet_hip/lib.py b/rock-art-radnet_amd/radnet_hip/lib.py
--- a/rock-art-radnet_amd/radnet_hip/lib.py
+++ b/rock-art-radnet_amd/radnet_hip/lib.py
@@ -233,6 +233,7 @@
         "radnet_conv_wgrad": (C.c_int, [vp, C.POINTER(ConvDesc)]),
         "radnet_conv_bwd": (C.c_int, [vp, C.POINTER(ConvDesc)]),
         "radnet_conv_wgrad_multi": (C.c_int, [vp, C.POINTER(ConvDesc), i32, C.POINTER(WgradAdam)]),
+        "radnet_conv_wgrad_multi_filters": (C.c_int, [vp, C.POINTER(ConvDesc), i32, C.POINTER(WgradAdam), C.POINTER(AdamWino), i32]),
         "radnet_conv_fwd_pair": (C.c_int, [vp, C.POINTER(ConvDesc), C.POINTER(ConvDesc)]),
         "radnet_conv_bottleneck": (C.c_int, [vp, C.POINTER(ConvDesc), C.POINTER(ConvDesc), C.POINTER(ConvDesc)]),
         "radnet_colsum": (C.c_int, [vp, vp, i32, i32, i32, vp, vp, i32]),
```

Result: no change. 605.8 images/sec, median of 6 (+0.3%).
